# oicr-gsi/ConsensusCruncher

Measured on AMD Instinct MI355X. Metric: input reads/sec through SSCS+DCS+SC consensus, higher is better.
Workload: dtype u8

## Files before the change

### consensuscruncher_amd/csrc/bam_assemble.hip.inc

```
#include "assemble_core.h"

namespace {

static_assert(sizeof(asmb::Spec) == sizeof(cc_out_spec), "asmb::Spec is cc_out_spec");
static_assert(sizeof(asmb::Src) == 40 && sizeof(cc_asm_src) == 48, "source layouts");

struct AsmStatus {
    unsigned long long first_bad;
    unsigned long long total;
    unsigned long long key_or;
    uint32_t max_size, guard;
    uint32_t tot, pad;
};
static_assert(sizeof(AsmStatus) == 40, "status layout");

constexpr int ASM_T = 256;
constexpr int ASM_LANES = 16;

struct DevFetch {
    static __device__ __forceinline__ upk::W16 fetch(const uint8_t* base, uint64_t a, uint32_t valid) {
        return DevSrc{base, 0}.fetch(a, valid);
    }
};

__global__ __launch_bounds__(ASM_T) void k_asm_sizes(asmb::Tables T, const asmb::Spec* __restrict__ spec, int64_t n,
                                                     uint32_t* __restrict__ sz, uint64_t* __restrict__ key,
                                                     uint32_t* __restrict__ val, AsmStatus* st) {
    __shared__ unsigned long long s_bad, s_tot, s_or;
    __shared__ uint32_t s_max;
    if (threadIdx.x == 0) { s_bad = ~0ULL; s_tot = 0; s_or = 0; s_max = 0; }
    __syncthreads();
    const int64_t i = (int64_t)blockIdx.x * ASM_T + threadIdx.x;
    if (i < n) {
        asmb::Lay y;
        uint64_t k = 0;
        const uint32_t e = asmb::layout(spec[i], T, y, &k);
        if (e) {
            atomicMin(&s_bad, ((unsigned long long)i << 8) | e);
            y.size = 0;
            k = 0;
        } else {
            atomicAdd(&s_tot, (unsigned long long)y.size);
            atomicOr(&s_or, (unsigned long long)k);
            atomicMax(&s_max, y.size);
        }
        sz[i] = y.size;
        key[i] = k;
        val[i] = (uint32_t)i;
    }
    __syncthreads();
    if (threadIdx.x == 0) {
        if (s_bad != ~0ULL) atomicMin(&st->first_bad, s_bad);
        atomicAdd(&st->total, s_tot);
        atomicOr(&st->key_or, s_or);
        atomicMax(&st->max_size, s_max);
    }
}

__global__ __launch_bounds__(ASM_T) void k_asm_gather(const uint32_t* __restrict__ sz, const uint32_t* __restrict__ perm,
                                                      int64_t n, int64_t o0, int64_t cnt, uint32_t* __restrict__ ssz) {
    const int64_t i = (int64_t)blockIdx.x * ASM_T + threadIdx.x;
    if (i >= cnt) return;
    const int64_t s = perm ? (int64_t)perm[o0 + i] : o0 + i;
    ssz[i] = sz[CC_IDX(s, n, DS_REC)];
}

__global__ __launch_bounds__(ASM_T) void k_asm_copy(asmb::Tables T, const asmb::Spec* __restrict__ spec,
                                                    const uint32_t* __restrict__ perm, int64_t n, int64_t o0, int64_t cnt,
                                                    const uint32_t* __restrict__ off32, uint64_t base, uint64_t total,
                                                    uint8_t* __restrict__ out, uint64_t* __restrict__ at, AsmStatus* st) {
    const int64_t i = (int64_t)blockIdx.x * (ASM_T / ASM_LANES) + (threadIdx.x / ASM_LANES);
    const uint32_t j = threadIdx.x % ASM_LANES;
    if (i >= cnt) return;
    const int64_t o = o0 + i;
    const int64_t s = perm ? (int64_t)perm[o] : o;
    asmb::Lay y;
    uint64_t k;
    const uint32_t e = asmb::layout(spec[CC_IDX(s, n, DS_REC)], T, y, &k);
    const uint64_t off = base + off32[i];
    if (e || off > total || y.size > total - off || (uint64_t)s >= (uint64_t)n) {
        if (j == 0) atomicOr(&st->guard, 1u);
        return;
    }
    if (j == 0) {
        at[o] = off;
        if (o == n - 1) at[n] = off + y.size;
    }
    uint8_t* d = out + off;
    const uint32_t head = min(y.size, (16u - ((uint32_t)off & 15u)) & 15u);
    const uint32_t lines = (y.size - head) >> 4, tail_at = head + (lines << 4);
    if (j < head) d[j] = (uint8_t)asmb::out16<DevFetch>(y, T, j, 1u).w[0];
    uint4* dl = reinterpret_cast<uint4*>(d + head);
    for (uint32_t c = j; c < lines; c += ASM_LANES) {
        const upk::W16 w = asmb::out16<DevFetch>(y, T, head + (c << 4), 16u);
        dl[c] = make_uint4(w.w[0], w.w[1], w.w[2], w.w[3]);
    }
    if (tail_at + j < y.size) d[tail_at + j] = (uint8_t)asmb::out16<DevFetch>(y, T, tail_at + j, 1u).w[0];
}

struct AsmGuard {
    cc_ctx* ctx;
    std::vector<void*> tmp;
    uint8_t* kept = nullptr;
    ~AsmGuard() {
        (void)hipStreamSynchronize(ctx->stream);
        for (void* p : tmp) (void)hipFree(p);
        if (kept) (void)hipFree(kept);
    }
};

int asm_upload_padded(cc_ctx* ctx, std::vector<void*>& tmp, const uint8_t** dst, const void* src, uint64_t bytes) {
    const size_t padded = (size_t)((bytes + 15) & ~15ull) + 32;
    uint8_t* up = nullptr;
    RC(dev_alloc(ctx, tmp, &up, (int64_t)padded));
    if (bytes) HIPCHK(hipMemcpyAsync(up, src, (size_t)bytes, hipMemcpyHostToDevice, ctx->stream));
    HIPCHK(hipMemsetAsync(up + bytes, 0, padded - (size_t)bytes, ctx->stream));
    *dst = up;
    return 0;
}

const char* asm_refusal(uint32_t bits) {
    if (bits & asmb::AE_KIND) return "unknown kind";
    if (bits & asmb::AE_SRC) return "src_file or src_rec out of range";
    if (bits & asmb::AE_TMPL) return "a template whose l_read_name, n_cigar and l_seq do not fit its block_size or its stream";
    if (bits & asmb::AE_NAME) return "name_id out of range";
    if (bits & asmb::AE_LONGNAME) return "a new name longer than 254 bytes";
    if (bits & asmb::AE_CONS) return "cons_off + cons_len outside the consensus arrays";
    return "rg_id outside the RG table";
}

struct AsmArgs {
// ... 115 lines not shown
            char buf[240];
            snprintf(buf, sizeof buf, "cc_bam_assemble: spec %lld: %s", (long long)(h_st->first_bad >> 8),
                     asm_refusal((uint32_t)(h_st->first_bad & 0xff)));
            ctx->err = buf;
            return CC_E_INVALID;
        }
        sum += h_st->total;
    }
    if (total) *total = sum;
    if (!alloc && !keep) return 0;
    uint8_t* out = alloc ? alloc(actx, sum) : nullptr;
    if ((alloc && !out) || !at) { ctx->err = "cc_bam_assemble: no buffer for the stream"; return CC_E_INVALID; }
    at[0] = a.header_bytes;
    uint8_t* d_out = nullptr;
    if (keep) {
        const size_t padded = (size_t)((sum + 15) & ~15ull) + 32;
        HIPCHK(hipMalloc((void**)&guard.kept, padded));
        d_out = guard.kept;
        HIPCHK(hipMemsetAsync(d_out + sum, 0, padded - (size_t)sum, ctx->stream));
    }
    if (n == 0) {
        if (a.header_bytes && out) memcpy(out, a.header, (size_t)a.header_bytes);
        if (keep) {
            if (a.header_bytes) HIPCHK(hipMemcpyAsync(d_out, a.header, (size_t)a.header_bytes, hipMemcpyHostToDevice, ctx->stream));
            HIPCHK(hipStreamSynchronize(ctx->stream));
            *keep = Resident{guard.kept, sum};
            guard.kept = nullptr;
        }
        return 0;
    }
    if (a.flags & CCIO_W_SORT) {
        unsigned b0 = 0, b1 = 0;
        asmb::key_digits(h_st->key_or, &b0, &b1);
        RC(dev_alloc(ctx, guard.tmp, &key2, n, 64));
        RC(dev_alloc(ctx, guard.tmp, &perm, n, 64));
        RC(sort_pairs(ctx, key, key2, val, perm, n, "asm_sort", b0, b1));
    }
    uint64_t bound = 0xffffffffull;
    if (const char* e = getenv("CC_ASM_SLICE_BYTES")) {
        const unsigned long long v = strtoull(e, nullptr, 10);
        if (v > 0 && v < bound) bound = v;
    }
    const int64_t per = asmb::slice_records(bound, h_st->max_size);
    const int64_t cap = std::min(per, n);
    RC(dev_alloc(ctx, guard.tmp, &ssz, cap, 64));
    RC(dev_alloc(ctx, guard.tmp, &off32, cap, 64));
    if (!keep) RC(dev_alloc(ctx, guard.tmp, &d_out, (int64_t)sum, 64));
    uint64_t* d_at = nullptr;
    RC(dev_alloc(ctx, guard.tmp, &d_at, n + 1));
    if (a.header_bytes) HIPCHK(hipMemcpyAsync(d_out, a.header, (size_t)a.header_bytes, hipMemcpyHostToDevice, ctx->stream));
    uint64_t base = a.header_bytes;
    for (int64_t o0 = 0; o0 < n; o0 += per) {
        const int64_t cnt = std::min(per, n - o0);
        klaunch(ctx, "k_asm_gather", k_asm_gather, nblk(cnt, ASM_T), ASM_T, sz, perm, n, o0, cnt, ssz);
        RC(scan_launch(ctx, ssz, cnt, &d_st->tot, "asm_scan", ScanStore{off32}));
        klaunch(ctx, "k_asm_copy", k_asm_copy, nblk(cnt, ASM_T / ASM_LANES), ASM_T, T, d_spec, perm, n, o0, cnt, off32, base, sum,
                d_out, d_at, d_st);
        HIPCHK(hipGetLastError());
        HIPCHK(hipMemcpyAsync(h_st, d_st, sizeof(AsmStatus), hipMemcpyDeviceToHost, ctx->stream));
        HIPCHK(hipStreamSynchronize(ctx->stream));
        if (h_st->guard) { ctx->err = "cc_bam_assemble: a record outside the stream (guarded)"; return CC_E_INVALID; }
        base += h_st->tot;
    }
    if (base != sum) { ctx->err = "cc_bam_assemble: the offsets' scan totals do not match the sizes"; return CC_E_INVALID; }
    if (out) {
        ProfScope ps(ctx, "asm_download");
        HIPCHK(hipMemcpyAsync(out, d_out, (size_t)sum, hipMemcpyDeviceToHost, ctx->stream));
        HIPCHK(hipMemcpyAsync(at, d_at, sizeof(uint64_t) * (size_t)(n + 1), hipMemcpyDeviceToHost, ctx->stream));
    } else {
        HIPCHK(hipMemcpyAsync(at, d_at, sizeof(uint64_t) * (size_t)(n + 1), hipMemcpyDeviceToHost, ctx->stream));
    }
    HIPCHK(hipStreamSynchronize(ctx->stream));
    if (keep) {
        *keep = Resident{guard.kept, sum};
        guard.kept = nullptr;
    }
    return 0;
}

int bam_assemble_locked(cc_ctx* ctx, const AsmArgs& a, cc_asm_alloc_fn alloc, void* actx, uint64_t* at, uint64_t* total,
                        int64_t* rid = nullptr) {
    if (rid) *rid = 0;
    if (!ctx) return CC_E_INVALID;
    if (a.n < 0 || a.nsrc < 0 || a.n_names < 0 || a.n_rg < 0 || (a.header_bytes && !a.header) ||
        (a.n > 0 && (!a.spec || (a.nsrc > 0 && !a.srcs))) || (a.n_names > 0 && !a.name_off && !a.names_set) || (a.names_bytes && !a.names && !a.names_set) ||
        (a.n_rg > 0 && (!a.rg_off || !a.rg_blob)) ||
        (a.cons_group < 0 && ((a.cons_seq_bytes && !a.cons_seq) || (a.cons_qual_bytes && !a.cons_qual)))) {
        ctx->err = "cc_bam_assemble: null or negative argument";
        return CC_E_INVALID;
    }
    if (a.cons_group >= 0 && !ctx->groups.count(a.cons_group)) { ctx->err = "cc_bam_assemble: unknown group"; return CC_E_INVALID; }
    if (a.names_set) {
        const auto it = ctx->name_sets.find(a.names_set);
        if (it == ctx->name_sets.end()) { ctx->err = "cc_bam_assemble: unknown name set"; return CC_E_INVALID; }
        if (a.n_names > it->second.n || a.names_bytes > (uint64_t)it->second.total) {
            ctx->err = "cc_bam_assemble: n_names or names_bytes larger than the name set's";
            return CC_E_INVALID;
        }
    }
    std::vector<const uint8_t*> resident((size_t)a.nsrc, nullptr);
    bool any = false;
    for (int32_t f = 0; f < a.nsrc; ++f) {
        const cc_asm_src& s = a.srcs[f];
        if (s.nrec < 0 || (s.nrec > 0 && !s.rec_off) || (!s.stream && !s.resident_id && s.bytes)) {
            ctx->err = "cc_bam_assemble: a source without a stream";
            return CC_E_INVALID;
        }
// ... 115 lines not shown
```

### consensuscruncher_amd/csrc/cc_engine.hip

```cpp
#include <algorithm>
#include <climits>
#include <cstdint>
#include <cstdio>
#include <cstring>

#include <dlfcn.h>
#include <sched.h>

#include <chrono>

#include <hip/hip_runtime.h>
#include <atomic>
#include <map>
#include <memory>
#include <mutex>
#include <type_traits>
#include <string>
#include <unordered_map>
#include <unordered_set>
#include <utility>
#include <vector>

#include "../../include/consensuscruncher_amd.h"

static std::atomic<long long> g_launches{0};
#define hipMemsetAsync(...) (g_launches.fetch_add(1, std::memory_order_relaxed), ::hipMemsetAsync(__VA_ARGS__))
#define hipMemcpyAsync(...) (g_launches.fetch_add(1, std::memory_order_relaxed), ::hipMemcpyAsync(__VA_ARGS__))

enum : uint32_t {
    EB_COLLISION = 1u << 0,
    EB_DUP_QNAME = 1u << 1,
    EB_N_HIGHQ = 1u << 3,
    EB_BAD_BASE = 1u << 4,
    EB_SHORT = 1u << 5,
    EB_NO_QUAL = 1u << 6,
    EB_NO_CIGAR = 1u << 7,
    EB_RG = 1u << 8,
    EB_THR = 1u << 9,
    EB_TOO_LONG = 1u << 10,
    EB_KEYERROR = 1u << 12,
    EB_CHAIN = 1u << 13,
    EB_NEEDSORT = 1u << 14,
    EB_PLAN = 1u << 11,
    EB_DEEPSORT = 1u << 15,
    EB_SCANWAIT = 1u << 16,
    EB_GUARD = 1u << 17,
};

__device__ unsigned int g_guard;
__device__ __noinline__ int64_t guard_fail() {
    atomicOr(&g_guard, 1u);
    return 0;
}
#ifdef CC_DEBUG_BOUNDS
__device__ unsigned long long g_dbg_fault;
__device__ __noinline__ int64_t dbg_fail(int site, int64_t i) {
    atomicCAS(&g_dbg_fault, 0ULL, ((unsigned long long)site << 48) | ((unsigned long long)i & 0xffffffffffffULL));
    return 0;
}
__device__ __forceinline__ int64_t dbg_idx(int64_t i, int64_t n, int site) {
    return (i < 0 || i >= n) ? dbg_fail(site, i) : i;
}
#define CC_IDX(i, n, site) ((std::remove_cv_t<std::remove_reference_t<decltype(i)>>)dbg_idx((int64_t)(i), (int64_t)(n), (site)))
#elif defined(CC_NO_GUARD)
#define CC_IDX(i, n, site) (i)
#else
__device__ __forceinline__ int64_t guard_idx(int64_t i, int64_t n) {
    return (uint64_t)i < (uint64_t)n ? i : guard_fail();
}
#define CC_IDX(i, n, site) ((std::remove_cv_t<std::remove_reference_t<decltype(i)>>)guard_idx((int64_t)(i), (int64_t)(n)))
#endif
enum : int {
    DS_REC = 1, DS_QNAME = 2, DS_PAYLOAD = 3, DS_SLOT = 4, DS_PAIR = 5, DS_MEMBER = 6, DS_VOTE_REC = 7,
};

struct TagKey {
    int32_t bc, tid, pos, mtid, mpos, cigA, cigB;
    uint32_t bits;
};
struct CKey {
    int32_t bc, tidLo, posLo, tidHi, posHi, cigA, cigB;
    uint32_t strand;
    uint32_t abstlen;
    uint32_t pad[3];
};

constexpr int GRP_SMALL = 64;

struct alignas(32) RecCore {
    int32_t tid, pos, mtid, mpos, tlen, cig, bc, flag;
};

struct DevTable {
    int64_t n;
    int32_t *tid, *pos, *mtid, *mpos, *tlen, *cig, *qlen, *lseq, *bc, *rg;
    uint16_t* flag;
    uint8_t *mapq, *rflags;
    uint64_t* qn_off;
    uint16_t* qn_len;
    uint64_t* qn_ol;
    RecCore* core;
    uint8_t* qn_blob;
    uint64_t* pay_off;
    uint8_t* payload;
    uint64_t pay_bytes, qn_bytes;
    uint64_t* rdig;
    uint64_t* qdig;
    uint64_t qdig_mask;
    uint4* meta;
    uint64_t* rkey;
    uint32_t* ebits;
    uint8_t* rdeep;
    int32_t* dlist;
    uint32_t* ndeep;
    int64_t n_deep;
    bool derive_pending;
    bool host_layout;
    int32_t max_len;
    int64_t* tbase;
    int32_t* ext;
    int32_t* geom;
    int32_t ntid;
    int64_t bkt_cap;
};

__device__ __forceinline__ uint32_t nib_irregular(uint32_t x, uint32_t m88) {
    uint32_t p = x - ((x >> 1) & 0x55555555u);
    p = (p & 0x33333333u) + ((p >> 2) & 0x33333333u);
    const uint32_t a = p ^ 0x11111111u, b = p ^ 0x44444444u;
    const uint32_t za = ~((a | 0x88888888u) - 0x11111111u) & 0x88888888u;
    const uint32_t zb = ~((b | 0x88888888u) - 0x11111111u) & 0x88888888u;
    return ~(za | zb) & m88;
}
__device__ __forceinline__ uint32_t nib_mask(int nbase, int w) {
    int vb = nbase - 8 * w;
    vb = vb < 0 ? 0 : (vb > 8 ? 8 : vb);
    const int full = vb >> 1;
    uint32_t m = full >= 4 ? 0x88888888u : (((1u << (8 * full)) - 1u) & 0x88888888u);
    if ((vb & 1) && full < 4) m |= 0x80u << (8 * full);
    return m;
}

constexpr int BC_T = 256;
__device__ __forceinline__ uint64_t pos_key(int32_t tid, int32_t pos) {
    return ((uint64_t)(uint32_t)(tid < 0 ? -1 : tid) << 32) | (uint64_t)(uint32_t)pos;
}

constexpr int DEEP_MIN = 65;
constexpr uint64_t QDIG_SEED = 0x6a09e667f3bcc909ULL;
__device__ __forceinline__ uint64_t qname_hash(const DevTable& T, int32_t r, uint64_t seed);
__device__ __forceinline__ void build_meta_rec(const DevTable& T, int32_t* __restrict__ rec_e, uint32_t* __restrict__ err,
                                               int32_t* __restrict__ dlist, uint32_t* __restrict__ ndeep, int64_t dcap) {
    const int64_t r = (int64_t)blockIdx.x * BC_T + threadIdx.x;
    if (r == 0) {
        const uint32_t eb = *T.ebits;
        if (eb) atomicOr(err, eb);
    }
    if (dlist) {
        bool dp = false;
        if (r < T.n) {
            const int32_t t = T.tid[r], p = T.pos[r];
            const bool start = r == 0 || T.tid[r - 1] != t || T.pos[r - 1] != p;
            const int64_t q = r + DEEP_MIN - 1;
            dp = start && q < T.n && T.tid[q] == t && T.pos[q] == p;
// ... 2153 lines not shown
                    for (int k = 0; k < SE / 2; ++k) {
                        const uint32_t i = (uint32_t)((h + k) * DF_ST + t);
                        const uint32_t pm = A[lo[k] + sp - 1];
                        if ((i & w) ? (pm <= v[k]) : (pm < v[k])) lo[k] += sp;
                    }
                }
#pragma unroll
                for (int k = 0; k < SE / 2; ++k) {
                    const uint32_t i = (uint32_t)((h + k) * DF_ST + t);
                    if (i >= p2) continue;
                    const uint32_t pm = A[lo[k]];
                    if ((i & w) ? (pm <= v[k]) : (pm < v[k])) lo[k] += 1;
                    const uint32_t st = i & ~(2 * w - 1), other = st + ((i & w) ? 0u : w);
                    B[st + (i & (w - 1)) + (lo[k] - other)] = v[k];
                }
            }
            __syncthreads();
            uint32_t* tmp = A; A = B; B = tmp;
        }
        for (int h = 0; h < SE; h += SE / 2) {
            uint32_t v[SE / 2];
            int32_t r[SE / 2];
#pragma unroll
            for (int k = 0; k < SE / 2; ++k) {
                const uint32_t i = (uint32_t)((h + k) * DF_ST + t);
                v[k] = i < m ? A[i] : 0u;
                r[k] = i < m ? CC_IDX((v[k] & 1u) ? V.rec2[v[k] >> 1] : V.rec1[v[k] >> 1], T.n, DS_REC) : 0;
            }
#pragma unroll
            for (int k = 0; k < SE / 2; ++k) {
                const uint32_t i = (uint32_t)((h + k) * DF_ST + t);
                if (i < m) deep_put(out, V, T, d.z + (int64_t)i, v[k], r[k], i == 0, i == 0 || (v[k] >> 1) != (A[i - 1] >> 1), err);
            }
        }
    }
}

__global__ __launch_bounds__(256) void k_fam_build(int64_t F, int64_t R, int64_t n_known, int one_region,
                                                   const int32_t* __restrict__ fam_beg,
                                                   const int32_t* __restrict__ fam_drop,
                                                   const uint32_t* __restrict__ rs_val, const uint64_t* __restrict__ rs_key,
                                                   const int32_t* __restrict__ pr_region, const uint64_t* __restrict__ rhash,
                                                   const int32_t* __restrict__ mem_rec, int32_t* __restrict__ fam_end,
                                                   int32_t* __restrict__ fam_n, int32_t* __restrict__ fam_first,
                                                   int32_t* __restrict__ fam_region, uint64_t* __restrict__ fam_hash,
                                                   uint8_t* __restrict__ cflag, int32_t* __restrict__ cfam,
                                                   int32_t* __restrict__ fam_o, PairView V, DevTable T,
                                                   TagKey* __restrict__ fam_tag, int32_t* __restrict__ fam_rec) {
    int64_t f = (int64_t)blockIdx.x * blockDim.x + threadIdx.x;
    if (f < F) {
        fam_o[f] = 0x7f7f7f7f;
        int32_t b = CC_IDX(fam_beg[f], R, DS_SLOT);
        int32_t e = (f + 1 < F) ? fam_beg[f + 1] : (int32_t)R;
        if (e < b || e > R) e = b + (int32_t)guard_fail() + 1;
        fam_end[f] = e;
        fam_n[f] = e - b - fam_drop[f];
        uint32_t fe = rs_val[b];
        fam_first[f] = (int32_t)fe;
        fam_region[f] = one_region ? 0 : pr_region[fe >> 1];
        fam_hash[f] = rhash && b >= n_known ? rhash[CC_IDX(mem_rec[b], T.n, DS_REC)] : rs_key[b];
        cflag[fe] = 1;
        cfam[fe] = (int32_t)f;
        if (fam_tag) {
            const int32_t r0 = mem_rec[b];
            fam_tag[f] = tag_of_rec(T, r0, V.tag[fe >> 1]);
            fam_rec[f] = r0;
        }
    }
}

__global__ __launch_bounds__(256) void k_fam_tags(int64_t F, const int32_t* __restrict__ fam_first,
                                                  const int32_t* __restrict__ fam_beg, const int32_t* __restrict__ mem_rec,
                                                  PairView V, DevTable T, TagKey* __restrict__ fam_tag,
                                                  int32_t* __restrict__ fam_rec) {
    const int64_t f = (int64_t)blockIdx.x * blockDim.x + threadIdx.x;
    if (f < F) {
        const int32_t r0 = mem_rec[fam_beg[f]];
        fam_tag[f] = tag_of_rec(T, r0, V.tag[fam_first[f] >> 1]);
        fam_rec[f] = r0;
    }
}

__global__ __launch_bounds__(256) void k_csn_keys(int64_t F, const int32_t* __restrict__ fam_by_k,
                                                  const int32_t* __restrict__ fam_first, const uint64_t* __restrict__ chash,
                                                  uint64_t* __restrict__ ekey, uint32_t* __restrict__ eval) {
    int64_t k = (int64_t)blockIdx.x * blockDim.x + threadIdx.x;
    if (k >= F) return;
    int32_t f = fam_by_k[k];
    ekey[k] = chash[fam_first[f] >> 1];
    eval[k] = (uint32_t)k;
}

__global__ __launch_bounds__(256) void k_csn_mark(int64_t F, const uint64_t* __restrict__ es_key,
                                                  const uint32_t* __restrict__ es_val, const int32_t* __restrict__ fam_by_k,
                                                  const int32_t* __restrict__ fam_first, PairView V, DevTable T,
                                                  uint32_t* __restrict__ segf, uint32_t* __restrict__ err) {
    int64_t j = (int64_t)blockIdx.x * blockDim.x + threadIdx.x;
    if (j >= F) return;
    bool start = (j == 0) || es_key[j - 1] != es_key[j];
    if (!start) {
        int32_t pa = fam_first[fam_by_k[es_val[j]]] >> 1, pb = fam_first[fam_by_k[es_val[j - 1]]] >> 1;
        if (!ckey_eq(ckey_of_pair(T, V, pa), ckey_of_pair(T, V, pb))) {
            atomicOr(err, EB_COLLISION);
            start = true;
        }
    }
    segf[j] = start;
// ... 535 lines not shown
    for (int pi = 0; pi < 4; ++pi) {
        int32_t c = 0;
#pragma unroll
        for (int i = 0; i < MODE_K; ++i)
            if (i < nv && val[i] == pri[pi]) c = num[i];
        if (c == best_cnt) { out = pri[pi]; return true; }
    }
    return true;
}

struct SwarWord {
    uint32_t pc, ca, cc, cg, orb, ql;
};

__device__ __forceinline__ uint32_t ff_of_80(uint32_t m80) { return (m80 - (m80 >> 7)) | m80; }

__device__ __forceinline__ uint32_t min60_bytes(uint32_t q) {
    const uint32_t hi = ff_of_80((((q | 0x80808080u) - 0x3d3d3d3du) | q) & 0x80808080u);
    return (hi & 0x3c3c3c3cu) | (~hi & q);
}

__device__ __forceinline__ void swar_member(SwarWord& s, uint32_t w, uint32_t q) {
    const uint32_t p80 = (((q | 0x80808080u) - 0x1e1e1e1eu) | q) & 0x80808080u;
    const uint32_t p1 = p80 >> 7;
    const uint32_t pff = (p80 - p1) | p80;
    s.pc += p1;
    s.ql = (q & pff) | (s.ql & ~pff);
    const uint32_t wp = w & pff;
    s.orb |= wp;
    s.ca += wp & 0x01010101u;
    s.cc += wp & 0x02020202u;
    s.cg += wp & 0x04040404u;
}

__global__ __launch_bounds__(256) void k_vote_plan(
    int64_t n, int64_t nmem, int64_t nvcap, const uint8_t* __restrict__ needv, const uint32_t* __restrict__ vx,
    const int32_t* __restrict__ emit_fam, const int2* __restrict__ emit_span, const uint4* __restrict__ mem_meta,
    const int32_t* __restrict__ mem_rec, DevTable T, int32_t* __restrict__ vote_fam, int4* __restrict__ vote_order,
    int32_t* __restrict__ emit_vslot, int32_t* __restrict__ out_meta, uint32_t* __restrict__ slow_n,
    int32_t* __restrict__ slow_list, uint32_t* __restrict__ n_items, int all_slow, uint32_t* __restrict__ err) {
    __shared__ uint32_t s_bin[64], s_cur[64];
    __shared__ int64_t s_vb;
    const int tid = threadIdx.x;
    const int64_t o = (int64_t)blockIdx.x * blockDim.x + tid;
    int4 rec = make_int4(0, 0, 0, -1);
    int key = -1;
    uint32_t eb = 0;
    if (o < n) {
        const bool need = needv[o] != 0;
        const uint32_t vxo = vx[o];
        const int32_t f = emit_fam[o];
        int2 sp = emit_span[o];
        const bool over = need && (int64_t)vxo >= nvcap;
        if (over) guard_fail();
        if (!need || over) {
            emit_vslot[o] = -1;
        } else {
            const int32_t v = (int32_t)vxo;
            vote_fam[v] = f;
            emit_vslot[o] = v;
            if (sp.x < 0 || sp.y < 0 || (int64_t)sp.x + sp.y > nmem) sp = make_int2((int32_t)guard_fail(), 0);
            const int32_t beg = sp.x, cnt = sp.y;
            const uint4* fm = mem_meta + beg;
            const uint4 m0 = cnt > 0 ? fm[0] : make_uint4(0u, 0u, 0u, 0u);
            const uint32_t ql0 = m0.z >> 16;
            const int32_t L = ql0 == 0xffffu ? -1 : (int32_t)ql0;
            uint32_t d = 0;
            const bool slow = cnt > VOTE_BIGN || all_slow;
            for (int32_t k0 = 0; !slow && k0 < cnt; k0 += 4) {
                uint4 mm[4];
#pragma unroll
                for (int u = 0; u < 4; ++u) mm[u] = k0 + u < cnt ? fm[k0 + u] : make_uint4(0u, 0u, 0u, 0u);
#pragma unroll
                for (int u = 0; u < 4; ++u) {
                    const uint4 m = mm[u];
                    if (!((m.w >> 23) & 1u)) continue;
                    const uint32_t ls = m.z & 0xffffu;
                    if (L < 0) eb |= EB_NO_CIGAR;
                    else if ((int32_t)ls < L) eb |= EB_SHORT;
                    if (((m.w >> 20) & CC_RF_QUAL_MISSING) && L > 0) eb |= EB_NO_QUAL;
                    if (((m.w >> 12) & 0xffu) != ((m0.w >> 12) & 0xffu)) d |= 1u;
                    if (m.y != m0.y) d |= 2u;
                    if ((m.w & 0xfffu) != (m0.w & 0xfffu)) d |= 4u;
                    const uint32_t rg7 = (m.w >> 24) & 0x7fu;
                    const bool badrg = ((m.w >> 20) & CC_RF_RG_UNSUPPORTED) != 0;
                    if (rg7 != ((m0.w >> 24) & 0x7fu)) d |= 8u;
                    if (rg7 == 0x7eu) d |= 64u;
                    if (rg7 == 0x7fu && !badrg) d |= 16u;
                    if (badrg) d |= 32u;
                }
            }
            key = 0;
            rec = make_int4(beg, 0, 0, v);
            if (slow) {
                slow_list[atomicAdd(slow_n, 1u)] = v;
                if (cnt > BIG_CH) atomicAdd(n_items, (uint32_t)((cnt + BIG_CH - 1) / BIG_CH));
                eb = 0;
            } else {
                int32_t mapq = (int32_t)((m0.w >> 12) & 0xffu), tlen = (int32_t)m0.y, flag = (int32_t)(m0.w & 0xfffu);
                const auto g_mapq = [](const uint4& m) { return (int32_t)((m.w >> 12) & 0xffu); };
                const auto g_tlen = [](const uint4& m) { return (int32_t)m.y; };
                const auto g_flag = [](const uint4& m) { return (int32_t)(m.w & 0xfffu); };
                if ((d & 1u) && !table_mode(cnt, fm, g_mapq, false, mapq))
                    mapq = serial_mode(0, cnt, fm, [&](int32_t, const uint4& m) { return g_mapq(m); }, false);
                if ((d & 2u) && !table_mode(cnt, fm, g_tlen, false, tlen))
                    tlen = serial_mode(0, cnt, fm, [&](int32_t, const uint4& m) { return g_tlen(m); }, false);
                if ((d & 4u) && !table_mode(cnt, fm, g_flag, true, flag))
                    flag = serial_mode(0, cnt, fm, [&](int32_t, const uint4& m) { return g_flag(m); }, true);
                int32_t rg = -1;
                if (!(d & 16u)) {
                    if (d & 32u) eb |= EB_RG;
                    else if (!(d & (8u | 64u))) rg = (int32_t)((m0.w >> 24) & 0x7fu);
                    else rg = serial_mode(0, cnt, fm, [&](int32_t j, const uint4& m) {
                        const uint32_t r7 = (m.w >> 24) & 0x7fu;
                        return r7 == 0x7eu ? T.rg[mem_rec[beg + j]] : (int32_t)r7; }, false);
                }
                const int32_t Lp = L < 0 ? 0 : L;
                out_meta[5 * v + 0] = Lp;
                out_meta[5 * v + 1] = mapq;
                out_meta[5 * v + 2] = tlen;
                out_meta[5 * v + 3] = flag;
                out_meta[5 * v + 4] = rg;
                rec = make_int4(beg, cnt, Lp, v);
                key = cnt;
            }
        }
    }
    if (eb) atomicOr(err, eb);
    if (tid < 64) s_bin[tid] = 0u;
    if (tid == 0) s_vb = (int64_t)blockIdx.x * blockDim.x < n ? (int64_t)vx[(int64_t)blockIdx.x * blockDim.x] : 0;
    __syncthreads();
    if (key >= 0) atomicAdd(&s_bin[key], 1u);
    __syncthreads();
    if (tid < 64) {
        const uint32_t c = s_bin[tid];
        uint32_t x = c;
#pragma unroll
        for (int d2 = 1; d2 < 64; d2 <<= 1) {
            const uint32_t y = __shfl_up(x, d2, 64);
            if (tid >= d2) x += y;
        }
        s_cur[tid] = x - c;
    }
    __syncthreads();
    if (key >= 0) {
        const int64_t at = s_vb + atomicAdd(&s_cur[key], 1u);
        if (at < nvcap) vote_order[at] = rec;
        else guard_fail();
    }
}

__device__ __noinline__ uint32_t lone_quality(const uint4* __restrict__ fm, int32_t cnt, int32_t i, uint32_t code,
                                              const uint8_t* __restrict__ payload) {
    uint32_t qs = 0;
    for (int32_t k = 0; k < cnt; ++k) {
        const uint4 mk = fm[k];
        const uint32_t lsk = mk.z & 0xffffu;
        if (!((mk.w >> 23) & 1u) || i >= (int32_t)lsk) continue;
        const uint64_t qok = (uint64_t)mk.x << 4;
        const uint32_t qq = payload[qok + i];
        const uint32_t by = payload[qok + ((lsk + 15u) & ~15u) + (i >> 1)];
        const uint32_t b = (i & 1) ? (by & 15u) : (by >> 4);
        if (qq >= 30u && b == code) qs += qq;
    }
    return qs > 60u ? 60u : qs;
}

__device__ __noinline__ bool passing_n(const uint4* __restrict__ fm, int32_t cnt, int32_t i,
                                       const uint8_t* __restrict__ payload) {
    for (int32_t k = 0; k < cnt; ++k) {
        const uint4 mk = fm[k];
        const uint32_t lsk = mk.z & 0xffffu;
        if (!((mk.w >> 23) & 1u) || i >= (int32_t)lsk) continue;
        const uint64_t qok = (uint64_t)mk.x << 4;
        const uint32_t by = payload[qok + ((lsk + 15u) & ~15u) + (i >> 1)];
        const uint32_t b = (i & 1) ? (by & 15u) : (by >> 4);
        if (payload[qok + i] >= 30u && b == 15u) return true;
    }
    return false;
}

__device__ __forceinline__ void swar_finish(SwarWord (&s)[4], const uint32_t (&lm)[4], uint32_t irr, bool act,
                                            int32_t i0, int32_t cnt, int64_t v, const uint4* __restrict__ fm,
                                            const DevTable& T, const int32_t* __restrict__ thr, int32_t uni_ok,
                                            int32_t qstride, uint8_t* __restrict__ out_seq,
                                            uint8_t* __restrict__ out_qual, uint32_t& eb) {
    if (irr) eb |= EB_BAD_BASE;
    uint32_t code[4], qo[4], multi = 0;
#pragma unroll
    for (int w = 0; w < 4; ++w) {
        const SwarWord& x = s[w];
        const uint32_t z80 = ~((x.pc | 0x80808080u) - 0x01010101u) & 0x80808080u;
        const uint32_t z15 = (z80 >> 3) - (z80 >> 7);
        code[w] = uni_ok ? (x.orb | z15) : 0x0f0f0f0fu;
        const uint32_t g2 = ff_of_80(((x.pc | 0x80808080u) - 0x02020202u) & 0x80808080u);
        qo[w] = (g2 & 0x3c3c3c3cu) | (~g2 & min60_bytes(x.ql));
        const uint32_t mu = x.orb & ((x.orb | 0x80808080u) - 0x01010101u) & lm[w];
        const uint32_t mb = ((mu | (mu >> 1) | (mu >> 2) | (mu >> 3)) & 0x01010101u) * 0x01020408u;
        multi |= (mb >> 24) << (4 * w);
    }
#pragma unroll 1
// ... 5 lines not shown
#define SV_SEL4(f) (w == 0 ? s[0].f : w == 1 ? s[1].f : w == 2 ? s[2].f : s[3].f)
        const uint32_t xca = SV_SEL4(ca), xcc = SV_SEL4(cc), xcg = SV_SEL4(cg), xpc = SV_SEL4(pc), xql = SV_SEL4(ql),
                       xorb = SV_SEL4(orb);
#undef SV_SEL4
        const int32_t a = (int32_t)((xca >> sh) & 0xffu);
        const int32_t cC = (int32_t)(((xcc >> sh) & 0xffu) >> 1);
        const int32_t gG = (int32_t)(((xcg >> sh) & 0xffu) >> 2);
        const int32_t pass = (int32_t)((xpc >> sh) & 0xffu);
        const int32_t tT = pass - a - cC - gG;
        const int32_t pos = i0 + 8 * (w >> 1) + 2 * j + (w & 1);
        if (((xorb >> sh) & 0xffu) == 15u && passing_n(fm, cnt, pos, T.payload)) eb |= EB_N_HIGHQ;
        int32_t best = a, mbase = 0;
        if (cC > best) { best = cC; mbase = 1; }
        if (gG > best) { best = gG; mbase = 2; }
        if (tT > best) { best = tT; mbase = 3; }
        const uint32_t cj = (pass > 0 && best >= thr[pass]) ? (1u << mbase) : 15u;
        uint32_t qj;
        if (best >= 2) qj = 60u;
        else if (best <= 0) qj = 0u;
        else if (pass == 1) { const uint32_t qq = (xql >> sh) & 0xffu; qj = qq > 60u ? 60u : qq; }
        else qj = lone_quality(fm, cnt, pos, 1u << mbase, T.payload);
        const uint32_t keep = ~(0xffu << sh);
        if (w == 0) { code[0] = (code[0] & keep) | (cj << sh); qo[0] = (qo[0] & keep) | (qj << sh); }
        else if (w == 1) { code[1] = (code[1] & keep) | (cj << sh); qo[1] = (qo[1] & keep) | (qj << sh); }
        else if (w == 2) { code[2] = (code[2] & keep) | (cj << sh); qo[2] = (qo[2] & keep) | (qj << sh); }
        else { code[3] = (code[3] & keep) | (cj << sh); qo[3] = (qo[3] & keep) | (qj << sh); }
    }
    if (act) {
        uint4 qout;
        qout.x = __builtin_amdgcn_perm(qo[1] & lm[1], qo[0] & lm[0], 0x05010400u);
        qout.y = __builtin_amdgcn_perm(qo[1] & lm[1], qo[0] & lm[0], 0x07030602u);
        qout.z = __builtin_amdgcn_perm(qo[3] & lm[3], qo[2] & lm[2], 0x05010400u);
        qout.w = __builtin_amdgcn_perm(qo[3] & lm[3], qo[2] & lm[2], 0x07030602u);
        *reinterpret_cast<uint4*>(out_qual + v * (int64_t)qstride + i0) = qout;
        *reinterpret_cast<uint2*>(out_seq + v * (int64_t)(qstride >> 1) + (i0 >> 1)) =
            make_uint2(((code[0] & lm[0]) << 4) | (code[1] & lm[1]), ((code[2] & lm[2]) << 4) | (code[3] & lm[3]));
    }
}

__global__ __launch_bounds__(256, CC_SV_WAVES) void k_sscs_vote_swar(
    int64_t nv, int32_t fpw, int32_t chunks, const int4* __restrict__ vote_order, const uint4* __restrict__ mem_meta,
    int64_t nmem, DevTable T, const int32_t* __restrict__ thr, int32_t uni_ok, int32_t qstride,
    uint8_t* __restrict__ out_seq, uint8_t* __restrict__ out_qual, uint32_t* __restrict__ err) {
    const int lane = threadIdx.x & 63;
    const int64_t wave = (int64_t)blockIdx.x * (blockDim.x >> 6) + (threadIdx.x >> 6);
    const int g = lane / chunks, c = lane - g * chunks;
    const int64_t t = wave * fpw + g;
    int32_t beg = 0, cnt = 0, L = 0;
    int64_t v = 0;
    if (g < fpw && t < nv) {
        const int4 vi = vote_order[t];
        beg = vi.x; cnt = vi.y; L = vi.z; v = vi.w;
        if (beg < 0 || cnt < 0 || (int64_t)beg + cnt > nmem || v < 0 || v >= nv) {
            beg = (int32_t)guard_fail();
            cnt = 0;
        }
    }
    const int32_t i0 = SV_POS * c;
    uint32_t eb = 0;
    const bool act = i0 < L;
    if (cnt > 0) {
        uint32_t lm[4];
        {
            uint32_t lp[4];
#pragma unroll
            for (int k = 0; k < 4; ++k) {
                const int32_t rem = L - i0 - 4 * k;
                lp[k] = rem >= 4 ? 0xffffffffu : (rem <= 0 ? 0u : ((1u << (8 * rem)) - 1u));
            }
            lm[0] = __builtin_amdgcn_perm(lp[1], lp[0], 0x06040200u);
            lm[1] = __builtin_amdgcn_perm(lp[1], lp[0], 0x07050301u);
            lm[2] = __builtin_amdgcn_perm(lp[3], lp[2], 0x06040200u);
            lm[3] = __builtin_amdgcn_perm(lp[3], lp[2], 0x07050301u);
        }
        SwarWord s[4];
#pragma unroll
        for (int k = 0; k < 4; ++k) s[k] = SwarWord{};
        const uint4* fm = mem_meta + beg;
        const int nbl = L - i0 < 16 ? (L - i0 > 0 ? L - i0 : 0) : 16;
        const uint32_t irx = nib_mask(nbl, 0), iry = nib_mask(nbl, 1);
        uint32_t irr = 0;
        const int gl = g * chunks;
        for (int32_t k0 = 0; k0 < cnt; k0 += chunks) {
            const uint4 mine = (k0 + c < cnt) ? fm[k0 + c] : make_uint4(0u, 0u, 0u, 0u);
            const int kn = cnt - k0 < chunks ? cnt - k0 : chunks;
            for (int u0 = 0; u0 < kn; u0 += SV_U) {
                uint4 qv[SV_U];
                uint2 sv[SV_U];
                uint32_t vm[SV_U];
#pragma unroll
                for (int u = 0; u < SV_U; ++u) {
                    const int src = gl + (u0 + u < kn ? u0 + u : kn - 1);
                    const uint32_t mx = (uint32_t)__shfl((int)mine.x, src);
                    const uint32_t mz = (uint32_t)__shfl((int)mine.z, src);
                    const uint32_t mw = (uint32_t)__shfl((int)mine.w, src);
                    const uint32_t ls = mz & 0xffffu;
                    const bool ok = act & (u0 + u < kn) & (((mw >> 23) & 1u) != 0u) & (i0 < (int32_t)ls);
                    vm[u] = ok ? 0xffffffffu : 0u;
                    const uint32_t off = ok ? (uint32_t)i0 : 0u;
                    const uint8_t* base = T.payload + CC_IDX((uint64_t)mx << 4, T.pay_bytes + 1, DS_PAYLOAD);
                    qv[u] = *reinterpret_cast<const uint4*>(base + off);
                    sv[u] = *reinterpret_cast<const uint2*>(base + ((ls + 15u) & ~15u) + (off >> 1));
                }
#pragma unroll
                for (int u = 0; u < SV_U; ++u) {
                    const uint4 q = qv[u];
                    const uint2 sq = sv[u];
// ... 573 lines not shown
            if (s >= 0) { dx = 1; break; }
            if (g < 0) { dx = 3; break; }
            if (G.fam_o[g] >= ox) { dx = 2; comp = false; break; }
            if (n == DUPLEX_CHAIN) { atomicOr(err, EB_CHAIN); break; }
            ++n;
            x = g;
            ox = G.fam_o[g];
        }
        for (int i = n - 1; i >= 0; --i) {
            const bool deleted = dx == 1 || dx == 3 || (dx == 2 && comp);
            if (deleted) { dx = 3; comp = false; }
            else { comp = dx == 2 && !comp; dx = 2; }
        }
        d = dx == 1 ? 0 : dx == 2 ? 1 : 2;
        if (d == 0) pr = S.fam_rec[s0];
        else if (d == 1) pr = G.fam_rec[g0];
        if (gdel) {
            const int32_t rt = G.fam_region[f];
            if (dx == 1) { atomicMin(&gdel[f], rt); atomicMin(&sdel[s0], rt); }
            else if (dx == 3) atomicMin(&gdel[f], rt);
            else if (dx == 2 && comp) { atomicMin(&gdel[f], rt); atomicMin(&gdel[g0], rt); }
        }
    }
    dec[q] = d;
    t_rec[q] = tr;
    p_rec[q] = pr;
    fl_corr[q] = (d == 0 || d == 1) ? 1 : 0;
}


__device__ __forceinline__ void duplex_word(uint32_t wa, uint32_t wb, uint32_t qa, uint32_t qb, int sc,
                                            uint32_t& code, uint32_t& qual) {
    uint32_t ok = ~(((wa ^ wb) | 0x80808080u) - 0x01010101u) & 0x80808080u;
    if (sc) {
        ok &= (((qa | 0x80808080u) - 0x1e1e1e1eu) | qa) & 0x80808080u;
        ok &= (((qb | 0x80808080u) - 0x1e1e1e1eu) | qb) & 0x80808080u;
    }
    const uint32_t ff = ff_of_80(ok);
    code = (wa & ff) | (0x0f0f0f0fu & ~ff);
    qual = min60_bytes(min60_bytes(qa) + min60_bytes(qb)) & ff;
}

__global__ __launch_bounds__(256) void k_duplex_vote_swar(
    int64_t nv, int sc, int32_t fpw, int32_t chunks, const int4* __restrict__ vpair,
    DevTable TA, DevTable TB, int32_t qstride, uint8_t* __restrict__ out_seq, uint8_t* __restrict__ out_qual,
    int32_t* __restrict__ out_meta, uint32_t* __restrict__ err) {
    const int lane = threadIdx.x & 63;
    const int64_t wave = (int64_t)blockIdx.x * (blockDim.x >> 6) + (threadIdx.x >> 6);
    const int g = lane / chunks, c = lane - g * chunks;
    const int64_t w = wave * fpw + g;
    uint32_t eb = 0;
    if (g < fpw && w < nv) {
        const int4 vp = vpair[w];
        const int32_t a = CC_IDX(vp.x, TA.n, DS_VOTE_REC), b = vp.y;
        const bool b_in_a = sc && vp.z == 1;
        const DevTable& TBx = b_in_a ? TA : TB;
        const uint8_t* bpay = TBx.payload;
        const uint4 ma = TA.meta[a], mb = TBx.meta[CC_IDX(b, TBx.n, DS_VOTE_REC)];
        const int32_t la = (int32_t)(ma.z & 0xffffu), lb = (int32_t)(mb.z & 0xffffu);
        int32_t L = la;
        if (lb < L) { eb |= EB_SHORT; L = 0; }
        if (L > 0 && (((ma.w | mb.w) >> 20) & CC_RF_QUAL_MISSING)) eb |= EB_NO_QUAL;
        for (int32_t i0 = SV_POS * c; i0 < L; i0 += SV_POS * chunks) {
            const uint64_t qa = (uint64_t)ma.x << 4, qb = (uint64_t)mb.x << 4;
            const uint64_t sa = qa + (uint64_t)((la + 15) & ~15), sb = qb + (uint64_t)((lb + 15) & ~15);
            const uint4 QA = *reinterpret_cast<const uint4*>(TA.payload + qa + i0);
            const uint4 QB = *reinterpret_cast<const uint4*>(bpay + qb + i0);
            const uint2 SA = *reinterpret_cast<const uint2*>(TA.payload + sa + (i0 >> 1));
            const uint2 SB = *reinterpret_cast<const uint2*>(bpay + sb + (i0 >> 1));
            uint32_t lp[4];
#pragma unroll
            for (int k = 0; k < 4; ++k) {
                const int32_t rem = L - i0 - 4 * k;
                lp[k] = rem >= 4 ? 0xffffffffu : (rem <= 0 ? 0u : ((1u << (8 * rem)) - 1u));
            }
            const uint4 QM = make_uint4(QA.x & lp[0], QA.y & lp[1], QA.z & lp[2], QA.w & lp[3]);
            const uint4 QN = make_uint4(QB.x & lp[0], QB.y & lp[1], QB.z & lp[2], QB.w & lp[3]);
            uint32_t code[4], qo[4];
            duplex_word((SA.x >> 4) & 0x0f0f0f0fu, (SB.x >> 4) & 0x0f0f0f0fu,
                        __builtin_amdgcn_perm(QM.y, QM.x, 0x06040200u), __builtin_amdgcn_perm(QN.y, QN.x, 0x06040200u),
                        sc, code[0], qo[0]);
            duplex_word(SA.x & 0x0f0f0f0fu, SB.x & 0x0f0f0f0fu,
                        __builtin_amdgcn_perm(QM.y, QM.x, 0x07050301u), __builtin_amdgcn_perm(QN.y, QN.x, 0x07050301u),
                        sc, code[1], qo[1]);
            duplex_word((SA.y >> 4) & 0x0f0f0f0fu, (SB.y >> 4) & 0x0f0f0f0fu,
                        __builtin_amdgcn_perm(QM.w, QM.z, 0x06040200u), __builtin_amdgcn_perm(QN.w, QN.z, 0x06040200u),
                        sc, code[2], qo[2]);
            duplex_word(SA.y & 0x0f0f0f0fu, SB.y & 0x0f0f0f0fu,
                        __builtin_amdgcn_perm(QM.w, QM.z, 0x07050301u), __builtin_amdgcn_perm(QN.w, QN.z, 0x07050301u),
                        sc, code[3], qo[3]);
            const uint32_t lm0 = __builtin_amdgcn_perm(lp[1], lp[0], 0x06040200u);
            const uint32_t lm1 = __builtin_amdgcn_perm(lp[1], lp[0], 0x07050301u);
            const uint32_t lm2 = __builtin_amdgcn_perm(lp[3], lp[2], 0x06040200u);
            const uint32_t lm3 = __builtin_amdgcn_perm(lp[3], lp[2], 0x07050301u);
            code[0] &= lm0; code[1] &= lm1; code[2] &= lm2; code[3] &= lm3;
            uint4 qout;
            qout.x = __builtin_amdgcn_perm(qo[1], qo[0], 0x05010400u) & lp[0];
            qout.y = __builtin_amdgcn_perm(qo[1], qo[0], 0x07030602u) & lp[1];
            qout.z = __builtin_amdgcn_perm(qo[3], qo[2], 0x05010400u) & lp[2];
            qout.w = __builtin_amdgcn_perm(qo[3], qo[2], 0x07030602u) & lp[3];
            *reinterpret_cast<uint4*>(out_qual + w * (int64_t)qstride + i0) = qout;
            *reinterpret_cast<uint2*>(out_seq + w * (int64_t)(qstride >> 1) + (i0 >> 1)) =
                make_uint2((code[0] << 4) | code[1], (code[2] << 4) | code[3]);
        }
        if (c == 0) {
            const int fa = (int)(ma.w & 0xfffu), fb = (int)(mb.w & 0xfffu);
            int32_t mapq = (int32_t)((ma.w >> 12) & 0xffu), tlen = (int32_t)ma.y, flag = fa, rg;
            const int32_t ra = TA.rg[a], rb = TBx.rg[b];
            if (sc) {
                rg = ra;
                if ((ma.w >> 20) & CC_RF_RG_UNSUPPORTED) eb |= EB_RG;
// ... 446 lines not shown
    __syncthreads();
    if (base + SCAN_TILE <= n) {
        if constexpr (Emit::kStaged) {
            typename Emit::Ld ld[SCAN_I];
            uint32_t fx[SCAN_I], xx[SCAN_I];
#pragma unroll
            for (int j = 0; j < SCAN_I / 4; ++j) {
                const int o = (j * SCAN_T + tid) * 4;
                const uint4 x = reinterpret_cast<const uint4*>(s_tile)[o >> 2];
                const uint32_t f = *reinterpret_cast<const uint32_t*>(in + base + o);
                xx[4 * j] = x.x; xx[4 * j + 1] = x.y; xx[4 * j + 2] = x.z; xx[4 * j + 3] = x.w;
#pragma unroll
                for (int k = 0; k < 4; ++k) fx[4 * j + k] = (f >> (8 * k)) & 0xffu;
            }
#pragma unroll
            for (int e = 0; e < SCAN_I; ++e) ld[e] = em.ld1(base + ((e >> 2) * SCAN_T + tid) * 4 + (e & 3), fx[e]);
#pragma unroll
            for (int e = 0; e < SCAN_I; ++e) em.ld2(ld[e], fx[e]);
#pragma unroll
            for (int e = 0; e < SCAN_I; ++e) em.st(base + ((e >> 2) * SCAN_T + tid) * 4 + (e & 3), xx[e], fx[e], ld[e]);
        } else {
#pragma unroll
            for (int j = 0; j < SCAN_I / 4; ++j) {
                const int o = (j * SCAN_T + tid) * 4;
                const uint4 x = reinterpret_cast<const uint4*>(s_tile)[o >> 2];
                if constexpr (Emit::kPlain) {
                    *reinterpret_cast<uint4*>(em.out + base + o) = x;
                } else {
                    const uint32_t f = *reinterpret_cast<const uint32_t*>(in + base + o);
                    em(base + o, x.x, f & 0xffu);
                    em(base + o + 1, x.y, (f >> 8) & 0xffu);
                    em(base + o + 2, x.z, (f >> 16) & 0xffu);
                    em(base + o + 3, x.w, f >> 24);
                }
            }
        }
    } else {
        for (int o = tid; o < SCAN_TILE; o += SCAN_T) {
            if (base + o >= n) continue;
            if constexpr (Emit::kPlain) em.out[base + o] = s_tile[o];
            else emit_one(em, base + o, s_tile[o], (uint32_t)in[base + o]);
        }
    }
}

__device__ __forceinline__ uint32_t stripe_sum(const uint32_t* __restrict__ stripes, int slot) {
    uint32_t v = 0;
    if (stripes)
        for (int k = 0; k < PSTRIPES; ++k) v += stripes[((int64_t)slot * PSTRIPES + k) * PSTRIDE];
    return v;
}

__global__ __launch_bounds__(64) void k_guard_fold(uint32_t* __restrict__ err) {
    if (threadIdx.x == 0 && g_guard) {
        atomicOr(err, EB_GUARD);
        g_guard = 0u;
    }
}
__global__ __launch_bounds__(256) void k_defer_pack(const uint32_t* __restrict__ err,
                                                    const unsigned long long* __restrict__ cnt,
                                                    const uint32_t* __restrict__ plan, int nplan,
                                                    const uint32_t* __restrict__ stripes, uint8_t* __restrict__ h) {
    const int t = threadIdx.x;
    if (t == 0) {
        *reinterpret_cast<uint32_t*>(h) = *err | (g_guard ? EB_GUARD : 0u);
        if (g_guard) g_guard = 0u;
    }
    if (cnt && t < CC_NUM_COUNTERS) {
        unsigned long long v = 0;
        for (int k = 0; k < CNT_STRIPES; ++k) v += cnt[CC_NUM_COUNTERS * k + t];
        reinterpret_cast<unsigned long long*>(h + 1024)[t] = v;
    }
    if (plan)
        for (int i = t; i < nplan; i += blockDim.x)
            reinterpret_cast<uint32_t*>(h + 256)[i] = plan[i] + stripe_sum(stripes, i);
}

__global__ __launch_bounds__(64) void k_stripe_fold(const uint32_t* __restrict__ stripes, uint32_t* __restrict__ plan,
                                                    int nplan) {
    for (int i = threadIdx.x; i < nplan; i += blockDim.x) plan[i] += stripe_sum(stripes, i);
}

constexpr int RS_T = 256, RS_I = 16, RS_TILE = RS_T * RS_I, RS_BINS = 256;
__global__ __launch_bounds__(RS_T) void k_rs_hist(const uint64_t* __restrict__ keys, int64_t n, int shift,
                                                  uint32_t* __restrict__ hist, int64_t nt) {
    __shared__ uint32_t s_h[RS_BINS];
    const int t = threadIdx.x;
    s_h[t] = 0u;
    __syncthreads();
    const int64_t base = (int64_t)blockIdx.x * RS_TILE;
    uint32_t d[RS_I];
#pragma unroll
    for (int i = 0; i < RS_I; ++i) {
        const int64_t x = base + (int64_t)i * RS_T + t;
        d[i] = x < n ? (uint32_t)(keys[x] >> shift) & 255u : 0xffffffffu;
    }
#pragma unroll
    for (int i = 0; i < RS_I; ++i)
        if (d[i] != 0xffffffffu) atomicAdd(&s_h[d[i]], 1u);
    __syncthreads();
    hist[(int64_t)t * nt + blockIdx.x] = s_h[t];
}
__global__ __launch_bounds__(RS_T) void k_rs_scatter(const uint64_t* __restrict__ kin, const uint32_t* __restrict__ vin,
                                                     int64_t n, int shift, const uint32_t* __restrict__ off, int64_t nt,
                                                     uint64_t* __restrict__ kout, uint32_t* __restrict__ vout) {
    __shared__ uint32_t s_base[RS_BINS];
    __shared__ uint32_t s_wc[RS_T / 64][RS_BINS];
    const int t = threadIdx.x, lane = t & 63, wv = t >> 6;
    s_base[t] = off[(int64_t)t * nt + blockIdx.x];
#pragma unroll
    for (int w = 0; w < RS_T / 64; ++w) s_wc[w][t] = 0u;
    const uint64_t lt = (1ULL << lane) - 1ULL;
    const int64_t base = (int64_t)blockIdx.x * RS_TILE;
    for (int i = 0; i < RS_I; ++i) {
        const int64_t x = base + (int64_t)i * RS_T + t;
        const bool valid = x < n;
        const uint64_t k = valid ? kin[x] : 0ULL;
        const uint32_t v = valid ? vin[x] : 0u;
        const uint32_t d = (uint32_t)(k >> shift) & 255u;
// ... 60 lines not shown
    X(vote_slow_list, int32_t) X(cutoff_thr, int32_t) X(vote_big_item, int32_t) X(vote_items, int4)                  \
    X(vote_partial, uint8_t) X(vote_item_fl, uint32_t) X(bc_swap, int32_t) X(dec, int32_t) X(t_rec, int32_t)         \
    X(p_rec, int32_t) X(fl_dcs, uint8_t) X(fl_corr, uint8_t) X(ht_key, unsigned long long) X(ht_val, int32_t)        \
    X(fam_bkt, int32_t) X(fam_del, int32_t) X(vslot, int32_t) X(vpair, int4) X(q_pair, int32_t) X(q_ckey, int32_t)   \
                               \
    X(grp_keys, uint32_t) X(grp_tab, int32_t) X(grp_slot_of, int32_t) X(grp_slot_first, int32_t)                     \
    X(grp_slot_cnt, int32_t) X(grp_start, uint32_t) X(grp_fx, uint32_t) X(grp_fsize, uint32_t)                       \
    X(grp_foff, uint32_t) X(grp_fkey, uint64_t) X(grp_fval, uint32_t) X(grp_skey, uint64_t) X(grp_sval, uint32_t)    \
    X(join_keys, uint32_t) X(join_pkeys, uint32_t) X(join_xkeys, uint32_t) X(join_tab, int32_t)                      \
    X(join_xtab, int32_t) X(join_p, int32_t) X(join_xs, int32_t) X(join_xfirst, int32_t) X(join_indeg, int32_t)      \
    X(join_dec, int32_t) X(join_part, int32_t) X(join_flags, uint32_t) X(join_used, uint8_t) X(join_gone, uint8_t)   \
    X(join_xgone, uint8_t) X(eb_h1, uint8_t) X(eb_h2, uint8_t) X(eb_l1, int32_t) X(eb_l2, int32_t)                   \
    X(eb_status, uint8_t) X(eb_bc, char) X(eb_cut1, int32_t) X(eb_cut2, int32_t) X(eb_bad1, uint32_t)                \
    X(eb_bad2, uint32_t) X(eb_counts, unsigned long long) X(eb_hist, unsigned long long)                             \
    X(eb_tkey, unsigned long long) X(eb_tval, int32_t) X(reduce_buf, int64_t) X(reduce_max, int64_t)

enum class B : int {
#define X(name, T) name,
    CC_GROUP_BUFFERS(X)
#undef X
    COUNT
};
constexpr const char* BUF_NAME[] = {
#define X(name, T) #name,
    CC_GROUP_BUFFERS(X)
#undef X
};
template <B id> struct BufType;
#define X(name, T) template <> struct BufType<B::name> { using type = T; };
CC_GROUP_BUFFERS(X)
#undef X
template <B id> using BufT = typename BufType<id>::type;

#define CC_PLAN_TOTALS(X)                                                                                            \
    X(n_resid) X(n_big) X(n_drop) X(n_long) X(lp_found) X(n_multi) X(resid_app) X(lp_total) X(resid_multi)           \
    X(deep_ovf) X(deep_items) X(deep_big) X(csn_shared) X(scan_resid) X(scan_pairs) X(scan_small) X(scan_bigE)       \
    X(scan_deep) X(scan_fam) X(scan_creation) X(scan_entries) X(scan_emit) X(scan_vote) X(vote_items) X(vote_slow)   \
    X(scan_bad) X(scan_dcs) X(scan_sc) X(grp_scan_fam) X(grp_scan_off)

enum class PT : int {
#define X(name) name,
    CC_PLAN_TOTALS(X)
#undef X
    COUNT
};
constexpr const char* PLAN_NAME[] = {
#define X(name) #name,
    CC_PLAN_TOTALS(X)
#undef X
};
constexpr int PLAN_SLOTS = 64;
static_assert((int)PT::COUNT <= PLAN_SLOTS, "a planned total's slot is its id");

enum Stage { ST_READ_BAM, ST_SSCS, ST_DCS, ST_SC, ST_COUNT };
constexpr const char* STAGE_NAME[ST_COUNT] = {"read_bam", "sscs", "dcs", "sc"};

struct Group {
    int32_t table = -1;
    int64_t S = 0, P = 0, R = 0, F = 0, E = 0, Q = 0, NV = 0;
    uint64_t seed = 0;
    int scoped = 0, delim_filter = 0, badread = 0;
    uint64_t ht_mask = 0;
    bool csn_fast = false;
    bool stripes_pending = false;
    bool no_deep_fam = false;
    int coord_sorted = 0;
    bool force_sort = false;
    int ident = 0;
    bool local_groups = false;
    int64_t counters[CC_NUM_COUNTERS] = {0};
    DevBuf buf[(int)B::COUNT];
    template <B id> BufT<id>* ptr() const { return (BufT<id>*)buf[(int)id].p; }
    int64_t plan[(int)PT::COUNT] = {0};
    bool plan_set[(int)PT::COUNT] = {false};
    bool planned[ST_COUNT] = {false};
    bool fast = false;
    bool members_built = false;
    int64_t n_deepg = 0;
    bool fam_tags_built = false;
    bool overlap = false;
    int32_t n_regions = 1;
    std::vector<PT> verify;
    std::vector<int32_t> swap_host;
    double thr_cutoff = -1.0;
};

struct DeferredCheck {
    Group* g = nullptr;
    int32_t gid = -1;
    int slot = 0;
    bool counters = false;
    bool bad_listed = false;
    std::vector<std::pair<int, int64_t>> expect;
};
constexpr int DEFER_SLOTS = 64;
constexpr size_t DEFER_SLOT_BYTES = 12288;

constexpr int CC_E_PLAN = -100;
constexpr int CC_E_NEEDSORT = -101;
constexpr int CC_E_DEEPSORT = -102;
constexpr int CC_E_SCANWAIT = -103;

using NameIndex = std::unordered_map<std::string, int>;
NameIndex name_index(const char* const* names, int n) {
    NameIndex ix;
    for (int i = 0; i < n; ++i) ix[names[i]] = i;
    return ix;
}
const NameIndex BUF_IDS = name_index(BUF_NAME, (int)B::COUNT);
const NameIndex PLAN_IDS = name_index(PLAN_NAME, (int)PT::COUNT);
inline int name_id(const NameIndex& ix, const char* name) {
    const auto it = ix.find(name);
    return it != ix.end() ? it->second : -1;
}

struct EngineSwitches {
    int scan1 = -1;
    int pc_tile = 0;
    bool resid_sort = false;
    bool resid_scan = false;
    bool qdig = true;
    int qdig_bits = 0;
    bool dcs_per_entry = false;
    int64_t lp_min = LP_MIN;
    bool ltab_cas = false;
    bool group_staged = false;
    bool meta_scalar = false;
    bool derive_separate = false;
    bool gr_by_pair = false;
    bool deep_sort = false;
    bool trace_upload = false;
};

EngineSwitches read_switches() {
    EngineSwitches sw;
    if (const char* v = getenv("CC_SCAN1")) sw.scan1 = v[0] == '1' ? 1 : 0;
    if (const char* v = getenv("CC_PC_TILE")) sw.pc_tile = atoi(v) == 512 ? 512 : 1024;
    sw.resid_sort = getenv("CC_RESID_SORT") != nullptr;
    sw.resid_scan = getenv("CC_RESID_SCAN") != nullptr;
    if (const char* v = getenv("CC_QDIG")) sw.qdig = v[0] != '0';
    if (const char* v = getenv("CC_QDIG_BITS")) sw.qdig_bits = atoi(v) > 0 && atoi(v) < 64 ? atoi(v) : 0;
    sw.dcs_per_entry = getenv("CC_DCS_PER_ENTRY") != nullptr;
    if (const char* v = getenv("CC_LP_MIN")) sw.lp_min = atoll(v);
    sw.ltab_cas = getenv("CC_LTAB_CAS") != nullptr;
    sw.group_staged = getenv("CC_GROUP_STAGED") != nullptr;
    sw.meta_scalar = getenv("CC_META_SCALAR") != nullptr;
    sw.derive_separate = getenv("CC_DERIVE_SEPARATE") != nullptr;
    sw.gr_by_pair = getenv("CC_GR_BY_PAIR") != nullptr;
    sw.deep_sort = getenv("CC_DEEP_SORT") != nullptr;
    sw.trace_upload = getenv("CC_TRACE_UPLOAD") != nullptr;
    return sw;
}

}

struct BgzfEnc;

struct NameSet {
    uint8_t* blob = nullptr;
    int64_t* off = nullptr;
    int64_t n = 0, total = 0;
};

struct cc_ctx {
    int device = 0;
    hipStream_t stream = nullptr;
    std::string err;
    EngineSwitches sw;
    std::map<int32_t, DevTable> tables;
    std::map<int32_t, std::vector<void*>> table_allocs;
    std::map<int32_t, std::unique_ptr<Group>> groups;
    int32_t next_id = 1;
    DevBuf tmp;
    DevBuf sort_buf;
    unsigned long long* scan_st = nullptr;
    uint32_t* scan_ticket = nullptr;
    int64_t scan_cap = 0;
    uint32_t scan_epoch = 0;
    uint32_t scan_spin_max = 1u << 22;
    bool scan_two = false;
    std::unordered_set<int32_t> full_qhash;
    int64_t scan_retries = 0;
    int64_t guard_reruns = 0;
    uint32_t* d_err = nullptr;
    unsigned long long* d_cnt = nullptr;
    void* h_pinned = nullptr;
    std::atomic<bool> profiling{false};
    std::unordered_set<std::string> prof_only;
    struct Prof { double ms = 0; int64_t n = 0; };
    std::map<std::string, Prof> prof;
    std::vector<std::pair<std::string, std::pair<hipEvent_t, hipEvent_t>>> pending;
    std::vector<hipEvent_t> event_pool;
    std::unique_ptr<Group> scratch;
    bool defer = false;
    std::vector<DeferredCheck> deferred;
    uint8_t* h_defer = nullptr;
    uint8_t* d_defer = nullptr;
    BgzfEnc* bgzf = nullptr;
    std::mutex bgzf_mu;
    int32_t asm_group = -1;
    uint8_t* names_buf = nullptr;
    int64_t names_total = -1;
    int64_t* names_off = nullptr;
    int64_t names_n = 0;
    std::map<int64_t, NameSet> name_sets;
    int64_t asm_names = 0;
};

namespace {

#define HIPCHK(x)                                                                               \
    do {                                                                                        \
        hipError_t e_ = (x);                                                                    \
        if (e_ != hipSuccess) {                                                                 \
            ctx->err = std::string("HIP error ") + hipGetErrorString(e_) + " at " #x;           \
            return CC_E_HIP;                                                                    \
        }                                                                                       \
    } while (0)

#define RC(x)                     \
    do {                          \
        int rc_ = (x);            \
        if (rc_) return rc_;      \
    } while (0)

int enter(cc_ctx* ctx) {
    HIPCHK(hipSetDevice(ctx->device));
    ctx->sw = read_switches();
    return 0;
}

inline unsigned nblk(int64_t n, int b = 256) { return (unsigned)((n + b - 1) / b); }

template <class... P, class... A>
inline void klaunch(hipStream_t stream, void (*kernel)(P...), dim3 grid, dim3 block, A&&... args) {
    g_launches.fetch_add(1, std::memory_order_relaxed);
    kernel<<<grid, block, 0, stream>>>(std::forward<A>(args)...);
}
template <class... P, class... A>
inline void klaunch(cc_ctx* ctx, void (*kernel)(P...), dim3 grid, dim3 block, A&&... args) {
    klaunch(ctx->stream, kernel, grid, block, std::forward<A>(args)...);
}

struct Fills {
    cc_ctx* ctx;
    FillSet fs{};
    int64_t maxw = 0;
    explicit Fills(cc_ctx* c) : ctx(c) { fs.k = 0; }
    int add(void* p, size_t bytes, uint32_t word) {
        if (!p || bytes < 4) return 0;
        if (fs.k == FillSet::K) { int rc = launch(); if (rc) return rc; }
        fs.p[fs.k] = (uint32_t*)p;
        fs.n[fs.k] = (int64_t)(bytes / 4);
        fs.v[fs.k] = word;
        maxw = std::max<int64_t>(maxw, (int64_t)(bytes / 4));
        ++fs.k;
        return 0;
    }
    int launch();
};

void* gbuf_bytes(cc_ctx* ctx, Group& g, B id, size_t need, int* rc) {
    DevBuf& b = g.buf[(int)id];
    if (b.bytes < need) {
        if (b.p) (void)hipFree(b.p);
        b.p = nullptr;
        hipError_t e = hipMalloc(&b.p, need);
        if (e != hipSuccess) {
            ctx->err = std::string("hipMalloc failed for ") + BUF_NAME[(int)id] + ": " + hipGetErrorString(e);
            *rc = CC_E_HIP;
            b.bytes = 0;
            return nullptr;
        }
        b.bytes = need;
    }
    return b.p;
}

template <B id>
BufT<id>* gbuf(cc_ctx* ctx, Group& g, int64_t count, int* rc) {
    using T = BufT<id>;
    void* p = gbuf_bytes(ctx, g, id, (size_t)std::max<int64_t>(count, 1) * sizeof(T), rc);
    if (p) g.buf[(int)id].used = (size_t)std::max<int64_t>(count, 0) * sizeof(T);
    return (T*)p;
}

void* tmp_storage(cc_ctx* ctx, size_t bytes, int* rc) {
    if (ctx->tmp.bytes < bytes) {
        if (ctx->tmp.p) (void)hipFree(ctx->tmp.p);
        ctx->tmp.p = nullptr;
        size_t nb = bytes + bytes / 4 + 4096;
        if (hipMalloc(&ctx->tmp.p, nb) != hipSuccess) {
            ctx->err = "hipMalloc temp storage failed";
            *rc = CC_E_HIP;
            ctx->tmp.bytes = 0;
            return nullptr;
        }
        ctx->tmp.bytes = nb;
    }
    return ctx->tmp.p;
}

struct ProfScope {
    cc_ctx* ctx;
    const char* name;
    hipEvent_t a = nullptr, b = nullptr;
    static hipEvent_t take(cc_ctx* ctx) {
        hipEvent_t e = nullptr;
        if (!ctx->event_pool.empty()) {
            e = ctx->event_pool.back();
            ctx->event_pool.pop_back();
        } else {
            (void)hipEventCreate(&e);
        }
        return e;
    }
    ProfScope(cc_ctx* c, const char* n) : ctx(c), name(n) {
        if (ctx->profiling && !ctx->prof_only.empty() && !ctx->prof_only.count(n)) name = nullptr;
        if (ctx->profiling && name) {
            a = take(ctx);
            b = take(ctx);
            (void)hipEventRecord(a, ctx->stream);
        }
    }
    ~ProfScope() {
        if (ctx->profiling && name) {
            (void)hipEventRecord(b, ctx->stream);
            ctx->pending.push_back({name, {a, b}});
        }
    }
};

template <class... P, class... A>
inline void klaunch(cc_ctx* ctx, const char* scope, void (*kernel)(P...), dim3 grid, dim3 block, A&&... args) {
    ProfScope ps(ctx, scope);
    klaunch(ctx->stream, kernel, grid, block, std::forward<A>(args)...);
}

void flush_prof(cc_ctx* ctx) {
    if (ctx->pending.empty()) return;
    (void)hipStreamSynchronize(ctx->stream);
    for (auto& p : ctx->pending) {
        float ms = 0;
        (void)hipEventElapsedTime(&ms, p.second.first, p.second.second);
        auto& pr = ctx->prof[p.first];
        pr.ms += ms;
        pr.n += 1;
        ctx->event_pool.push_back(p.second.first);
        ctx->event_pool.push_back(p.second.second);
    }
    ctx->pending.clear();
}

template <class Emit, class TIn>
int scan_launch(cc_ctx* ctx, const TIn* in, int64_t n, uint32_t* d_tot, const char* name, Emit em);

int sort_pairs(cc_ctx* ctx, const uint64_t* kin, uint64_t* kout, const uint32_t* vin, uint32_t* vout, int64_t n,
               const char* name, unsigned begin_bit = 0, unsigned end_bit = 64) {
    if (n <= 0) return 0;
    if (n > (int64_t)UINT32_MAX - 1) { ctx->err = "sort: more than 2^32 - 2 pairs"; return CC_E_UNSUPPORTED; }
    const int passes = end_bit > begin_bit ? (int)((end_bit - begin_bit + 7) / 8) : 0;
    const int64_t nt = (n + RS_TILE - 1) / RS_TILE;
    const size_t need = (size_t)n * 12 + 2 * sizeof(uint32_t) * (size_t)RS_BINS * (size_t)nt + 256;
    if (ctx->sort_buf.bytes < need) {
        if (ctx->sort_buf.p) {
            HIPCHK(hipStreamSynchronize(ctx->stream));
            (void)hipFree(ctx->sort_buf.p);
        }
        ctx->sort_buf.p = nullptr;
        ctx->sort_buf.bytes = 0;
        const size_t nb = need + need / 4;
        HIPCHK(hipMalloc(&ctx->sort_buf.p, nb));
        ctx->sort_buf.bytes = nb;
    }
    uint8_t* sb = (uint8_t*)ctx->sort_buf.p;
    uint64_t* tk = (uint64_t*)sb;
    uint32_t* tv = (uint32_t*)(sb + (size_t)n * 8);
    uint32_t* hist = (uint32_t*)(sb + (((size_t)n * 12 + 127) & ~(size_t)127));
    uint32_t* off = hist + (size_t)RS_BINS * nt;
    uint32_t* tot = (uint32_t*)ctx->d_err + 14;
    ProfScope ps(ctx, name);
    if (passes == 0) {
        HIPCHK(hipMemcpyAsync(kout, kin, sizeof(uint64_t) * n, hipMemcpyDeviceToDevice, ctx->stream));
        HIPCHK(hipMemcpyAsync(vout, vin, sizeof(uint32_t) * n, hipMemcpyDeviceToDevice, ctx->stream));
        return 0;
    }
    const uint64_t* sk = kin;
    const uint32_t* sv = vin;
    for (int p = 0; p < passes; ++p) {
        const int shift = (int)begin_bit + 8 * p;
        uint64_t* dk = ((passes - p) & 1) ? kout : tk;
        uint32_t* dv = ((passes - p) & 1) ? vout : tv;
        klaunch(ctx, k_rs_hist, (unsigned)nt, RS_T, sk, n, shift, hist, nt);
        RC(scan_launch(ctx, hist, (int64_t)RS_BINS * nt, tot, "sort_scan", ScanStore{off}));
        klaunch(ctx, k_rs_scatter, (unsigned)nt, RS_T, sk, sv, n, shift, off, nt, dk, dv);
        sk = dk;
        sv = dv;
    }
    return 0;
}

constexpr int64_t SCAN_ONE_MAX = 64;
template <class Emit, class TIn>
int scan_launch(cc_ctx* ctx, const TIn* in, int64_t n, uint32_t* d_tot, const char* name, Emit em) {
    const int64_t nb = (n + SCAN_TILE - 1) / SCAN_TILE;
    uintptr_t al = (uintptr_t)in;
    if constexpr (Emit::kPlain) al |= (uintptr_t)em.out;
    if (al & 15u) { ctx->err = "scan operands must be 16-B aligned"; return CC_E_INVALID; }
    const bool one = !ctx->scan_two && (ctx->sw.scan1 >= 0 ? ctx->sw.scan1 == 1 : nb <= SCAN_ONE_MAX);
    if (one && nb > 0) {
        if (nb > ctx->scan_cap) {
            const int64_t cap = std::max<int64_t>(nb, 1 << 14);
            if (ctx->scan_st) {
                HIPCHK(hipStreamSynchronize(ctx->stream));
                (void)hipFree(ctx->scan_st);
            }
            ctx->scan_st = nullptr;
            ctx->scan_cap = 0;
            HIPCHK(hipMalloc((void**)&ctx->scan_st, sizeof(unsigned long long) * cap + 64));
            HIPCHK(hipMemsetAsync(ctx->scan_st, 0, sizeof(unsigned long long) * cap + 64, ctx->stream));
            ctx->scan_ticket = reinterpret_cast<uint32_t*>(ctx->scan_st + cap);
            ctx->scan_cap = cap;
            ctx->scan_epoch = 0;
        }
        if (++ctx->scan_epoch >= (1u << 30)) {
            HIPCHK(hipMemsetAsync(ctx->scan_st, 0, sizeof(unsigned long long) * ctx->scan_cap, ctx->stream));
            ctx->scan_epoch = 1;
        }
        const ScanLB lb{ctx->scan_st, ctx->scan_ticket, ctx->scan_epoch, ctx->d_err, ctx->scan_spin_max};
        klaunch(ctx, name, k_scan_one<Emit, TIn>, (unsigned)nb, SCAN_T, in, n, nb, d_tot, em, lb);
        return 0;
    }
    int rc = 0;
    uint32_t* part = (uint32_t*)tmp_storage(ctx, (size_t)nb * 4 + 64, &rc);
    if (!part) return rc;
    ProfScope ps(ctx, name);
    klaunch(ctx, k_scan_reduce<TIn>, (unsigned)nb, SCAN_T, in, n, part);
    klaunch(ctx, k_scan_down<Emit, TIn>, (unsigned)nb, SCAN_T, in, n, part, d_tot, em);
    return 0;
}



hipError_t stream_wait(cc_ctx* ctx) {
    const auto t0 = std::chrono::steady_clock::now();
    for (uint32_t i = 0;; ++i) {
        const hipError_t e = hipStreamQuery(ctx->stream);
        if (e != hipErrorNotReady) return e;
        if ((i & 63u) == 63u && std::chrono::steady_clock::now() - t0 > std::chrono::microseconds(200)) sched_yield();
    }
}

int dbg_fault(cc_ctx* ctx) {
#ifdef CC_DEBUG_BOUNDS
    unsigned long long f = 0;
    HIPCHK(hipMemcpyFromSymbol(&f, HIP_SYMBOL(g_dbg_fault), sizeof(f), 0, hipMemcpyDeviceToHost));
    if (f) {
        const unsigned long long zero = 0;
        HIPCHK(hipMemcpyToSymbol(HIP_SYMBOL(g_dbg_fault), &zero, sizeof(zero), 0, hipMemcpyHostToDevice));
        static const char* names[] = {"?", "record index", "qname offset", "payload offset", "ranked slot", "pair",
                                      "member record", "vote record"};
        const int site = (int)(f >> 48);
        char buf[160];
        snprintf(buf, sizeof buf, "device bounds check failed: %s %lld out of range (debug build)",
                 names[site >= 0 && site < 8 ? site : 0], (long long)(int64_t)(f & 0xffffffffffffULL));
        ctx->err = buf;
        return CC_E_INVALID;
    }
#else
    (void)ctx;
#endif
    return 0;
}

int Fills::launch() {
    if (fs.k == 0) return 0;
    const unsigned blocks = std::min<unsigned>(nblk((maxw + 3) / 4), 2048u);
    klaunch(ctx, k_fill, blocks, 256, fs);
    fs.k = 0;
    maxw = 0;
    return hipGetLastError() == hipSuccess ? 0 : CC_E_HIP;
}
// ... 36 lines not shown
template <class Emit, class TIn>
int scan_emit(cc_ctx* ctx, Group& g, const TIn* in, int64_t n, int64_t* total, PT id, Emit em) {
    if (n <= 0) { *total = 0; return 0; }
    int rc = 0;
    uint32_t* d_tot = plan_slot(ctx, g, id, &rc);
    if (rc) return rc;
    RC(scan_launch(ctx, in, n, d_tot, PLAN_NAME[(int)id], em));
    return planned_total(ctx, g, id, d_tot, total);
}
template <class TIn>
int scan_total(cc_ctx* ctx, Group& g, const TIn* in, uint32_t* out, int64_t n, int64_t* total, PT id) {
    return scan_emit(ctx, g, in, n, total, id, ScanStore{out});
}

int finish_pass(cc_ctx* ctx, Group& g, uint32_t* bits, bool counters, bool* plan_ok) {
    if (ctx->defer && g.fast && ctx->h_defer && ctx->deferred.size() < (size_t)DEFER_SLOTS) {
        DeferredCheck d;
        d.g = &g;
        for (auto& kv : ctx->groups)
            if (kv.second.get() == &g) d.gid = kv.first;
        d.slot = (int)ctx->deferred.size();
        d.counters = counters;
        d.bad_listed = g.counters[CC_CNT_BAD_LISTED] > 0;
        uint8_t* dh = ctx->d_defer + (size_t)d.slot * DEFER_SLOT_BYTES;
        const bool totals = !g.verify.empty();
        klaunch(ctx, k_defer_pack, 1, 256, ctx->d_err, counters ? ctx->d_cnt : nullptr,
                totals ? g.ptr<B::plan_totals>() : nullptr, PLAN_SLOTS,
                g.stripes_pending ? g.ptr<B::plan_stripes>() : nullptr, dh);
        g.stripes_pending = false;
        if (totals)
            for (const PT id : g.verify) d.expect.push_back({(int)id, g.plan[(int)id]});
        g.verify.clear();
        ctx->deferred.push_back(std::move(d));
        *bits = 0;
        *plan_ok = true;
        return 0;
    }
    uint8_t* h = (uint8_t*)ctx->h_pinned;
    klaunch(ctx, k_guard_fold, 1, 64, ctx->d_err);
    HIPCHK(hipMemcpyAsync(h + 16, ctx->d_err, 4, hipMemcpyDeviceToHost, ctx->stream));
    if (counters)
        HIPCHK(hipMemcpyAsync(h + 1024, ctx->d_cnt, sizeof(unsigned long long) * CC_NUM_COUNTERS * CNT_STRIPES,
                              hipMemcpyDeviceToHost,
                              ctx->stream));
    if (g.stripes_pending) {
        klaunch(ctx, k_stripe_fold, 1, 64, g.ptr<B::plan_stripes>(), g.ptr<B::plan_totals>(), PLAN_SLOTS);
        g.stripes_pending = false;
    }
    if (!g.verify.empty())
        HIPCHK(hipMemcpyAsync(h + 256, g.ptr<B::plan_totals>(), 4 * PLAN_SLOTS, hipMemcpyDeviceToHost, ctx->stream));
    HIPCHK(stream_wait(ctx));
    RC(dbg_fault(ctx));
    *bits = *(uint32_t*)(h + 16);
    if ((*bits & EB_GUARD) && g.fast) ++ctx->guard_reruns;
    const bool cap_over = (*bits & EB_PLAN) != 0 || (g.fast && (*bits & EB_GUARD) != 0);
    *bits &= g.fast ? ~(EB_PLAN | EB_GUARD) : ~EB_PLAN;
    if (counters)
        for (int i = 0; i < CC_NUM_COUNTERS; ++i) {
            int64_t t = 0;
            for (int k = 0; k < CNT_STRIPES; ++k) t += (int64_t)((unsigned long long*)(h + 1024))[CC_NUM_COUNTERS * k + i];
            g.counters[i] = t;
        }
    *plan_ok = !cap_over;
    for (const PT id : g.verify)
        if ((int64_t)((uint32_t*)(h + 256))[(int)id] != g.plan[(int)id]) *plan_ok = false;
    g.verify.clear();
    return 0;
}

template <typename Pass>
int run_planned(cc_ctx* ctx, Group& g, Stage stage, Pass pass) {
    int rc = CC_E_PLAN;
    if (g.planned[stage]) {
        g.fast = true;
        g.verify.clear();
        rc = pass();
        g.fast = false;
    }
    if (rc == CC_E_PLAN) {
        g.verify.clear();
        rc = pass();
    }
    if (rc == CC_E_SCANWAIT && !ctx->scan_two) {
        ++ctx->scan_retries;
        if (getenv("CC_SCAN_SPIN_MAX")) fprintf(stderr, "[cc] %s: look-back scan bound hit, pass re-run (%lld)\n", STAGE_NAME[stage],
                                                (long long)ctx->scan_retries);
        ctx->scan_two = true;
        g.verify.clear();
        rc = pass();
        ctx->scan_two = false;
    }
    if (rc == CC_E_SCANWAIT) rc = CC_E_INVALID;
    g.planned[stage] = rc == 0;
    return rc;
}

int read_err(cc_ctx* ctx, uint32_t* bits) {
    uint32_t* h = (uint32_t*)ctx->h_pinned + 4;
    klaunch(ctx, k_guard_fold, 1, 64, ctx->d_err);
    HIPCHK(hipMemcpyAsync(h, ctx->d_err, 4, hipMemcpyDeviceToHost, ctx->stream));
    HIPCHK(stream_wait(ctx));
    *bits = *h;
    return dbg_fault(ctx);
}

int err_code(cc_ctx* ctx, uint32_t bits) {
    if (!bits) return 0;
    if (bits & EB_COLLISION) { ctx->err = "64-bit key hash collision (retry with another seed)"; return CC_E_COLLISION; }
    if (bits & EB_KEYERROR) { ctx->err = "KeyError: read_dict[tag] already deleted (consensus_helper.py:490 with overlapping bed regions, or DCS_maker.py:258 with duplex keys that are not mutual)"; return CC_E_KEYERROR; }
    if (bits & EB_N_HIGHQ) { ctx->err = "IndexError: N base with quality >= 30 in a family of size >= 2 (SSCS_maker.py:129)"; return CC_E_N_HIGHQ; }
    if (bits & EB_SHORT) { ctx->err = "IndexError: read shorter than the consensus length"; return CC_E_SHORT_READ; }
    if (bits & EB_BAD_BASE) { ctx->err = "ValueError: base outside ACGTN in a voted family (SSCS_maker.py:122)"; return CC_E_BAD_BASE; }
    if (bits & EB_NO_QUAL) { ctx->err = "TypeError: read without base qualities in a vote"; return CC_E_NO_QUAL; }
    if (bits & EB_NO_CIGAR) { ctx->err = "TypeError: infer_query_length() is None (no cigar)"; return CC_E_NO_CIGAR; }
    if (bits & EB_RG) { ctx->err = "RG tag of a non-string type"; return CC_E_UNSUPPORTED; }
    if (bits & EB_THR) { ctx->err = "cutoff table too short"; return CC_E_INVALID; }
    if (bits & EB_CHAIN) { ctx->err = "a chain of duplex partners longer than the engine follows"; return CC_E_UNSUPPORTED; }
    if (bits & EB_SCANWAIT) { ctx->err = "scan look-back wait bound exceeded"; return CC_E_SCANWAIT; }
    if (bits & EB_TOO_LONG) { ctx->err = "record too long for the 16-bit length fields or payload > 64 GiB"; return CC_E_UNSUPPORTED; }
    if (bits & EB_GUARD) { ctx->err = "a guarded index was outside its array (no load was made from it)"; return CC_E_INVALID; }
    ctx->err = "unknown device error";
    return CC_E_INVALID;
}

int finish_stage(cc_ctx* ctx, Group& g, int64_t* n_out, int64_t n) {
    uint32_t bits = 0;
    bool plan_ok = true;
    RC(finish_pass(ctx, g, &bits, false, &plan_ok));
    if (!plan_ok) return CC_E_PLAN;
    if (n_out) *n_out = n;
    return err_code(ctx, bits);
}
// ... 107 lines not shown
    const int32_t fpw = 64 / chunks;
    klaunch(ctx, mode ? "k_duplex_vote_sc" : "k_duplex_vote_dcs", k_duplex_vote_swar, nblk((n + fpw - 1) / fpw, 4), 256,
            n, mode, fpw, chunks, vpair, TA, TB, qstride, cons_seq, cons_qual, vmeta, ctx->d_err);
}

struct DuplexBufs {
    int32_t *d_swap, *dec, *t_rec, *p_rec;
    uint8_t* fl;
};
template <B FL>
int duplex_head(cc_ctx* ctx, Group& g, const int32_t* bc_swap, int32_t n_bc, int64_t Q, DuplexBufs* d) {
    int brc = 0;
    g.Q = Q;
    HIPCHK(hipMemsetAsync(ctx->d_err, 0, 4, ctx->stream));
    d->d_swap = GB(bc_swap, std::max(n_bc, 1));
    RC(upload_swap(ctx, g, d->d_swap, bc_swap, n_bc));
    d->dec = GB(dec, Q);
    d->t_rec = GB(t_rec, Q);
    d->p_rec = GB(p_rec, Q);
    d->fl = gbuf<FL>(ctx, g, (Q + 15) & ~15LL, &brc);
    return brc;
}
int duplex_tail(cc_ctx* ctx, Group& g, const DuplexBufs& d, int64_t Q, PT id, int32_t mode, const DevTable& TA,
                const DevTable& TB) {
    int brc = 0;
    int64_t NV = 0;
    int32_t* vslot = GB(vslot, Q);
    int4* vpair = GB(vpair, Q);
    RC(scan_emit(ctx, g, d.fl, Q, &NV, id, EmitVotePairs{d.t_rec, d.p_rec, d.dec, vslot, vpair}));
    g.NV = NV;
    const int32_t ml = std::max(TA.max_len, TB.max_len);
    const int32_t qstride = (int32_t)((ml + 15) & ~15);
    uint8_t* cons_seq = GB(cons_seq, NV * (qstride / 2));
    uint8_t* cons_qual = GB(cons_qual, NV * qstride);
    int32_t* vmeta = GB(vote_meta, 5 * NV);
    duplex_vote(ctx, mode, NV, vpair, TA, TB, ml, qstride, cons_seq, cons_qual, vmeta);
    return 0;
}

}

#include "bgzf_crc32.hip.inc"
#include "bgzf_deflate.hip.inc"
#include "bgzf_inflate.hip.inc"

extern "C" {

int cc_create(int device_id, cc_ctx** out) {
    if (!out) return CC_E_INVALID;
    std::unique_ptr<cc_ctx> c(new cc_ctx());
    cc_ctx* ctx = c.get();
    ctx->device = device_id;
    HIPCHK(hipSetDevice(device_id));
    HIPCHK(hipStreamCreateWithFlags(&ctx->stream, hipStreamNonBlocking));
    HIPCHK(hipMalloc((void**)&ctx->d_err, 64));
    HIPCHK(hipMalloc((void**)&ctx->d_cnt, sizeof(unsigned long long) * CC_NUM_COUNTERS * CNT_STRIPES));
    HIPCHK(hipHostMalloc(&ctx->h_pinned, 1024 + sizeof(unsigned long long) * CC_NUM_COUNTERS * CNT_STRIPES));
    if (const char* sm = getenv("CC_SCAN_SPIN_MAX")) ctx->scan_spin_max = (uint32_t)strtoul(sm, nullptr, 10);
    *out = c.release();
    return 0;
}

int cc_destroy(cc_ctx* ctx) {
    if (!ctx) return CC_E_INVALID;
    (void)hipSetDevice(ctx->device);
    (void)hipStreamSynchronize(ctx->stream);
    bgzf_free(ctx);
    for (auto& g : ctx->groups)
        for (DevBuf& b : g.second->buf)
            if (b.p) (void)hipFree(b.p);
    for (auto& t : ctx->table_allocs)
        for (void* p : t.second) (void)hipFree(p);
    if (ctx->scratch)
        for (DevBuf& b : ctx->scratch->buf)
            if (b.p) (void)hipFree(b.p);
    if (ctx->tmp.p) (void)hipFree(ctx->tmp.p);
    if (ctx->sort_buf.p) (void)hipFree(ctx->sort_buf.p);
    if (ctx->scan_st) (void)hipFree(ctx->scan_st);
    if (ctx->names_buf) (void)hipFree(ctx->names_buf);
    if (ctx->names_off) (void)hipFree(ctx->names_off);
    for (auto& s : ctx->name_sets) {
        if (s.second.blob) (void)hipFree(s.second.blob);
        if (s.second.off) (void)hipFree(s.second.off);
    }
    flush_prof(ctx);
    for (hipEvent_t e : ctx->event_pool) (void)hipEventDestroy(e);
    (void)hipFree(ctx->d_err);
    (void)hipFree(ctx->d_cnt);
    (void)hipHostFree(ctx->h_pinned);
    if (ctx->h_defer) (void)hipHostFree(ctx->h_defer);
    (void)hipStreamDestroy(ctx->stream);
    delete ctx;
    return 0;
}

const char* cc_last_error(cc_ctx* ctx) { return ctx ? ctx->err.c_str() : "null context"; }

void* cc_host_alloc(cc_ctx* ctx, uint64_t bytes) {
    void* p = nullptr;
    if (hipHostMalloc(&p, bytes ? bytes : 1) != hipSuccess) {
        if (ctx) ctx->err = "hipHostMalloc failed";
        return nullptr;
    }
    return p;
}
void cc_host_free(cc_ctx*, void* p) {
    if (p) (void)hipHostFree(p);
}

int cc_set_profiling(cc_ctx* ctx, int on) {
    if (!ctx) return CC_E_INVALID;
    flush_prof(ctx);
    ctx->profiling = on != 0;
    if (on) ctx->prof.clear();
    if (on) bgzf_prof(ctx, true, nullptr, nullptr);
    if (on) bgzf_dec_prof(ctx, true, nullptr, nullptr, nullptr, nullptr);
    if (on) bgzf_crc_prof(ctx, true, nullptr, nullptr);
    if (on) bgzf_idx_prof(ctx, true, nullptr, nullptr);
    return 0;
}

int cc_profile_only(cc_ctx* ctx, const char* names) {
    if (!ctx) return CC_E_INVALID;
    ctx->prof_only.clear();
    if (!names) return 0;
    std::string all(names), cur;
    for (char c : all) {
        if (c == '\n') { if (!cur.empty()) ctx->prof_only.insert(cur); cur.clear(); }
        else cur.push_back(c);
    }
    if (!cur.empty()) ctx->prof_only.insert(cur);
    return 0;
}

int cc_kernel_times(cc_ctx* ctx, char* names, int names_cap, double* ms, int64_t* launches, int cap) {
    if (!ctx) return CC_E_INVALID;
    flush_prof(ctx);
    {
        double bms = 0, up = 0, down = 0;
        int64_t bn = 0, un = 0;
        bgzf_prof(ctx, false, &bms, &bn, &up, &down, &un);
        if (bn) {
            ctx->prof["bgzf_deflate"] = {bms, bn};
            ctx->prof["bgzf_upload"] = {up, un};
// ... 1 lines not shown
        }
    }
    {
        double ims = 0, up = 0, down = 0;
        int64_t in = 0;
        bgzf_dec_prof(ctx, false, &ims, &in, &up, &down);
        if (in) {
            ctx->prof["bgzf_inflate"] = {ims, in};
            ctx->prof["bgzf_in_upload"] = {up, in};
            ctx->prof["bgzf_in_download"] = {down, in};
        }
    }
    {
        double cms = 0;
        int64_t cn = 0;
        bgzf_crc_prof(ctx, false, &cms, &cn);
        if (cn) ctx->prof["bgzf_crc32"] = {cms, cn};
    }
    {
        double xms = 0, pms = 0;
        int64_t xn = 0, pn = 0;
        bgzf_idx_prof(ctx, false, &xms, &xn, &pms, &pn);
        if (xn) ctx->prof["index_fields"] = {xms, xn};
        if (pn) ctx->prof["resident_put"] = {pms, pn};
    }
    int i = 0;
    std::string all;
    for (auto& p : ctx->prof) {
        if (i < cap) {
            if (ms) ms[i] = p.second.ms;
            if (launches) launches[i] = p.second.n;
        }
        all += p.first;
        all.push_back('\n');
        ++i;
    }
    if (names && names_cap > 0) snprintf(names, names_cap, "%s", all.c_str());
    return i;
}

int cc_defer(cc_ctx* ctx, int on) {
    if (!ctx) return CC_E_INVALID;
    if (!ctx->h_defer && on) {
        HIPCHK(hipHostMalloc((void**)&ctx->h_defer, (size_t)DEFER_SLOTS * DEFER_SLOT_BYTES));
        HIPCHK(hipHostGetDevicePointer((void**)&ctx->d_defer, ctx->h_defer, 0));
    }
    ctx->defer = on != 0;
    return 0;
}

int cc_commit(cc_ctx* ctx) {
    if (!ctx) return CC_E_INVALID;
    if (ctx->deferred.empty()) return 0;
    HIPCHK(stream_wait(ctx));
    if (const int rc = dbg_fault(ctx)) { ctx->deferred.clear(); return rc; }
    bool ok = true;
    for (const DeferredCheck& d : ctx->deferred) {
        if (!ctx->groups.count(d.gid) || ctx->groups[d.gid].get() != d.g) continue;
        Group& g = *d.g;
        const uint8_t* h = ctx->h_defer + (size_t)d.slot * DEFER_SLOT_BYTES;
        if (*(const uint32_t*)h != 0) ok = false;
        for (const auto& e : d.expect)
            if ((int64_t)((const uint32_t*)(h + 256))[e.first] != e.second) ok = false;
        if (d.counters) {
            for (int i = 0; i < CC_NUM_COUNTERS; ++i) {
                if (i == CC_CNT_COUNTER || i == CC_CNT_PAIRS || i == CC_CNT_READ_ENDS || i == CC_CNT_FAMILIES ||
                    i == CC_CNT_ENTRIES || i == CC_CNT_DROPPED)
                    continue;
                g.counters[i] = (int64_t)((const unsigned long long*)(h + 1024))[i];
            }
            g.counters[CC_CNT_COUNTER] = g.S - g.counters[CC_CNT_FOREIGN] - g.counters[CC_CNT_UNMAPPED];
        }
        if (!d.counters && d.bad_listed != (g.counters[CC_CNT_BAD_LISTED] > 0)) ok = false;
    }
    ctx->deferred.clear();
    if (!ok) {
        ctx->err = "a deferred pass did not hold its plan or met an error: replay the calls with deferral off";
        return CC_E_REPLAY;
    }
    return 0;
}

int cc_debug_poison(cc_ctx* ctx, int32_t group_id, const char* name, int64_t bytes, int32_t value) {
    if (!ctx || !name || !ctx->groups.count(group_id) || bytes < 0) return CC_E_INVALID;
    RC(enter(ctx));
    Group& g = *ctx->groups[group_id];
    const int id = name_id(BUF_IDS, name);
    if (id < 0 || !g.buf[id].p) { ctx->err = std::string("no buffer named ") + name; return CC_E_INVALID; }
    DevBuf& b = g.buf[id];
    int brc = 0;
    void* p = gbuf_bytes(ctx, g, (B)id, std::max((size_t)bytes, b.bytes), &brc);
    if (brc) return brc;
    HIPCHK(hipMemsetAsync(p, value & 0xff, b.bytes, ctx->stream));
    HIPCHK(hipStreamSynchronize(ctx->stream));
    return 0;
}

int cc_debug_skew_plan(cc_ctx* ctx, int32_t group_id, const char* name, int64_t delta) {
    if (!ctx || !name || !ctx->groups.count(group_id)) return CC_E_INVALID;
    Group& g = *ctx->groups[group_id];
    const int id = name_id(PLAN_IDS, name);
    if (id < 0 || !g.plan_set[id]) { ctx->err = std::string("no planned total named ") + name; return CC_E_INVALID; }
    g.plan[id] += delta;
    return 0;
}

}
// ... 54 lines not shown
    uint32_t *d_a = nullptr, *d_b = nullptr, *d_tot = nullptr;
    const int64_t b_words = kind == 2 ? n + DBG_TAIL : kind == 3 ? 4 * (n + DBG_TAIL) : 0;
    RC(dbg_input(ctx, bufs, &d_in, in, n * (kind == 0 ? 4 : 1)));
    if (kind == 3) RC(dbg_input(ctx, bufs, &d_aux, aux, 12 * n));
    RC(dbg_words(ctx, bufs, &d_a, n + DBG_TAIL, DBG_CANARY));
    if (b_words) RC(dbg_words(ctx, bufs, &d_b, b_words, DBG_CANARY));
    RC(dbg_words(ctx, bufs, &d_tot, 4, 0u));
    HIPCHK(hipMemsetAsync(ctx->d_err, 0, 4, ctx->stream));
    if (n > 0) {
        if (kind == 0) RC(scan_launch(ctx, (const uint32_t*)d_in , n, d_tot, "debug_scan", ScanStore{d_a}));
        if (kind == 1) RC(scan_launch(ctx, d_in, n, d_tot, "debug_scan", ScanStore{d_a}));
        if (kind == 2)
            RC(scan_launch(ctx, d_in, n, d_tot, "debug_scan", EmitList{(int32_t*)d_a, (int32_t*)d_b}));
        if (kind == 3)
            RC(scan_launch(ctx, d_in, n, d_tot, "debug_scan",
                           EmitVotePairs{d_aux, d_aux + n, d_aux + 2 * n, (int32_t*)d_a, (int4*)d_b}));
    }
    uint32_t* h_tot = (uint32_t*)ctx->h_pinned;
    HIPCHK(hipMemcpyAsync(out_a, d_a, sizeof(uint32_t) * (size_t)(n + DBG_TAIL), hipMemcpyDeviceToHost, ctx->stream));
    if (b_words) HIPCHK(hipMemcpyAsync(out_b, d_b, sizeof(uint32_t) * (size_t)b_words, hipMemcpyDeviceToHost, ctx->stream));
    HIPCHK(hipMemcpyAsync(h_tot, d_tot, 4, hipMemcpyDeviceToHost, ctx->stream));
    RC(dbg_finish(ctx));
    *total = (int64_t)h_tot[0];
    return 0;
}

int cc_debug_sort_pairs(cc_ctx* ctx, int32_t engine, const uint64_t* keys, const uint32_t* vals, int64_t n,
                        uint32_t begin_bit, uint32_t end_bit, uint64_t* out_keys, uint32_t* out_vals) {
    if (!ctx) return CC_E_INVALID;
    if (engine < -1 || engine > 1 || n < 0 || n >= INT32_MAX - DBG_TAIL || begin_bit > end_bit || end_bit > 64 ||
        !out_keys || !out_vals || (n > 0 && (!keys || !vals))) {
        ctx->err = "cc_debug_sort_pairs: engine -1..1, 0 <= n < 2^31 - 65, begin_bit <= end_bit <= 64, and the arrays";
        return CC_E_INVALID;
    }
    RC(enter(ctx));
    DbgSwitches sw{ctx, ctx->sw};
    ctx->sw.scan1 = engine;
    DbgBufs bufs;
    uint64_t *d_k = nullptr, *d_ko = nullptr;
    uint32_t *d_v = nullptr, *d_vo = nullptr;
    RC(dbg_input(ctx, bufs, &d_k, keys, 8 * n));
    RC(dbg_input(ctx, bufs, &d_v, vals, 4 * n));
    RC(dbg_words(ctx, bufs, &d_ko, 2 * (n + DBG_TAIL), DBG_CANARY));
    RC(dbg_words(ctx, bufs, &d_vo, n + DBG_TAIL, DBG_CANARY));
    HIPCHK(hipMemsetAsync(ctx->d_err, 0, 4, ctx->stream));
    RC(sort_pairs(ctx, d_k, d_ko, d_v, d_vo, n, "debug_sort", begin_bit, end_bit));
    HIPCHK(hipMemcpyAsync(out_keys, d_ko, sizeof(uint64_t) * (size_t)(n + DBG_TAIL), hipMemcpyDeviceToHost, ctx->stream));
    HIPCHK(hipMemcpyAsync(out_vals, d_vo, sizeof(uint32_t) * (size_t)(n + DBG_TAIL), hipMemcpyDeviceToHost, ctx->stream));
    return dbg_finish(ctx);
}

int cc_synchronize(cc_ctx* ctx) {
    if (!ctx) return CC_E_INVALID;
    HIPCHK(hipStreamSynchronize(ctx->stream));
    flush_prof(ctx);
    return dbg_fault(ctx);
}

int cc_debug_build(void) {
#ifdef CC_DEBUG_BOUNDS
    return 1;
#else
    return 0;
#endif
}

int64_t cc_launch_count(void) { return g_launches.load(std::memory_order_relaxed); }

int64_t cc_guard_reruns(cc_ctx* ctx) { return ctx ? ctx->guard_reruns : CC_E_INVALID; }

}
namespace {
int derive_table(cc_ctx* ctx, DevTable& T) {
    if (T.n <= 0) return 0;
    HIPCHK(hipMemsetAsync(T.ndeep, 0, 16, ctx->stream));
    klaunch(ctx, "k_derive", k_derive<false>, nblk(T.n, GT), GT, T, T.dlist, T.ndeep, T.n / DEEP_MIN + 2, DeriveCls{});
    HIPCHK(hipGetLastError());
    return 0;
}
int flush_derive(cc_ctx* ctx, int32_t id) {
    auto it = ctx->tables.find(id);
    if (it == ctx->tables.end() || !it->second.derive_pending) return 0;
    it->second.derive_pending = false;
    return derive_table(ctx, it->second);
}
}
extern "C" {

int cc_table_derive(cc_ctx* ctx, int32_t table_id) {
    if (!ctx || !ctx->tables.count(table_id)) return CC_E_INVALID;
    if (ctx->tables[table_id].host_layout) return 0;
    RC(enter(ctx));
    if (ctx->sw.derive_separate) return derive_table(ctx, ctx->tables[table_id]);
    ctx->tables[table_id].derive_pending = true;
    return 0;
}

int cc_table_upload(cc_ctx* ctx, const cc_records* r, int32_t max_len, int32_t* table_id) {
    if (!ctx || !r || !table_id) return CC_E_INVALID;
    RC(enter(ctx));
    int32_t id = ctx->next_id++;
    std::vector<void*>& al = ctx->table_allocs[id];
    DevTable T;
    T.n = r->n;
    T.max_len = max_len;
    RC(upload(ctx, al, &T.tid, r->tid, r->n));
    RC(upload(ctx, al, &T.pos, r->pos, r->n));
    RC(upload(ctx, al, &T.mtid, r->mtid, r->n));
    RC(upload(ctx, al, &T.mpos, r->mpos, r->n));
    RC(upload(ctx, al, &T.tlen, r->tlen, r->n));
    RC(upload(ctx, al, &T.flag, r->flag, r->n));
    RC(upload(ctx, al, &T.mapq, r->mapq, r->n));
    RC(upload(ctx, al, &T.cig, r->cigar_id, r->n));
    RC(upload(ctx, al, &T.qlen, r->qlen, r->n));
    RC(upload(ctx, al, &T.lseq, r->lseq, r->n));
    RC(upload(ctx, al, &T.bc, r->bc_id, r->n));
    RC(upload(ctx, al, &T.rg, r->rg_id, r->n));
    RC(upload(ctx, al, &T.rflags, r->rflags, r->n));
    RC(upload(ctx, al, &T.qn_off, r->qn_off, r->n));
    RC(upload(ctx, al, &T.qn_len, r->qn_len, r->n));
    RC(upload(ctx, al, &T.qn_blob, r->qn_blob, (int64_t)r->qn_blob_bytes + 16));
    HIPCHK(hipMalloc((void**)&T.qn_ol, sizeof(uint64_t) * std::max<int64_t>(r->n, 1)));
    al.push_back(T.qn_ol);
    RC(upload(ctx, al, &T.pay_off, r->pay_off, r->n));
    RC(upload(ctx, al, &T.payload, r->payload, (int64_t)r->payload_bytes + 64));
    T.pay_bytes = r->payload_bytes;
    T.qn_bytes = r->qn_blob_bytes;
    if (!r->rdig) { ctx->err = "cc_records.rdig is required"; return CC_E_INVALID; }
    RC(upload(ctx, al, &T.rdig, r->rdig, r->n));
    T.qdig_mask = ctx->sw.qdig_bits ? (1ULL << ctx->sw.qdig_bits) - 1 : ~0ULL;
    T.host_layout = r->meta && r->rkey && r->core && r->qn_ol && r->qdig && r->rdeep && r->dlist && r->ext &&
                    r->n_deep >= 0 && r->n_deep <= r->n / DEEP_MIN + 2 && T.qdig_mask == ~0ULL;
    if (T.host_layout) {
        RC(upload(ctx, al, &T.core, reinterpret_cast<const RecCore*>(r->core), r->n));
        RC(upload(ctx, al, &T.meta, reinterpret_cast<const uint4*>(r->meta), r->n));
        RC(upload(ctx, al, &T.rkey, r->rkey, r->n));
        RC(upload(ctx, al, &T.qdig, r->qdig, r->n));
        RC(upload(ctx, al, &T.rdeep, r->rdeep, r->n));
        HIPCHK(hipMemcpyAsync(T.qn_ol, r->qn_ol, sizeof(uint64_t) * (size_t)r->n, hipMemcpyHostToDevice, ctx->stream));
        g_launches.fetch_add(1, std::memory_order_relaxed);
        HIPCHK(hipMalloc((void**)&T.dlist, sizeof(int32_t) * (r->n / DEEP_MIN + 2)));
        al.push_back(T.dlist);
        if (r->n_deep > 0)
            HIPCHK(hipMemcpyAsync(T.dlist, r->dlist, sizeof(int32_t) * (size_t)r->n_deep, hipMemcpyHostToDevice,
                                  ctx->stream));
    } else {
        HIPCHK(hipMalloc((void**)&T.core, sizeof(RecCore) * std::max<int64_t>(r->n, 1)));
        al.push_back(T.core);
        HIPCHK(hipMalloc((void**)&T.meta, sizeof(uint4) * std::max<int64_t>(r->n, 1)));
        al.push_back(T.meta);
        HIPCHK(hipMalloc((void**)&T.rkey, sizeof(uint64_t) * std::max<int64_t>(r->n, 1)));
        al.push_back(T.rkey);
        HIPCHK(hipMalloc((void**)&T.qdig, sizeof(uint64_t) * std::max<int64_t>(r->n, 1)));
        al.push_back(T.qdig);
        HIPCHK(hipMalloc((void**)&T.rdeep, std::max<int64_t>(r->n, 1)));
        al.push_back(T.rdeep);
// ... 16 lines not shown
    HIPCHK(hipMalloc((void**)&T.tbase, sizeof(int64_t) * (T.ntid + 1)));
    al.push_back(T.tbase);
    HIPCHK(hipMalloc((void**)&T.geom, 16));
    al.push_back(T.geom);
    HIPCHK(hipMemsetAsync(T.ext, 0, sizeof(int32_t) * std::max(T.ntid, 1), ctx->stream));
    if (T.host_layout) {
        const int32_t ne = std::min(T.ntid, r->n_ext);
        if (ne > 0)
            HIPCHK(hipMemcpyAsync(T.ext, r->ext, sizeof(int32_t) * (size_t)ne, hipMemcpyHostToDevice, ctx->stream));
        HIPCHK(hipMemsetAsync(T.ndeep, 0, 16, ctx->stream));
        const uint32_t nd = (uint32_t)r->n_deep;
        HIPCHK(hipMemcpyAsync(T.ndeep, &nd, 4, hipMemcpyHostToDevice, ctx->stream));
        HIPCHK(hipStreamSynchronize(ctx->stream));
        T.n_deep = r->n_deep;
    } else {
        RC(derive_table(ctx, T));
        if (r->n > 0) {
            uint32_t nd = 0;
            HIPCHK(hipMemcpyAsync(&nd, T.ndeep, 4, hipMemcpyDeviceToHost, ctx->stream));
            HIPCHK(hipStreamSynchronize(ctx->stream));
            T.n_deep = nd;
        }
    }
    HIPCHK(hipStreamSynchronize(ctx->stream));
    if (ctx->sw.trace_upload)
        fprintf(stderr, "[cc] table %d: %lld records, %lld deep groups, %s layout\n", id, (long long)T.n,
                (long long)T.n_deep, T.host_layout ? "decoder" : "device");
    ctx->tables[id] = T;
    *table_id = id;
    return 0;
}

}

#include "table_unpack.hip.inc"
#include "bam_assemble.hip.inc"
#include "name_format.hip.inc"
#include "bam_index.hip.inc"

namespace {
int prep_table(cc_ctx* ctx, const DevTable& T, Fills& fill, int32_t* rec_e) {
    RC(fill.launch());
    if (T.n <= 0) return 0;
    klaunch(ctx, "k_build_meta", k_build_meta, nblk(T.n, BC_T), BC_T, T, rec_e, ctx->d_err, nullptr, nullptr,
            (int64_t)0);
    return 0;
}
}

extern "C" {

int cc_table_free(cc_ctx* ctx, int32_t id) {
    if (!ctx || !ctx->tables.count(id)) return CC_E_INVALID;
    (void)hipStreamSynchronize(ctx->stream);
    for (void* p : ctx->table_allocs[id]) (void)hipFree(p);
    ctx->table_allocs.erase(id);
    ctx->tables.erase(id);
    return 0;
}

int64_t cc_table_fetch(cc_ctx* ctx, int32_t id, const char* name, void* dst, int64_t cap) {
    if (!ctx || !name || !ctx->tables.count(id)) return CC_E_INVALID;
    RC(enter(ctx));
    RC(flush_derive(ctx, id));
    const DevTable& T = ctx->tables[id];
    const std::string nm(name);
    const void* src = nullptr;
    int64_t bytes = 0;
    if (nm == "rkey") { src = T.rkey; bytes = 8 * T.n; }
    else if (nm == "meta") { src = T.meta; bytes = 16 * T.n; }
    else if (nm == "core") { src = T.core; bytes = 32 * T.n; }
    else if (nm == "qn_ol") { src = T.qn_ol; bytes = 8 * T.n; }
    else if (nm == "qdig") { src = T.qdig; bytes = 8 * T.n; }
    else if (nm == "rdeep") { src = T.rdeep; bytes = T.n; }
    else if (nm == "dlist") { src = T.dlist; bytes = 4 * T.n_deep; }
    else if (nm == "ext") { src = T.ext; bytes = 4 * (int64_t)T.ntid; }
    else if (nm == "tid") { src = T.tid; bytes = 4 * T.n; }
    else if (nm == "pos") { src = T.pos; bytes = 4 * T.n; }
    else if (nm == "mtid") { src = T.mtid; bytes = 4 * T.n; }
    else if (nm == "mpos") { src = T.mpos; bytes = 4 * T.n; }
    else if (nm == "tlen") { src = T.tlen; bytes = 4 * T.n; }
    else if (nm == "flag") { src = T.flag; bytes = 2 * T.n; }
    else if (nm == "mapq") { src = T.mapq; bytes = T.n; }
    else if (nm == "cigar_id") { src = T.cig; bytes = 4 * T.n; }
    else if (nm == "qlen") { src = T.qlen; bytes = 4 * T.n; }
    else if (nm == "lseq") { src = T.lseq; bytes = 4 * T.n; }
    else if (nm == "bc_id") { src = T.bc; bytes = 4 * T.n; }
    else if (nm == "rg_id") { src = T.rg; bytes = 4 * T.n; }
    else if (nm == "rflags") { src = T.rflags; bytes = T.n; }
    else if (nm == "qn_off") { src = T.qn_off; bytes = 8 * T.n; }
    else if (nm == "qn_len") { src = T.qn_len; bytes = 2 * T.n; }
    else if (nm == "pay_off") { src = T.pay_off; bytes = 8 * T.n; }
    else if (nm == "rdig") { src = T.rdig; bytes = 8 * T.n; }
    else if (nm == "qn_blob") { src = T.qn_blob; bytes = (int64_t)T.qn_bytes + 16; }
    else if (nm == "payload") { src = T.payload; bytes = (int64_t)T.pay_bytes + 64; }
    else { ctx->err = "no table column " + nm; return CC_E_INVALID; }
    if (!dst) return bytes;
    if (cap < bytes) { ctx->err = "cc_table_fetch: destination too small"; return CC_E_INVALID; }
    if (bytes > 0) HIPCHK(hipMemcpyAsync(dst, src, (size_t)bytes, hipMemcpyDeviceToHost, ctx->stream));
    HIPCHK(hipStreamSynchronize(ctx->stream));
    return bytes;
}

}

namespace {
int vote_families(cc_ctx* ctx, Group& g, const DevTable& T, int64_t NE, uint8_t* needv, uint32_t* vxs,
                  int32_t* emit_fam, int2* emit_span, double cutoff, int64_t* NV_out) {
    int brc = 0;
    int64_t NV = 0;
// ... 612 lines not shown
    ReadBamPass p(ctx, *ctx->groups[gid]);
    RC(p.setup());
    RC(p.filters());
    RC(p.pairing());
    RC(p.pair_keys());
    RC(p.grouping());
    RC(p.families());
    RC(p.csn());
    Group& g = p.g;
    uint32_t bits = 0;
    bool plan_ok = true;
    RC(finish_pass(ctx, g, &bits, true, &plan_ok));
    if (bits & EB_NEEDSORT) return CC_E_NEEDSORT;
    if (bits & EB_DEEPSORT) return CC_E_DEEPSORT;
    if (!plan_ok) return CC_E_PLAN;
    g.counters[CC_CNT_COUNTER] = p.S - g.counters[CC_CNT_FOREIGN] - g.counters[CC_CNT_UNMAPPED];
    g.counters[CC_CNT_PAIRS] = p.P;
    g.counters[CC_CNT_READ_ENDS] = p.R;
    g.counters[CC_CNT_FAMILIES] = p.F;
    g.counters[CC_CNT_ENTRIES] = p.E;
    g.counters[CC_CNT_DROPPED] = p.R - p.V;
    g.members_built = p.members;
    return err_code(ctx, bits);
}

int read_bam_run(cc_ctx* ctx, int32_t gid) {
    Group& g = *ctx->groups[gid];
    auto run = [&]() {
        int rc = run_planned(ctx, g, ST_READ_BAM, [&] { return read_bam_pass(ctx, gid); });
        for (int k = 0; k < 2 && (rc == CC_E_NEEDSORT || rc == CC_E_DEEPSORT); ++k) {
            if (rc == CC_E_NEEDSORT) g.force_sort = true;
            else g.no_deep_fam = true;
            g.planned[ST_READ_BAM] = false;
            rc = run_planned(ctx, g, ST_READ_BAM, [&] { return read_bam_pass(ctx, gid); });
        }
        return rc;
    };
    int rc = run();
    if (rc == CC_E_COLLISION && !ctx->full_qhash.count(g.table)) {
        ctx->full_qhash.insert(g.table);
        g.planned[ST_READ_BAM] = false;
        rc = run();
    }
    return rc;
}

}

extern "C" {

int cc_read_bam(cc_ctx* ctx, int32_t table_id, int64_t S, const int32_t* stream_rec, const int32_t* stream_region,
                int32_t n_regions, const int32_t* region_run, const cc_read_bam_params* prm, int32_t* group_id) {
    if (!ctx || !prm || !group_id || !ctx->tables.count(table_id) || S < 0 || S >= INT32_MAX / 2) return CC_E_INVALID;
    RC(enter(ctx));
    int32_t gid = ctx->next_id++;
    ctx->groups[gid].reset(new Group());
    Group& g = *ctx->groups[gid];
    g.table = table_id;
    g.seed = prm->seed;
    g.scoped = prm->scope_by_run;
    g.delim_filter = prm->delim_filter;
    g.badread = prm->badread_file;
    g.coord_sorted = prm->coord_sorted;
    g.S = S;
    g.n_regions = n_regions;
    g.ident = S == ctx->tables[table_id].n;
    for (int64_t i = 0; g.ident && i < S; ++i) g.ident = stream_rec[i] == (int32_t)i;
    if (!g.ident) {
        std::vector<bool> seen((size_t)ctx->tables[table_id].n, false);
        for (int64_t i = 0; i < S && !g.overlap; ++i) {
            const int32_t r = stream_rec[i];
            if (r < 0 || r >= ctx->tables[table_id].n) continue;
            g.overlap = seen[(size_t)r];
            seen[(size_t)r] = true;
        }
        if (g.overlap) g.coord_sorted = 0;
    }
    int brc = 0;
    int32_t* d_srec = GB(stream_rec, S);
    int32_t* d_sreg = GB(stream_region, S);
    int32_t* d_run = GB(region_run, std::max<int32_t>(n_regions, 1));
    if (S > 0) {
        HIPCHK(hipMemcpyAsync(d_srec, stream_rec, sizeof(int32_t) * S, hipMemcpyHostToDevice, ctx->stream));
        HIPCHK(hipMemcpyAsync(d_sreg, stream_region, sizeof(int32_t) * S, hipMemcpyHostToDevice, ctx->stream));
    }
    if (n_regions > 0)
        HIPCHK(hipMemcpyAsync(d_run, region_run, sizeof(int32_t) * n_regions, hipMemcpyHostToDevice, ctx->stream));
    *group_id = gid;
    return read_bam_run(ctx, gid);
}

int cc_read_bam_rerun(cc_ctx* ctx, int32_t group_id, uint64_t seed) {
    if (!ctx || !ctx->groups.count(group_id)) return CC_E_INVALID;
    RC(enter(ctx));
    ctx->groups[group_id]->seed = seed;
    return read_bam_run(ctx, group_id);
}

int cc_group_counters(cc_ctx* ctx, int32_t group_id, int64_t* counters) {
    if (!ctx || !ctx->groups.count(group_id) || !counters) return CC_E_INVALID;
    memcpy(counters, ctx->groups[group_id]->counters, sizeof(int64_t) * CC_NUM_COUNTERS);
    return 0;
}

int cc_group_free(cc_ctx* ctx, int32_t group_id) {
    if (!ctx || !ctx->groups.count(group_id)) return CC_E_INVALID;
    (void)hipStreamSynchronize(ctx->stream);
    {
        Group* gp = ctx->groups[group_id].get();
        std::vector<DeferredCheck> keep;
        for (auto& d : ctx->deferred)
            if (d.g != gp) keep.push_back(d);
        ctx->deferred.swap(keep);
    }
    for (DevBuf& b : ctx->groups[group_id]->buf)
        if (b.p) (void)hipFree(b.p);
    ctx->groups.erase(group_id);
    return 0;
}

int cc_consensus_maker(cc_ctx* ctx, int32_t group_id, double cutoff, int64_t* n_out) {
    if (!ctx || !ctx->groups.count(group_id)) return CC_E_INVALID;
    RC(enter(ctx));
    Group& g = *ctx->groups[group_id];
    auto pass = [&]() -> int {
        RC(flush_derive(ctx, g.table));
        const DevTable& T = ctx->tables[g.table];
        int brc = 0;
        const int64_t E = g.E, R = g.R;
        if (!g.members_built) {
            uint4* mm = GB(mem_meta, R);
            if (R > 0)
                klaunch(ctx, k_mem_meta, nblk(R), 256, R, g.ptr<B::mem_rec>(), g.ptr<B::mem_valid>(), T, mm);
            g.members_built = true;
        }
        const uint8_t* has2 = g.ptr<B::has2>();
        uint32_t* hx = GB(hx, (E + 3) & ~3LL);
        int64_t E2 = 0;
        RC(scan_total(ctx, g, has2, hx, E, &E2, PT::scan_emit));
        if (!g.csn_fast && g.n_regions > 1 && E > 0) {
            uint64_t* ek = GB(emit_ekey, E);
            uint64_t* sk = GB(emit_skey, E);
            uint32_t* ev = GB(emit_eval, E);
            uint32_t* sv = GB(emit_sval, E);
            klaunch(ctx, k_emit_keys, nblk(E), 256, E, has2, g.ptr<B::ent_f>(), g.ptr<B::fam_region>(), ek, ev);
            RC(sort_pairs(ctx, ek, sk, ev, sv, E, "sort_emit"));
            if (E2 > 0)
                klaunch(ctx, k_emit_rank, nblk(E2), 256, E2, sv, hx);
        }
        const int64_t NE = 2 * E2;
        int32_t* emit_fam = GB(emit_fam, NE);
        int32_t* emit_n = GB(emit_n, NE);
        int32_t* emit_rec = GB(emit_rec, NE);
        int32_t* emit_ckey = GB(emit_ckey, 9 * E2);
        uint8_t* needv = GB(needv, (NE + 15) & ~15LL);
        int2* emit_span = GB(emit_span, NE);
        uint32_t* vxs = GB(vxs, (NE + 3) & ~3LL);
        if (E > 0)
            klaunch(ctx, "k_sscs_emit", k_sscs_emit, nblk(E), 256, E, g.ptr<B::ent_f>(), g.ptr<B::ent_pair>(), has2, hx,
                    g.ptr<B::fam_n>(), g.ptr<B::fam_beg>(), g.ptr<B::fam_end>(), g.ptr<B::mem_rec>(), emit_fam, emit_n,
                    emit_rec, needv, emit_span, pair_view(g), T, emit_ckey);
        int64_t NV = 0;
        RC(vote_families(ctx, g, T, NE, needv, vxs, emit_fam, emit_span, cutoff, &NV));
        const int64_t S = g.S;
        int64_t NB = 0;
        int32_t* bad_rec = GB(bad_rec, S);
        if (g.counters[CC_CNT_BAD_LISTED] > 0)
            RC(scan_emit(ctx, g, g.ptr<B::badflag>(), S, &NB, PT::scan_bad,
                         EmitGather{g.ptr<B::stream_rec>(), bad_rec}));
        bad_rec = GB(bad_rec, NB);
        return finish_stage(ctx, g, n_out, NE);
    };
    return run_planned(ctx, g, ST_SSCS, pass);
}

int cc_duplex_consensus(cc_ctx* ctx, int32_t group_id, const int32_t* bc_swap, int32_t n_bc, int64_t* n_out) {
    if (!ctx || !ctx->groups.count(group_id) || (!bc_swap && n_bc > 0)) return CC_E_INVALID;
    RC(enter(ctx));
    Group& g = *ctx->groups[group_id];
    auto pass = [&]() -> int {
        RC(flush_derive(ctx, g.table));
        const DevTable& T = ctx->tables[g.table];
        int brc = 0;
        const int64_t Q = 2 * g.E;
        DuplexBufs d;
        RC(duplex_head<B::fl_dcs>(ctx, g, bc_swap, n_bc, Q, &d));
        int32_t *const d_swap = d.d_swap, *const dec = d.dec, *const t_rec = d.t_rec, *const p_rec = d.p_rec;
        uint8_t* const fl_dcs = d.fl;
        if (!g.local_groups) RC(build_ht(ctx, g));
        RC(ensure_fam_tags(ctx, g));
        GroupView G = view_of(g);
        if (Q > 0) {
            ProfScope ps(ctx, "k_dcs_decide");
            if (G.local && !ctx->sw.dcs_per_entry)
                klaunch(ctx, k_dcs_decide_fam, (unsigned)((std::max<int64_t>(g.F, Q) + DD_T - 1) / DD_T), DD_T, Q, G,
                        d_swap, n_bc, dec, t_rec, p_rec, fl_dcs, ctx->d_err);
            else
                klaunch(ctx, k_dcs_decide, nblk(Q), 256, Q, G, d_swap, n_bc, dec, t_rec, p_rec, fl_dcs, ctx->d_err);
        }
        if (g.n_regions > 1 && g.F > 0) {
            int32_t* fdel = GB(fam_del, g.F);
            klaunch(ctx, k_dcs_deleted, nblk(g.F), 256, g.F, g.ptr<B::fam_o>(), g.ptr<B::fam_region>(), Q, dec, fdel);
            RC(deleted_late(ctx, g, fdel));
        }
        RC(duplex_tail(ctx, g, d, Q, PT::scan_dcs, 0, T, T));
        return finish_stage(ctx, g, n_out, Q);
    };
    return run_planned(ctx, g, ST_DCS, pass);
}

int cc_singleton_correction(cc_ctx* ctx, int32_t sgroup, int32_t ssgroup, const int32_t* bc_swap, int32_t n_bc,
                            int64_t* n_out) {
    if (!ctx || !ctx->groups.count(sgroup) || !ctx->groups.count(ssgroup) || (!bc_swap && n_bc > 0))
        return CC_E_INVALID;
    RC(enter(ctx));
    Group& g = *ctx->groups[sgroup];
    Group& s = *ctx->groups[ssgroup];
    auto pass = [&]() -> int {
        RC(flush_derive(ctx, g.table));
        RC(flush_derive(ctx, s.table));
        const DevTable& TA = ctx->tables[g.table];
        const DevTable& TB = ctx->tables[s.table];
        int brc = 0;
        const int64_t Q = 2 * g.E;
        DuplexBufs d;
        RC(duplex_head<B::fl_corr>(ctx, g, bc_swap, n_bc, Q, &d));
        int32_t *const d_swap = d.d_swap, *const dec = d.dec, *const t_rec = d.t_rec, *const p_rec = d.p_rec;
        uint8_t* const fl = d.fl;
        const bool deep_g = TA.n_deep > 0, deep_s = TB.n_deep > 0;
        if (!g.local_groups || deep_g) RC(build_ht(ctx, g));
        RC(ensure_fam_tags(ctx, g));
        RC(ensure_fam_tags(ctx, s));
        GroupView G = view_of(g), SV = view_of(s);
        G.use_ht = deep_g ? 1 : 0;
        bool sb = false;
        if (!deep_s) RC(build_fam_buckets(ctx, s, &SV, &sb));
        if (!sb) {
            RC(build_ht(ctx, s));
            SV = view_of(s);
        }
        const bool ov = (g.n_regions > 1 || s.n_regions > 1) && g.F > 0;
        int32_t* gdel = nullptr;
        int32_t* sdel = nullptr;
        if (ov) {
            gdel = GB(fam_del, g.F);
            HIPCHK(hipMemsetAsync(gdel, 0x7f, sizeof(int32_t) * g.F, ctx->stream));
            sdel = gbuf<B::fam_del>(ctx, s, std::max<int64_t>(s.F, 1), &brc);
            if (brc) return brc;
            HIPCHK(hipMemsetAsync(sdel, 0x7f, sizeof(int32_t) * std::max<int64_t>(s.F, 1), ctx->stream));
        }
        if (Q > 0)
            klaunch(ctx, "k_sc_decide", k_sc_decide, nblk(Q), 256, Q, G, SV, g.ptr<B::region_run>(), d_swap, n_bc, dec,
                    t_rec, p_rec, fl, gdel, sdel, ctx->d_err);
        if (ov) {
            RC(deleted_late(ctx, g, gdel));
            if (s.F > 0) RC(deleted_late(ctx, s, sdel));
        }
        RC(duplex_tail(ctx, g, d, Q, PT::scan_sc, 1, TA, TB));
        int32_t* q_pair = GB(q_pair, Q);
        int32_t* q_ckey = GB(q_ckey, 9 * Q);
        if (Q > 0) {
            klaunch(ctx, k_q_pairs, nblk(Q), 256, Q, g.ptr<B::ent_pair>(), q_pair);
            klaunch(ctx, k_ckey_out, nblk(Q), 256, Q, q_pair, pair_view(g), ctx->tables[g.table], q_ckey);
        }
        return finish_stage(ctx, g, n_out, Q);
    };
    return run_planned(ctx, g, ST_SC, pass);
}

int64_t cc_fetch(cc_ctx* ctx, int32_t group_id, const char* name, void* dst, int64_t cap) {
    if (!ctx || !ctx->groups.count(group_id) || !name) return CC_E_INVALID;
    RC(enter(ctx));
    Group& g = *ctx->groups[group_id];
    const int id = name_id(BUF_IDS, name);
    if (id < 0 || !g.buf[id].p) {
        ctx->err = std::string("no result array named ") + name;
        return CC_E_INVALID;
    }
    const DevBuf& b = g.buf[id];
    int64_t bytes = (int64_t)b.used;
    if (!dst) return bytes;
    int64_t nb = std::min(bytes, cap);
    if (nb > 0) {
        HIPCHK(hipMemcpyAsync(dst, b.p, (size_t)nb, hipMemcpyDeviceToHost, ctx->stream));
        HIPCHK(hipStreamSynchronize(ctx->stream));
    }
    return nb;
}


}

namespace {
int function_prep(cc_ctx* ctx, const DevTable& T) {
    if (T.n > 0)
        klaunch(ctx, "k_build_meta", k_build_meta, 1, BC_T, T, nullptr, ctx->d_err, nullptr, nullptr, (int64_t)0);
    return 0;
}

Group& scratch_group(cc_ctx* ctx, int32_t table) {
    if (!ctx->scratch) ctx->scratch.reset(new Group());
    Group& g = *ctx->scratch;
    g.table = table;
    g.fast = false;
    g.verify.clear();
    return g;
}

int copy_rows(cc_ctx* ctx, void* dst, int64_t to, const void* src, int64_t from, int64_t width, int64_t rows) {
    if (rows <= 0 || width <= 0) return 0;
    HIPCHK(hipMemcpy2DAsync(dst, (size_t)to, src, (size_t)from, (size_t)width, (size_t)rows, hipMemcpyDeviceToHost,
                            ctx->stream));
    return 0;
}
}

extern "C" {

int cc_sscs_vote(cc_ctx* ctx, int32_t table_id, const int32_t* member_index, const int64_t* fam_offsets, int64_t nfam,
                 double cutoff, uint8_t* out_seq, uint8_t* out_qual, int32_t* out_meta, int32_t out_stride) {
    if (!ctx || !ctx->tables.count(table_id) || nfam < 0 || (nfam > 0 && (!fam_offsets || !out_seq || !out_qual ||
                                                                         !out_meta)))
        return CC_E_INVALID;
    if (nfam > 0 && fam_offsets[nfam] > 0 && !member_index) return CC_E_INVALID;
    RC(enter(ctx));
    RC(flush_derive(ctx, table_id));
    const DevTable T = ctx->tables[table_id];
    if (out_stride < T.max_len || (out_stride & 1)) {
        ctx->err = "out_stride must be even and at least the table's longest read";
        return CC_E_INVALID;
    }
    const int64_t R = nfam > 0 ? fam_offsets[nfam] : 0;
    if (nfam > 0 && fam_offsets[0] != 0) { ctx->err = "fam_offsets[0] must be 0"; return CC_E_INVALID; }
    if (R > INT32_MAX) { ctx->err = "too many members"; return CC_E_INVALID; }
    std::vector<int32_t> beg(nfam), end(nfam), cnt(nfam), fam(nfam);
    std::vector<int2> span(nfam);
    for (int64_t k = 0; k < nfam; ++k) {
        if (fam_offsets[k + 1] <= fam_offsets[k]) {
            ctx->err = "IndexError: empty family (SSCS_maker.py:107)";
            return CC_E_INVALID;
        }
        beg[k] = (int32_t)fam_offsets[k];
        end[k] = (int32_t)fam_offsets[k + 1];
        cnt[k] = end[k] - beg[k];
        fam[k] = (int32_t)k;
        span[k] = make_int2(beg[k], cnt[k]);
    }
    for (int64_t j = 0; j < R; ++j)
        if (member_index[j] < 0 || member_index[j] >= T.n) { ctx->err = "member index outside the table"; return CC_E_INVALID; }
    Group& g = scratch_group(ctx, table_id);
    int brc = 0;
    int32_t* mem_rec = GB(mem_rec, R);
    uint32_t* mem_valid = GB(mem_valid, R);
    uint4* mem_meta = GB(mem_meta, R);
// ... 810 lines not shown

struct cc_comm {
    void* comm = nullptr;
    int32_t world = 1, rank = 0;
};

extern "C" {

int cc_comm_unique_id(char* id, int32_t cap) {
    Rccl* r = rccl(nullptr);
    if (!r || !id || cap < NCCL_ID_BYTES) return CC_E_INVALID;
    return r->get_id(id) == 0 ? 0 : CC_E_UNSUPPORTED;
}

int cc_comm_init(cc_ctx* ctx, int32_t world, int32_t rank, const char* id, cc_comm** out) {
    if (!ctx || !out || !id || world < 1 || rank < 0 || rank >= world) return CC_E_INVALID;
    Rccl* r = rccl(&ctx->err);
    if (!r) return CC_E_UNSUPPORTED;
    RC(enter(ctx));
    std::unique_ptr<cc_comm> c(new cc_comm());
    c->world = world;
    c->rank = rank;
    NcclId uid;
    memcpy(uid.internal, id, sizeof(uid.internal));
    const int rc = r->init_rank(&c->comm, world, uid, rank);
    if (rc != 0) {
        ctx->err = std::string("ncclCommInitRank: ") + (r->errstr ? r->errstr(rc) : "error");
        return CC_E_UNSUPPORTED;
    }
    *out = c.release();
    return 0;
}

int cc_comm_destroy(cc_comm* comm) {
    if (!comm) return CC_E_INVALID;
    Rccl* r = rccl(nullptr);
    if (r && comm->comm) r->destroy(comm->comm);
    delete comm;
    return 0;
}

int cc_reduce_stats(cc_ctx* ctx, cc_comm* comm, int64_t* counters, int32_t n_counters, int64_t* fam_count,
                    int64_t* fam_first, int32_t fam_len) {
    if (!ctx || n_counters < 0 || fam_len < 0 || (n_counters > 0 && !counters) ||
        (fam_len > 0 && (!fam_count || !fam_first)))
        return CC_E_INVALID;
    if (!comm) return 0;
    Rccl* r = rccl(&ctx->err);
    if (!r) return CC_E_UNSUPPORTED;
    RC(enter(ctx));
    const int64_t nsum = (int64_t)n_counters + fam_len, ntot = nsum + fam_len;
    if (ntot == 0) return 0;
    int brc = 0;
    if (!ctx->scratch) ctx->scratch.reset(new Group());
    Group& g = *ctx->scratch;
    int64_t* d = GB(reduce_buf, ntot);
    std::vector<int64_t> h((size_t)ntot);
    std::copy(counters, counters + n_counters, h.begin());
    if (fam_len) {
        std::copy(fam_count, fam_count + fam_len, h.begin() + n_counters);
        std::copy(fam_first, fam_first + fam_len, h.begin() + nsum);
    }
    HIPCHK(hipMemcpyAsync(d, h.data(), sizeof(int64_t) * ntot, hipMemcpyHostToDevice, ctx->stream));
    int rc = r->group_start();
    if (rc == 0 && nsum > 0) rc = r->allreduce(d, d, (size_t)nsum, NCCL_INT64, NCCL_SUM, comm->comm, ctx->stream);
    if (rc == 0 && fam_len > 0)
        rc = r->allreduce(d + nsum, d + nsum, (size_t)fam_len, NCCL_INT64, NCCL_MIN, comm->comm, ctx->stream);
    const int rc2 = r->group_end();
    if (rc || rc2) {
        ctx->err = std::string("ncclAllReduce: ") + (r->errstr ? r->errstr(rc ? rc : rc2) : "error");
        return CC_E_UNSUPPORTED;
    }
    HIPCHK(hipMemcpyAsync(h.data(), d, sizeof(int64_t) * ntot, hipMemcpyDeviceToHost, ctx->stream));
    HIPCHK(hipStreamSynchronize(ctx->stream));
    std::copy(h.begin(), h.begin() + n_counters, counters);
    if (fam_len) {
        std::copy(h.begin() + n_counters, h.begin() + nsum, fam_count);
        std::copy(h.begin() + nsum, h.end(), fam_first);
    }
    return 0;
}

int cc_allreduce_max(cc_ctx* ctx, cc_comm* comm, int64_t* v, int32_t n) {
    if (!ctx || n < 0 || (n > 0 && !v)) return CC_E_INVALID;
    if (!comm || n == 0) return 0;
    Rccl* r = rccl(&ctx->err);
    if (!r) return CC_E_UNSUPPORTED;
    RC(enter(ctx));
    int brc = 0;
    if (!ctx->scratch) ctx->scratch.reset(new Group());
    Group& g = *ctx->scratch;
    int64_t* d = GB(reduce_max, n);
    HIPCHK(hipMemcpyAsync(d, v, sizeof(int64_t) * n, hipMemcpyHostToDevice, ctx->stream));
    const int rc = r->allreduce(d, d, (size_t)n, NCCL_INT64, NCCL_MAX, comm->comm, ctx->stream);
    if (rc) {
        ctx->err = std::string("ncclAllReduce: ") + (r->errstr ? r->errstr(rc) : "error");
        return CC_E_UNSUPPORTED;
    }
    HIPCHK(hipMemcpyAsync(v, d, sizeof(int64_t) * n, hipMemcpyDeviceToHost, ctx->stream));
    HIPCHK(hipStreamSynchronize(ctx->stream));
    return 0;
}

}
```

### consensuscruncher_amd/csrc/name_format.hip.inc

```
#include "name_core.h"

namespace {

struct NameStatus {
    unsigned long long first_bad;
    unsigned long long total;
    uint32_t guard, tot;
};
static_assert(sizeof(NameStatus) == 24, "status layout");

constexpr int NM_T = 256;
constexpr int NM_LANES = 16;

struct NameTab {
    const uint8_t* blob;
    const uint64_t* qn_off;
    const uint16_t* qn_len;
    uint64_t bytes;
    int64_t n;
};

struct DevNameSrc {
    static __device__ __forceinline__ upk::W16 fetch(const uint8_t* base, uint64_t a, uint32_t valid) {
        return DevFetch::fetch(base, a, valid);
// ... 57 lines not shown
    return *tl <= 255u && *dl <= 255u && !(*ta & 7u) && !(*da & 7u) && *ta <= T.bytes && ((*tl + 7u) & ~7u) <= T.bytes - *ta &&
           *da <= T.bytes && ((*dl + 7u) & ~7u) <= T.bytes - *da;
}

__global__ __launch_bounds__(NM_T) void k_name_sizes_dcs(NameTab T, const int64_t* __restrict__ rec_tag,
                                                         const int64_t* __restrict__ rec_ds, int64_t n,
                                                         uint32_t* __restrict__ len, uint64_t* __restrict__ lay,
                                                         NameStatus* st) {
    const int64_t i = (int64_t)blockIdx.x * NM_T + threadIdx.x;
    unsigned long long bad = ~0ULL;
    uint32_t l = 0;
    if (i < n) {
        uint64_t ta, da;
        uint32_t tl, dl;
        nmc::DcsLay y;
        uint32_t e = nmc::NE_REC;
        if (name_slots(T, rec_tag[i], rec_ds[i], &ta, &tl, &da, &dl)) e = nmc::dcs_layout<DevNameSrc>(T.blob, ta, tl, da, dl, y);
        if (e) bad = ((unsigned long long)i << 8) | e;
        else l = y.len;
        len[i] = l;
        lay[i] = e ? 0ull : nmc::dcs_pack(y);
    }
    name_status(bad, l, st);
}

template <class Out>
__device__ __forceinline__ void name_store(uint8_t* __restrict__ out, uint64_t off, uint32_t len, uint32_t j, Out out16) {
    uint8_t* d = out + off;
    const uint32_t head = min(len, (16u - ((uint32_t)off & 15u)) & 15u);
    const uint32_t lines = (len - head) >> 4, tail_at = head + (lines << 4);
    uint4* dl = reinterpret_cast<uint4*>(d + head);
    const uint32_t steps = 2u + (lines + NM_LANES - 1u) / NM_LANES;
    for (uint32_t s = 0; s < steps; ++s) {
        const bool line = s >= 2u;
        const uint32_t c = (s - 2u) * NM_LANES + j;
        const uint32_t at = line ? head + (c << 4) : (s == 0u ? j : tail_at + j);
        const bool on = line ? c < lines : (s == 0u ? j < head : at < len);
        if (!on) continue;
        const upk::W16 w = out16(at, line ? 16u : 1u);
        if (line) dl[c] = make_uint4(w.w[0], w.w[1], w.w[2], w.w[3]);
        else d[at] = (uint8_t)w.w[0];
    }
}

template <class Src>
__global__ __launch_bounds__(NM_T) void k_name_write_csn(Src src, int64_t n, nmc::Strs bc, nmc::Strs cg,
                                                         const uint32_t* __restrict__ off32, uint64_t total,
                                                         uint8_t* __restrict__ out, int64_t* __restrict__ off64,
                                                         NameStatus* st) {
    const int64_t i = (int64_t)blockIdx.x * (NM_T / NM_LANES) + (threadIdx.x / NM_LANES);
    const uint32_t j = threadIdx.x % NM_LANES;
    if (i >= n) return;
    const int32_t* f = src.fields(i);
    (void)CC_IDX(f[0], bc.n, DS_REC);
    (void)CC_IDX(f[5], cg.n, DS_REC);
    (void)CC_IDX(f[6], cg.n, DS_REC);
    nmc::CsnLay y;
    const uint32_t e = nmc::csn_layout(f, src.suf(i), bc, cg, y);
    const uint64_t off = off32[i];
    if (e || off > total || y.len > total - off) {
        if (j == 0) atomicOr(&st->guard, 1u);
        return;
    }
    if (j == 0) {
        off64[i] = (int64_t)off;
        if (i == n - 1) off64[n] = (int64_t)(off + y.len);
    }
    name_store(out, off, y.len, j, [&](uint32_t at, uint32_t valid) NMC_INL { return nmc::csn_out16<DevNameSrc>(y, bc, cg, at, valid); });
}

__global__ __launch_bounds__(NM_T) void k_name_write_dcs(NameTab T, const int64_t* __restrict__ rec_tag,
                                                         const int64_t* __restrict__ rec_ds, const uint64_t* __restrict__ lay,
                                                         int64_t n, const uint32_t* __restrict__ off32, uint64_t total,
                                                         uint8_t* __restrict__ out, int64_t* __restrict__ off64,
                                                         NameStatus* st) {
    const int64_t i = (int64_t)blockIdx.x * (NM_T / NM_LANES) + (threadIdx.x / NM_LANES);
    const uint32_t j = threadIdx.x % NM_LANES;
    if (i >= n) return;
    const int64_t rt = CC_IDX(rec_tag[i], T.n, DS_REC), rd = CC_IDX(rec_ds[i], T.n, DS_REC);
    uint64_t ta, da;
    uint32_t tl, dl;
    const bool ok = name_slots(T, rt, rd, &ta, &tl, &da, &dl);
    const nmc::DcsLay y = nmc::dcs_unpack(lay[i]);
    const uint64_t off = off32[i];
    if (!ok || off > total || y.len > total - off || y.tb + 1u + y.cl > tl || y.t1 + 1u + y.tfl > tl || y.db > dl ||
        y.d1 + 1u + y.dfl > dl) {
        if (j == 0) atomicOr(&st->guard, 1u);
        return;
    }
    if (j == 0) {
        off64[i] = (int64_t)off;
        if (i == n - 1) off64[n] = (int64_t)(off + y.len);
    }
    name_store(out, off, y.len, j,
               [&](uint32_t at, uint32_t valid) NMC_INL { return nmc::dcs_out16<DevNameSrc>(y, T.blob, ta, da, at, valid); });
}

const char* name_refusal(uint32_t bits) {
    if (bits & nmc::NE_BC) return "field 0 outside the barcode table";
    if (bits & nmc::NE_CG5) return "field 5 outside the cigar table";
    if (bits & nmc::NE_CG6) return "field 6 outside the cigar table";
    if (bits & nmc::NE_STR) return "a string's offsets outside its blob";
    if (bits & nmc::NE_T_NOUS) return "no '_' in the tag name";
    if (bits & nmc::NE_T_NOCOLON) return "no ':' in the tag name";
    if (bits & nmc::NE_D_NOCOLON) return "no ':' in the partner name";
    return "a record index outside the table";
}

std::atomic<int64_t> g_names_next{1};

void names_release(cc_ctx* ctx) {
    if (ctx->names_buf || ctx->names_off) {
        (void)hipStreamSynchronize(ctx->stream);
        if (ctx->names_buf) (void)hipFree(ctx->names_buf);
        if (ctx->names_off) (void)hipFree(ctx->names_off);
    }
    ctx->names_buf = nullptr;
    ctx->names_off = nullptr;
    ctx->names_n = 0;
    ctx->names_total = -1;
}

const NameSet* names_find(cc_ctx* ctx, int64_t id) {
    const auto it = id > 0 ? ctx->name_sets.find(id) : ctx->name_sets.end();
    return it != ctx->name_sets.end() ? &it->second : nullptr;
}

struct NameGuard {
    cc_ctx* ctx;
    std::vector<void*> tmp;
    uint8_t* blob = nullptr;
    int64_t* off = nullptr;
// ... 274 lines not shown
```

### consensuscruncher_amd/csrc/table_unpack.hip.inc

```
#include "unpack_core.h"

namespace {

enum : uint32_t { UE_BAD = 1u, UE_TOO_LONG = 2u, UE_RFLAGS = 4u };
struct UnpackStatus {
    uint32_t err, pad;
    unsigned long long first_bad;
    int32_t max_len, max_tid;
    unsigned long long sum16, sum8;
    uint32_t tot16, tot8;
};
static_assert(sizeof(UnpackStatus) == 48, "status layout");

constexpr int UPK_T = 256;
constexpr int UPK_LANES = 16;

struct DevSrc {
    const uint8_t* base;
    uint64_t off;
    __device__ __forceinline__ upk::W16 fetch(uint64_t a, uint32_t valid) const {
        const uint4* p = reinterpret_cast<const uint4*>(base + (a & ~15ull));
        const uint32_t sh = (uint32_t)a & 15u;
        const uint4 v0 = p[0];
        uint4 v1 = make_uint4(0u, 0u, 0u, 0u);
// ... 104 lines not shown
        T.qn_off[r] = qo;
    }
    const DevSrc s{recs, off};
    const uint32_t np = (uint32_t)(upk::pay_slot(lseq) >> 4);
    uint4* pd = reinterpret_cast<uint4*>(T.payload + po);
    for (uint32_t c = j; c < np; c += UPK_LANES) {
        const upk::W16 w = upk::pay_chunk(s, qual_off, seq_off, lseq, c);
        pd[c] = make_uint4(w.w[0], w.w[1], w.w[2], w.w[3]);
    }
    const uint32_t nq = upk::qn_slot(lqn) >> 3;
    uint2* qd = reinterpret_cast<uint2*>(T.qn_blob + qo);
    for (uint32_t c = j; c < nq; c += UPK_LANES) {
        const upk::W8 w = upk::qn_chunk(s, qn_len, c);
        qd[c] = make_uint2(w.w[0], w.w[1]);
    }
}

struct UnpackGuard {
    cc_ctx* ctx;
    int32_t id;
    std::vector<void*> tmp;
    bool keep = false;
    ~UnpackGuard() {
        (void)hipStreamSynchronize(ctx->stream);
        for (void* p : tmp) (void)hipFree(p);
        if (!keep) {
            for (void* p : ctx->table_allocs[id]) (void)hipFree(p);
            ctx->table_allocs.erase(id);
        }
    }
};

template <class T>
int dev_alloc(cc_ctx* ctx, std::vector<void*>& allocs, T** dst, int64_t count, size_t extra = 0) {
    HIPCHK(hipMalloc((void**)dst, (size_t)std::max<int64_t>(count, 1) * sizeof(T) + extra));
    allocs.push_back(*dst);
    return 0;
}

int table_unpack(cc_ctx* ctx, const uint8_t* recs, const uint8_t* resident, uint64_t shift, uint64_t bytes,
                 const uint64_t* rec_off, int64_t n, const int32_t* cigar_id, const int32_t* bc_id, const int32_t* rg_id,
                 const uint8_t* rflags, int32_t* max_len, int32_t* table_id) {
    if (!ctx || !max_len || !table_id || n < 0) return CC_E_INVALID;
    if (n > 0 && ((!recs && !resident) || !rec_off || !cigar_id || !bc_id || !rg_id || !rflags)) {
        ctx->err = "cc_table_unpack: null argument";
        return CC_E_INVALID;
    }
    if (n > (int64_t)INT32_MAX) { ctx->err = "cc_table_unpack: more than 2^31 - 1 records"; return CC_E_UNSUPPORTED; }
    RC(enter(ctx));
    const int32_t id = ctx->next_id++;
    std::vector<void*>& al = ctx->table_allocs[id];
    UnpackGuard guard{ctx, id};
    DevTable T{};
    T.n = n;
    RC(dev_alloc(ctx, al, &T.tid, n));
    RC(dev_alloc(ctx, al, &T.pos, n));
    RC(dev_alloc(ctx, al, &T.mtid, n));
    RC(dev_alloc(ctx, al, &T.mpos, n));
    RC(dev_alloc(ctx, al, &T.tlen, n));
    RC(dev_alloc(ctx, al, &T.flag, n));
    RC(dev_alloc(ctx, al, &T.mapq, n));
    RC(upload(ctx, al, &T.cig, cigar_id, n));
    RC(dev_alloc(ctx, al, &T.qlen, n));
    RC(dev_alloc(ctx, al, &T.lseq, n));
    RC(upload(ctx, al, &T.bc, bc_id, n));
    RC(upload(ctx, al, &T.rg, rg_id, n));
    RC(dev_alloc(ctx, al, &T.rflags, n));
    RC(dev_alloc(ctx, al, &T.qn_off, n));
    RC(dev_alloc(ctx, al, &T.qn_len, n));
    RC(dev_alloc(ctx, al, &T.qn_ol, n));
    RC(dev_alloc(ctx, al, &T.pay_off, n));
    RC(dev_alloc(ctx, al, &T.rdig, n));
    UnpackStatus* h_st = reinterpret_cast<UnpackStatus*>((uint8_t*)ctx->h_pinned + 768);
    *h_st = UnpackStatus{};
    h_st->first_bad = ~0ULL;
    h_st->max_tid = -1;
    const uint8_t* d_recs = resident;
    uint8_t* d_rf = nullptr;
    uint64_t* d_off = nullptr;
    uint32_t *sz16 = nullptr, *sz8 = nullptr, *off16 = nullptr, *off8 = nullptr;
    if (n > 0) {
        if (!resident) {
            const size_t padded = (size_t)((bytes + 15) & ~15ull) + 32;
            uint8_t* up = nullptr;
            RC(dev_alloc(ctx, guard.tmp, &up, (int64_t)padded));
            ProfScope ps(ctx, "unpack_stream_upload");
            HIPCHK(hipMemcpyAsync(up, recs, (size_t)bytes, hipMemcpyHostToDevice, ctx->stream));
            HIPCHK(hipMemsetAsync(up + bytes, 0, padded - (size_t)bytes, ctx->stream));
            d_recs = up;
        }
        RC(upload(ctx, guard.tmp, &d_off, rec_off, n));
        RC(upload(ctx, guard.tmp, &d_rf, rflags, n));
        RC(dev_alloc(ctx, guard.tmp, &sz16, n, 64));
        RC(dev_alloc(ctx, guard.tmp, &sz8, n, 64));
        RC(dev_alloc(ctx, guard.tmp, &off16, n, 64));
        RC(dev_alloc(ctx, guard.tmp, &off8, n, 64));
        UnpackStatus* d_st = nullptr;
        RC(dev_alloc(ctx, guard.tmp, &d_st, 1));
        HIPCHK(hipMemcpyAsync(d_st, h_st, sizeof(UnpackStatus), hipMemcpyHostToDevice, ctx->stream));
        klaunch(ctx, "k_unpack_sizes", k_unpack_sizes, nblk(n, UPK_T), UPK_T, d_recs, shift, bytes, d_off, n, d_rf, T, sz16,
                sz8, d_st);
        HIPCHK(hipGetLastError());
        RC(scan_launch(ctx, sz16, n, &d_st->tot16, "unpack_scan_pay", ScanStore{off16}));
        RC(scan_launch(ctx, sz8, n, &d_st->tot8, "unpack_scan_qn", ScanStore{off8}));
        HIPCHK(hipGetLastError());
        HIPCHK(hipMemcpyAsync(h_st, d_st, sizeof(UnpackStatus), hipMemcpyDeviceToHost, ctx->stream));
// ... 98 lines not shown
```

### consensuscruncher_amd/native.py

```python
import ctypes as C
import os

import numpy as np

LIBDIR = os.path.join(os.path.dirname(os.path.abspath(__file__)), "lib")

CC_E = {
    -1: "CC_E_INVALID", -2: "CC_E_HIP", -3: "CC_E_N_HIGHQ", -4: "CC_E_BAD_BASE", -5: "CC_E_SHORT_READ",
    -6: "CC_E_NO_QUAL", -7: "CC_E_NO_CIGAR", -8: "CC_E_DUP_QNAME",
    -9: "CC_E_AMBIGUOUS",
    -10: "CC_E_COLLISION", -11: "CC_E_UNSUPPORTED", -12: "CC_E_KEYERROR",
    -13: "CC_E_REPLAY",
}
CC_E_INVALID = -1
CC_E_N_HIGHQ = -3
CC_E_COLLISION = -10
CC_E_UNSUPPORTED = -11
CC_E_KEYERROR = -12
CC_E_REPLAY = -13

CNT = dict(COUNTER=0, UNMAPPED=1, UNMAPPED_MATE=2, MULTIPLE_MAPPING=3, BAD_SPACER=4, PAIRS=5, READ_ENDS=6,
           FAMILIES=7, ENTRIES=8, UNPAIRED=9, ORPHAN_TAGS=10, DROPPED=11, BAD_LISTED=12, FOREIGN=13)
NUM_COUNTERS = 16
REGION_MOVED = 1 << 30
# ... 176 lines not shown
    "cc_synchronize": (C.c_int, [P]),
    "cc_bgzf_deflate": (C.c_int64, [P, P, C.c_uint64, P, C.c_uint64, P, C.c_int64]),
    "cc_bgzf_hook": (C.c_int, [P, C.POINTER(P), C.POINTER(P)]),
    "cc_bgzf_set_effort": (C.c_int, [P, C.c_int]),
    "cc_bgzf_inflate": (C.c_int64, [P, P, P, P, P, P, C.c_int64, P, P]),
    "cc_bgzf_inflate_hook": (C.c_int, [P, C.POINTER(P), C.POINTER(P)]),
    "cc_bgzf_inflate_keep": (C.c_int64, [P, P, P, P, P, P, C.c_int64, P, P, C.c_uint64, i64p]),
    "cc_bgzf_inflate_keep_hook": (C.c_int, [P, C.POINTER(P), C.POINTER(P), C.POINTER(P)]),
    "cc_resident_patch": (C.c_int, [P, C.c_int64, C.c_uint64, P, C.c_uint64]),
    "cc_resident_free": (C.c_int, [P, C.c_int64]),
    "cc_resident_fetch": (C.c_int64, [P, C.c_int64, P, C.c_uint64]),
    "cc_resident_count": (C.c_int64, [P]),
    "cc_crc32": (C.c_int, [P, P, C.c_uint64, P, P, C.c_int64, P]),
    "cc_resident_crc32": (C.c_int, [P, C.c_int64, P, P, C.c_int64, P]),
    "cc_bgzf_inflate_crc": (C.c_int64, [P, P, P, P, P, P, C.c_int64, P, P, P]),
    "cc_bgzf_inflate_keep_crc": (C.c_int64, [P, P, P, P, P, P, C.c_int64, P, P, C.c_uint64, i64p, P]),
    "cc_bgzf_inflate_crc_hook": (C.c_int, [P, C.POINTER(P), C.POINTER(P)]),
    "cc_bgzf_inflate_keep_crc_hook": (C.c_int, [P, C.POINTER(P), C.POINTER(P), C.POINTER(P)]),
    "cc_bgzf_set_crc": (C.c_int, [P, C.c_int]),
    "cc_defer": (C.c_int, [P, C.c_int]),
    "cc_commit": (C.c_int, [P]),
    "cc_debug_skew_plan": (C.c_int, [P, C.c_int32, C.c_char_p, C.c_int64]),
    "cc_debug_build": (C.c_int, []),
    "cc_launch_count": (C.c_int64, []),
    "cc_table_upload": (C.c_int, [P, C.POINTER(cc_records), C.c_int32, i32p]),
    "cc_table_unpack": (C.c_int, [P, P, C.c_uint64, P, C.c_int64, P, P, P, P, i32p, i32p]),
    "cc_table_unpack_resident": (C.c_int, [P, C.c_int64, C.c_uint64, C.c_uint64, P, C.c_int64, P, P, P, P, i32p,
                                           i32p]),
    "cc_bam_assemble": (C.c_int, [P, P, C.c_uint64, C.POINTER(cc_asm_src), C.c_int32, P, C.c_int64, P, P, C.c_int64,
                                  C.c_uint64, P, C.c_uint64, P, C.c_uint64, C.c_int32, P, P, C.c_int32, C.c_int, P,
                                  C.c_uint64, P, C.POINTER(C.c_uint64)]),
    "cc_bam_assemble_hook": (C.c_int, [P, C.POINTER(P), C.POINTER(P)]),
    "cc_bam_assemble_keep": (C.c_int, [P, P, C.c_uint64, C.POINTER(cc_asm_src), C.c_int32, P, C.c_int64, P, P,
                                       C.c_int64, C.c_uint64, P, C.c_uint64, P, C.c_uint64, C.c_int32, P, P, C.c_int32,
                                       C.c_int, P, C.c_uint64, P, C.POINTER(C.c_uint64), i64p]),
    "cc_out_resident_hooks": (C.c_int, [P, C.POINTER(ccio_out_resident), C.POINTER(P)]),
    "cc_bgzf_deflate_resident": (C.c_int64, [P, C.c_int64, C.c_uint64, C.c_uint64, P, C.c_uint64, P, C.c_int64]),
    "cc_index_fields": (C.c_int, [P, C.c_int64, P, C.c_int64, P]),
    "cc_resident_put": (C.c_int, [P, P, C.c_uint64, i64p]),
    "cc_bam_assemble_group": (C.c_int, [P, C.c_int32]),
    "cc_format_csn_names": (C.c_int, [P, C.c_int64, P, P, P, P, C.c_int64, P, P, C.c_int64, P, i64p]),
    "cc_format_dcs_names": (C.c_int, [P, C.c_int32, C.c_int64, P, P, P, i64p]),
    "cc_names_read": (C.c_int, [P, P, C.c_int64]),
    "cc_format_csn_names_group": (C.c_int, [P, C.c_int32, P, P, C.c_int64, P, P, C.c_int64, P, i64p]),
    "cc_names_keep": (C.c_int, [P, i64p]),
    "cc_names_fetch": (C.c_int64, [P, C.c_int64, P, C.c_int64]),
    "cc_names_free": (C.c_int, [P, C.c_int64]),
    "cc_names_count": (C.c_int64, [P]),
    "cc_bam_assemble_names": (C.c_int, [P, C.c_int64]),
    "cc_table_free": (C.c_int, [P, C.c_int32]),
    "cc_table_derive": (C.c_int, [P, C.c_int32]),
    "cc_table_fetch": (C.c_int64, [P, C.c_int32, C.c_char_p, P, C.c_int64]),
    "cc_guard_reruns": (C.c_int64, [P]),
    "cc_debug_poison": (C.c_int, [P, C.c_int32, C.c_char_p, C.c_int64, C.c_int32]),
    "cc_debug_scan": (C.c_int, [P, C.c_int32, C.c_int32, P, C.c_int64, P, P, P, i64p]),
    "cc_debug_sort_pairs": (C.c_int, [P, C.c_int32, P, P, C.c_int64, C.c_uint32, C.c_uint32, P, P]),
    "cc_read_bam": (C.c_int, [P, C.c_int32, C.c_int64, P, P, C.c_int32, P, C.POINTER(cc_read_bam_params), i32p]),
    "cc_read_bam_rerun": (C.c_int, [P, C.c_int32, C.c_uint64]),
    "cc_group_counters": (C.c_int, [P, C.c_int32, P]),
    "cc_group_free": (C.c_int, [P, C.c_int32]),
    "cc_consensus_maker": (C.c_int, [P, C.c_int32, C.c_double, i64p]),
    "cc_duplex_consensus": (C.c_int, [P, C.c_int32, P, C.c_int32, i64p]),
    "cc_singleton_correction": (C.c_int, [P, C.c_int32, C.c_int32, P, C.c_int32, i64p]),
    "cc_fetch": (C.c_int64, [P, C.c_int32, C.c_char_p, P, C.c_int64]),
    "cc_sscs_vote": (C.c_int, [P, C.c_int32, P, P, C.c_int64, C.c_double, P, P, P, C.c_int32]),
    "cc_pair_vote": (C.c_int, [P, C.c_int32, C.c_int32, C.c_int32, P, P, C.c_int64, P, P, P, C.c_int32]),
    "cc_group": (C.c_int, [P, C.c_int64, P, C.c_int32, P, P, i64p]),
    "cc_duplex_join": (C.c_int, [P, C.c_int32, C.c_int64, P, P, C.c_int64, P, C.c_int32, P, P, C.c_int32, P,
                                 C.c_int32, P, P, P, P, C.c_int32]),
    "cc_extract_barcodes": (C.c_int, [P, C.c_int64, P, P, P, P, C.c_char_p, P, C.c_int32, P, P, P, P, P, P, P, P, P]),
    "cc_comm_unique_id": (C.c_int, [C.c_char_p, C.c_int32]),
    "cc_comm_init": (C.c_int, [P, C.c_int32, C.c_int32, C.c_char_p, C.POINTER(P)]),
    "cc_comm_destroy": (C.c_int, [P]),
    "cc_reduce_stats": (C.c_int, [P, P, P, C.c_int32, P, P, C.c_int32]),
    "cc_allreduce_max": (C.c_int, [P, P, P, C.c_int32]),
}


def _bind(lib, sigs):
    for name, (res, args) in sigs.items():
        fn = getattr(lib, name)
        fn.restype = res
        fn.argtypes = args
    return lib


def io():
    global _io
    if _io is None:
        path = os.path.join(LIBDIR, "libccio.so")
        if not os.path.exists(path):
            raise ImportError("libccio.so not built; run __graft_entry__.build()")
        _io = _bind(C.CDLL(path), IO_SIGS)
    return _io


def amd_path():
    return os.environ.get("CCAMD_LIB") or os.path.join(LIBDIR, "libccamd.so")


def lib_sha(path=None):
    import hashlib
    h = hashlib.sha256()
    with open(path or amd_path(), "rb") as f:
        for blk in iter(lambda: f.read(1 << 20), b""):
            h.update(blk)
# ... 20 lines not shown
```

### include/consensuscruncher_amd.h

```cpp
#ifndef CONSENSUSCRUNCHER_AMD_H
#define CONSENSUSCRUNCHER_AMD_H

#include <stdint.h>

#ifdef __cplusplus
extern "C" {
#endif

#define CC_OK 0
#define CC_E_INVALID -1
#define CC_E_HIP -2
#define CC_E_N_HIGHQ -3
#define CC_E_BAD_BASE -4
#define CC_E_SHORT_READ -5
#define CC_E_NO_QUAL -6
#define CC_E_NO_CIGAR -7
#define CC_E_DUP_QNAME -8
#define CC_E_AMBIGUOUS -9
#define CC_E_COLLISION -10
#define CC_E_UNSUPPORTED -11
#define CC_E_KEYERROR -12
#define CC_E_REPLAY -13

#define CC_RF_BAD_SPACER 1u
// ... 220 lines not shown
    int32_t badread_file;
    int32_t scope_by_run;
    int32_t coord_sorted;
    uint64_t seed;
} cc_read_bam_params;

int cc_create(int device_id, cc_ctx **ctx);
int cc_destroy(cc_ctx *ctx);
const char *cc_last_error(cc_ctx *ctx);
void *cc_host_alloc(cc_ctx *ctx, uint64_t bytes);
void cc_host_free(cc_ctx *ctx, void *p);
int cc_set_profiling(cc_ctx *ctx, int on);
int cc_profile_only(cc_ctx *ctx, const char *names);
int cc_kernel_times(cc_ctx *ctx, char *names, int names_cap, double *ms, int64_t *launches, int cap);
int cc_synchronize(cc_ctx *ctx);
int64_t cc_bgzf_deflate(cc_ctx *ctx, const uint8_t *data, uint64_t n, uint8_t *stage, uint64_t slot,
                        uint32_t *out_len, int64_t cap);
int cc_bgzf_hook(cc_ctx *ctx, ccio_deflate_fn *fn, void **user);
int cc_bgzf_set_effort(cc_ctx *ctx, int effort);
int64_t cc_bgzf_inflate(cc_ctx *ctx, const uint8_t *comp, const uint64_t *coff, const uint32_t *clen,
                        const uint64_t *uoff, const uint32_t *ulen, int64_t members, uint8_t *out, uint8_t *ok);
int cc_bgzf_inflate_hook(cc_ctx *ctx, ccio_inflate_fn *fn, void **user);
int64_t cc_bgzf_inflate_keep(cc_ctx *ctx, const uint8_t *comp, const uint64_t *coff, const uint32_t *clen,
                             const uint64_t *uoff, const uint32_t *ulen, int64_t members, uint8_t *out, uint8_t *ok,
                             uint64_t total, int64_t *resident_id);
int cc_bgzf_inflate_keep_hook(cc_ctx *ctx, ccio_inflate_keep_fn *keep, ccio_resident_patch_fn *patch, void **user);
int cc_resident_patch(cc_ctx *ctx, int64_t id, uint64_t off, const uint8_t *bytes, uint64_t n);
int cc_resident_free(cc_ctx *ctx, int64_t id);
int64_t cc_resident_fetch(cc_ctx *ctx, int64_t id, uint8_t *dst, uint64_t cap);
int64_t cc_resident_count(cc_ctx *ctx);
int cc_resident_put(cc_ctx *ctx, const uint8_t *bytes, uint64_t n, int64_t *id);
int64_t cc_bgzf_deflate_resident(cc_ctx *ctx, int64_t id, uint64_t off, uint64_t n, uint8_t *stage, uint64_t slot,
                                 uint32_t *out_len, int64_t cap);
int cc_index_fields(cc_ctx *ctx, int64_t id, const uint64_t *at, int64_t n, cc_index_field *fields);
int cc_crc32(cc_ctx *ctx, const uint8_t *data, uint64_t nbytes, const uint64_t *off, const uint64_t *len, int64_t n,
             uint32_t *crc);
int cc_resident_crc32(cc_ctx *ctx, int64_t id, const uint64_t *off, const uint64_t *len, int64_t n, uint32_t *crc);
int64_t cc_bgzf_inflate_crc(cc_ctx *ctx, const uint8_t *comp, const uint64_t *coff, const uint32_t *clen,
                            const uint64_t *uoff, const uint32_t *ulen, int64_t members, uint8_t *out, uint8_t *ok,
                            uint32_t *crc);
int64_t cc_bgzf_inflate_keep_crc(cc_ctx *ctx, const uint8_t *comp, const uint64_t *coff, const uint32_t *clen,
                                 const uint64_t *uoff, const uint32_t *ulen, int64_t members, uint8_t *out, uint8_t *ok,
                                 uint64_t total, int64_t *resident_id, uint32_t *crc);
int cc_bgzf_inflate_crc_hook(cc_ctx *ctx, ccio_inflate_crc_fn *fn, void **user);
int cc_bgzf_inflate_keep_crc_hook(cc_ctx *ctx, ccio_inflate_keep_crc_fn *keep, ccio_resident_patch_fn *patch,
                                  void **user);
int cc_bgzf_set_crc(cc_ctx *ctx, int on);
int cc_defer(cc_ctx *ctx, int on);
int cc_commit(cc_ctx *ctx);
int cc_debug_skew_plan(cc_ctx *ctx, int32_t group_id, const char *name, int64_t delta);
int cc_debug_build(void);
int64_t cc_launch_count(void);
int64_t cc_guard_reruns(cc_ctx *ctx);
int cc_debug_poison(cc_ctx *ctx, int32_t group_id, const char *name, int64_t bytes, int32_t value);
int cc_debug_scan(cc_ctx *ctx, int32_t kind, int32_t engine, const void *in, int64_t n, const int32_t *aux,
                  void *out_a, void *out_b, int64_t *total);
int cc_debug_sort_pairs(cc_ctx *ctx, int32_t engine, const uint64_t *keys, const uint32_t *vals, int64_t n,
                        uint32_t begin_bit, uint32_t end_bit, uint64_t *out_keys, uint32_t *out_vals);

int cc_table_upload(cc_ctx *ctx, const cc_records *rec, int32_t max_len, int32_t *table_id);
int cc_table_unpack(cc_ctx *ctx, const uint8_t *recs, uint64_t bytes, const uint64_t *rec_off, int64_t n,
                    const int32_t *cigar_id, const int32_t *bc_id, const int32_t *rg_id, const uint8_t *rflags,
                    int32_t *max_len, int32_t *table_id);
int cc_bam_assemble(cc_ctx *ctx, const uint8_t *header, uint64_t header_bytes, const cc_asm_src *srcs, int32_t nsrc,
                    const cc_out_spec *spec, int64_t n, const char *names, const int64_t *name_off, int64_t n_names,
                    uint64_t names_bytes, const uint8_t *cons_seq, uint64_t cons_seq_bytes, const uint8_t *cons_qual,
                    uint64_t cons_qual_bytes, int32_t cons_group, const char *rg_blob, const int64_t *rg_off,
                    int32_t n_rg, int flags, uint8_t *out, uint64_t cap, uint64_t *at, uint64_t *total);
int cc_bam_assemble_hook(cc_ctx *ctx, ccio_assemble_fn *fn, void **user);
int cc_bam_assemble_keep(cc_ctx *ctx, const uint8_t *header, uint64_t header_bytes, const cc_asm_src *srcs,
                         int32_t nsrc, const cc_out_spec *spec, int64_t n, const char *names, const int64_t *name_off,
                         int64_t n_names, uint64_t names_bytes, const uint8_t *cons_seq, uint64_t cons_seq_bytes,
                         const uint8_t *cons_qual, uint64_t cons_qual_bytes, int32_t cons_group, const char *rg_blob,
                         const int64_t *rg_off, int32_t n_rg, int flags, uint8_t *out, uint64_t cap, uint64_t *at,
                         uint64_t *total, int64_t *resident_id);
int cc_out_resident_hooks(cc_ctx *ctx, ccio_out_resident *cb, void **user);
int cc_bam_assemble_group(cc_ctx *ctx, int32_t group_id);
int cc_bam_assemble_names(cc_ctx *ctx, int64_t names_id);
int cc_format_csn_names(cc_ctx *ctx, int64_t n, const int32_t *f9, const int64_t *suffix, const char *bc_blob,
                        const int64_t *bc_off, int64_t n_bc, const char *cg_blob, const int64_t *cg_off, int64_t n_cg,
                        int64_t *off, int64_t *total);
int cc_format_dcs_names(cc_ctx *ctx, int32_t table, int64_t n, const int64_t *rec_tag, const int64_t *rec_ds,
                        int64_t *off, int64_t *total);
int cc_names_read(cc_ctx *ctx, char *blob, int64_t cap);
int cc_format_csn_names_group(cc_ctx *ctx, int32_t group_id, const char *bc_blob, const int64_t *bc_off, int64_t n_bc,
                              const char *cg_blob, const int64_t *cg_off, int64_t n_cg, int64_t *off, int64_t *total);
int cc_names_keep(cc_ctx *ctx, int64_t *names_id);
int64_t cc_names_fetch(cc_ctx *ctx, int64_t names_id, char *blob, int64_t cap);
int cc_names_free(cc_ctx *ctx, int64_t names_id);
int64_t cc_names_count(cc_ctx *ctx);
int cc_table_unpack_resident(cc_ctx *ctx, int64_t id, uint64_t base, uint64_t bytes, const uint64_t *rec_off,
                             int64_t n, const int32_t *cigar_id, const int32_t *bc_id, const int32_t *rg_id,
                             const uint8_t *rflags, int32_t *max_len, int32_t *table_id);
int cc_table_free(cc_ctx *ctx, int32_t table_id);
int cc_table_derive(cc_ctx *ctx, int32_t table_id);
int64_t cc_table_fetch(cc_ctx *ctx, int32_t table_id, const char *name, void *dst, int64_t cap);

#define CC_REGION_MOVED (1 << 30)
int cc_read_bam(cc_ctx *ctx, int32_t table_id, int64_t n_stream, const int32_t *stream_rec,
                const int32_t *stream_region, int32_t n_regions, const int32_t *region_run,
                const cc_read_bam_params *params, int32_t *group_id);
int cc_group_counters(cc_ctx *ctx, int32_t group_id, int64_t *counters );
int cc_group_free(cc_ctx *ctx, int32_t group_id);

int cc_consensus_maker(cc_ctx *ctx, int32_t group_id, double cutoff, int64_t *n_out);
int cc_read_bam_rerun(cc_ctx *ctx, int32_t group_id, uint64_t seed);
// ... 40 lines not shown
```

Measured before the change: 2.977 billion.

## Run consensus groups on multiple HIP stream lanes with per-group error state

```diff
diff --git a/consensuscruncher_amd/csrc/bam_assemble.hip.inc b/consensuscruncher_amd/csrc/bam_assemble.hip.inc
--- a/consensuscruncher_amd/csrc/bam_assemble.hip.inc
+++ b/consensuscruncher_amd/csrc/bam_assemble.hip.inc
@@ -58,11 +58,12 @@
 }
 
 __global__ __launch_bounds__(ASM_T) void k_asm_gather(const uint32_t* __restrict__ sz, const uint32_t* __restrict__ perm,
-                                                      int64_t n, int64_t o0, int64_t cnt, uint32_t* __restrict__ ssz) {
+                                                      int64_t n, int64_t o0, int64_t cnt, uint32_t* __restrict__ ssz,
+                                                      AsmStatus* st) {
     const int64_t i = (int64_t)blockIdx.x * ASM_T + threadIdx.x;
     if (i >= cnt) return;
     const int64_t s = perm ? (int64_t)perm[o0 + i] : o0 + i;
-    ssz[i] = sz[CC_IDX(s, n, DS_REC)];
+    ssz[i] = sz[CC_IDXG(s, n, DS_REC, &st->guard)];
 }
 
 __global__ __launch_bounds__(ASM_T) void k_asm_copy(asmb::Tables T, const asmb::Spec* __restrict__ spec,
@@ -76,7 +77,7 @@
     const int64_t s = perm ? (int64_t)perm[o] : o;
     asmb::Lay y;
     uint64_t k;
-    const uint32_t e = asmb::layout(spec[CC_IDX(s, n, DS_REC)], T, y, &k);
+    const uint32_t e = asmb::layout(spec[CC_IDXG(s, n, DS_REC, &st->guard)], T, y, &k);
     const uint64_t off = base + off32[i];
     if (e || off > total || y.size > total - off || (uint64_t)s >= (uint64_t)n) {
         if (j == 0) atomicOr(&st->guard, 1u);
@@ -298,7 +299,7 @@
     uint64_t base = a.header_bytes;
     for (int64_t o0 = 0; o0 < n; o0 += per) {
         const int64_t cnt = std::min(per, n - o0);
-        klaunch(ctx, "k_asm_gather", k_asm_gather, nblk(cnt, ASM_T), ASM_T, sz, perm, n, o0, cnt, ssz);
+        klaunch(ctx, "k_asm_gather", k_asm_gather, nblk(cnt, ASM_T), ASM_T, sz, perm, n, o0, cnt, ssz, d_st);
         RC(scan_launch(ctx, ssz, cnt, &d_st->tot, "asm_scan", ScanStore{off32}));
         klaunch(ctx, "k_asm_copy", k_asm_copy, nblk(cnt, ASM_T / ASM_LANES), ASM_T, T, d_spec, perm, n, o0, cnt, off32, base, sum,
                 d_out, d_at, d_st);
diff --git a/consensuscruncher_amd/csrc/cc_engine.hip b/consensuscruncher_amd/csrc/cc_engine.hip
--- a/consensuscruncher_amd/csrc/cc_engine.hip
+++ b/consensuscruncher_amd/csrc/cc_engine.hip
@@ -47,9 +47,10 @@
     EB_GUARD = 1u << 17,
 };
 
-__device__ unsigned int g_guard;
-__device__ __noinline__ int64_t guard_fail() {
-    atomicOr(&g_guard, 1u);
+constexpr int ERR_WORDS = 16, ERR_GUARD = 15;
+
+__device__ __noinline__ int64_t guard_fail(unsigned int* guard) {
+    if (guard) atomicOr(guard, 1u);
     return 0;
 }
 #ifdef CC_DEBUG_BOUNDS
@@ -61,15 +62,16 @@
 __device__ __forceinline__ int64_t dbg_idx(int64_t i, int64_t n, int site) {
     return (i < 0 || i >= n) ? dbg_fail(site, i) : i;
 }
-#define CC_IDX(i, n, site) ((std::remove_cv_t<std::remove_reference_t<decltype(i)>>)dbg_idx((int64_t)(i), (int64_t)(n), (site)))
+#define CC_IDXG(i, n, site, guard) ((std::remove_cv_t<std::remove_reference_t<decltype(i)>>)dbg_idx((int64_t)(i), (int64_t)(n), (site)))
 #elif defined(CC_NO_GUARD)
-#define CC_IDX(i, n, site) (i)
+#define CC_IDXG(i, n, site, guard) (i)
 #else
-__device__ __forceinline__ int64_t guard_idx(int64_t i, int64_t n) {
-    return (uint64_t)i < (uint64_t)n ? i : guard_fail();
-}
-#define CC_IDX(i, n, site) ((std::remove_cv_t<std::remove_reference_t<decltype(i)>>)guard_idx((int64_t)(i), (int64_t)(n)))
+__device__ __forceinline__ int64_t guard_idx(int64_t i, int64_t n, unsigned int* guard) {
+    return (uint64_t)i < (uint64_t)n ? i : guard_fail(guard);
+}
+#define CC_IDXG(i, n, site, guard) ((std::remove_cv_t<std::remove_reference_t<decltype(i)>>)guard_idx((int64_t)(i), (int64_t)(n), (guard)))
 #endif
+#define CC_IDX(i, n, site) CC_IDXG(i, n, site, T.guard)
 enum : int {
     DS_REC = 1, DS_QNAME = 2, DS_PAYLOAD = 3, DS_SLOT = 4, DS_PAIR = 5, DS_MEMBER = 6, DS_VOTE_REC = 7,
 };
@@ -110,6 +112,7 @@
     uint4* meta;
     uint64_t* rkey;
     uint32_t* ebits;
+    uint32_t* guard;
     uint8_t* rdeep;
     int32_t* dlist;
     uint32_t* ndeep;
@@ -2369,7 +2372,7 @@
         fam_o[f] = 0x7f7f7f7f;
         int32_t b = CC_IDX(fam_beg[f], R, DS_SLOT);
         int32_t e = (f + 1 < F) ? fam_beg[f + 1] : (int32_t)R;
-        if (e < b || e > R) e = b + (int32_t)guard_fail() + 1;
+        if (e < b || e > R) e = b + (int32_t)guard_fail(T.guard) + 1;
         fam_end[f] = e;
         fam_n[f] = e - b - fam_drop[f];
         uint32_t fe = rs_val[b];
@@ -3011,14 +3014,14 @@
         const int32_t f = emit_fam[o];
         int2 sp = emit_span[o];
         const bool over = need && (int64_t)vxo >= nvcap;
-        if (over) guard_fail();
+        if (over) guard_fail(T.guard);
         if (!need || over) {
             emit_vslot[o] = -1;
         } else {
             const int32_t v = (int32_t)vxo;
             vote_fam[v] = f;
             emit_vslot[o] = v;
-            if (sp.x < 0 || sp.y < 0 || (int64_t)sp.x + sp.y > nmem) sp = make_int2((int32_t)guard_fail(), 0);
+            if (sp.x < 0 || sp.y < 0 || (int64_t)sp.x + sp.y > nmem) sp = make_int2((int32_t)guard_fail(T.guard), 0);
             const int32_t beg = sp.x, cnt = sp.y;
             const uint4* fm = mem_meta + beg;
             const uint4 m0 = cnt > 0 ? fm[0] : make_uint4(0u, 0u, 0u, 0u);
@@ -3105,7 +3108,7 @@
     if (key >= 0) {
         const int64_t at = s_vb + atomicAdd(&s_cur[key], 1u);
         if (at < nvcap) vote_order[at] = rec;
-        else guard_fail();
+        else guard_fail(T.guard);
     }
 }
 
@@ -3217,7 +3220,7 @@
         const int4 vi = vote_order[t];
         beg = vi.x; cnt = vi.y; L = vi.z; v = vi.w;
         if (beg < 0 || cnt < 0 || (int64_t)beg + cnt > nmem || v < 0 || v >= nv) {
-            beg = (int32_t)guard_fail();
+            beg = (int32_t)guard_fail(T.guard);
             cnt = 0;
         }
     }
@@ -3897,11 +3900,11 @@
     uint32_t eb = 0;
     if (g < fpw && w < nv) {
         const int4 vp = vpair[w];
-        const int32_t a = CC_IDX(vp.x, TA.n, DS_VOTE_REC), b = vp.y;
+        const int32_t a = CC_IDXG(vp.x, TA.n, DS_VOTE_REC, TA.guard), b = vp.y;
         const bool b_in_a = sc && vp.z == 1;
         const DevTable& TBx = b_in_a ? TA : TB;
         const uint8_t* bpay = TBx.payload;
-        const uint4 ma = TA.meta[a], mb = TBx.meta[CC_IDX(b, TBx.n, DS_VOTE_REC)];
+        const uint4 ma = TA.meta[a], mb = TBx.meta[CC_IDXG(b, TBx.n, DS_VOTE_REC, TA.guard)];
         const int32_t la = (int32_t)(ma.z & 0xffffu), lb = (int32_t)(mb.z & 0xffffu);
         int32_t L = la;
         if (lb < L) { eb |= EB_SHORT; L = 0; }
@@ -4454,9 +4457,9 @@
 }
 
 __global__ __launch_bounds__(64) void k_guard_fold(uint32_t* __restrict__ err) {
-    if (threadIdx.x == 0 && g_guard) {
+    if (threadIdx.x == 0 && err[ERR_GUARD]) {
         atomicOr(err, EB_GUARD);
-        g_guard = 0u;
+        err[ERR_GUARD] = 0u;
     }
 }
 __global__ __launch_bounds__(256) void k_defer_pack(const uint32_t* __restrict__ err,
@@ -4465,8 +4468,9 @@
                                                     const uint32_t* __restrict__ stripes, uint8_t* __restrict__ h) {
     const int t = threadIdx.x;
     if (t == 0) {
-        *reinterpret_cast<uint32_t*>(h) = *err | (g_guard ? EB_GUARD : 0u);
-        if (g_guard) g_guard = 0u;
+        uint32_t* guard = const_cast<uint32_t*>(err) + ERR_GUARD;
+        *reinterpret_cast<uint32_t*>(h) = *err | (*guard ? EB_GUARD : 0u);
+        if (*guard) *guard = 0u;
     }
     if (cnt && t < CC_NUM_COUNTERS) {
         unsigned long long v = 0;
@@ -4633,11 +4637,24 @@
 constexpr int PLAN_SLOTS = 64;
 static_assert((int)PT::COUNT <= PLAN_SLOTS, "a planned total's slot is its id");
 
+struct Touch {
+    hipEvent_t ev = nullptr;
+    int lane = -1;
+};
+constexpr int CC_MAX_LANES = 4;
+
 enum Stage { ST_READ_BAM, ST_SSCS, ST_DCS, ST_SC, ST_COUNT };
 constexpr const char* STAGE_NAME[ST_COUNT] = {"read_bam", "sscs", "dcs", "sc"};
 
 struct Group {
     int32_t table = -1;
+    int lane = 0;
+    Touch touch;
+    uint32_t* d_err = nullptr;
+    unsigned long long* d_cnt = nullptr;
+    int64_t reruns = 0;
+    int64_t guard_reruns = 0;
+    int64_t lane_waits = 0;
     int64_t S = 0, P = 0, R = 0, F = 0, E = 0, Q = 0, NV = 0;
     uint64_t seed = 0;
     int scoped = 0, delim_filter = 0, badread = 0;
@@ -4711,6 +4728,7 @@
     bool gr_by_pair = false;
     bool deep_sort = false;
     bool trace_upload = false;
+    int lanes = CC_MAX_LANES;
 };
 
 EngineSwitches read_switches() {
@@ -4730,6 +4748,7 @@
     sw.gr_by_pair = getenv("CC_GR_BY_PAIR") != nullptr;
     sw.deep_sort = getenv("CC_DEEP_SORT") != nullptr;
     sw.trace_upload = getenv("CC_TRACE_UPLOAD") != nullptr;
+    if (const char* v = getenv("CC_LANES")) sw.lanes = std::min(std::max(atoi(v), 1), CC_MAX_LANES);
     return sw;
 }
 
@@ -4743,21 +4762,34 @@
     int64_t n = 0, total = 0;
 };
 
+struct Lane {
+    hipStream_t stream = nullptr;
+    DevBuf tmp;
+    DevBuf sort_buf;
+    unsigned long long* scan_st = nullptr;
+    uint32_t* scan_ticket = nullptr;
+    int64_t scan_cap = 0;
+    uint32_t scan_epoch = 0;
+    void* h_pinned = nullptr;
+};
+
 struct cc_ctx {
     int device = 0;
+    Lane lanes[CC_MAX_LANES];
+    Lane* lane = nullptr;
     hipStream_t stream = nullptr;
+    int n_lanes = 1;
+    int next_lane = 0;
+    bool loose = false;
+    hipEvent_t loose_ev = nullptr;
+    bool loose_wait[CC_MAX_LANES] = {false, false, false, false};
+    std::map<int32_t, Touch> table_touch;
     std::string err;
     EngineSwitches sw;
     std::map<int32_t, DevTable> tables;
     std::map<int32_t, std::vector<void*>> table_allocs;
     std::map<int32_t, std::unique_ptr<Group>> groups;
     int32_t next_id = 1;
-    DevBuf tmp;
-    DevBuf sort_buf;
-    unsigned long long* scan_st = nullptr;
-    uint32_t* scan_ticket = nullptr;
-    int64_t scan_cap = 0;
-    uint32_t scan_epoch = 0;
     uint32_t scan_spin_max = 1u << 22;
     bool scan_two = false;
     std::unordered_set<int32_t> full_qhash;
@@ -4805,10 +4837,107 @@
         if (rc_) return rc_;      \
     } while (0)
 
+int wait_lanes(cc_ctx* ctx) {
+    for (Lane& l : ctx->lanes) HIPCHK(hipStreamSynchronize(l.stream));
+    return 0;
+}
+int lanes_in_use(cc_ctx* ctx) {
+    const int n = ctx->profiling && ctx->prof_only.empty() ? 1 : ctx->sw.lanes;
+    if (n != ctx->n_lanes) {
+        RC(wait_lanes(ctx));
+        ctx->n_lanes = n;
+    }
+    return 0;
+}
+void bind(cc_ctx* ctx, int lane, Group& g) {
+    ctx->lane = &ctx->lanes[lane];
+    ctx->stream = ctx->lane->stream;
+    ctx->h_pinned = ctx->lane->h_pinned;
+    ctx->d_err = g.d_err;
+    ctx->d_cnt = g.d_cnt;
+    for (auto& t : ctx->tables) t.second.guard = g.d_err + ERR_GUARD;
+}
 int enter(cc_ctx* ctx) {
     HIPCHK(hipSetDevice(ctx->device));
     ctx->sw = read_switches();
+    RC(lanes_in_use(ctx));
+    if (ctx->n_lanes > 1) RC(wait_lanes(ctx));
+    bind(ctx, 0, *ctx->scratch);
+    ctx->loose = true;
     return 0;
+}
+
+struct PassScope {
+    cc_ctx* ctx = nullptr;
+    int lane = 0;
+    Touch* t[4] = {nullptr, nullptr, nullptr, nullptr};
+    ~PassScope() {
+        if (!ctx || ctx->n_lanes <= 1) return;
+        for (Touch* x : t) {
+            if (!x) continue;
+            if (!x->ev && hipEventCreateWithFlags(&x->ev, hipEventDisableTiming) != hipSuccess) {
+                (void)hipStreamSynchronize(ctx->lanes[lane].stream);
+                x->ev = nullptr;
+                x->lane = -1;
+                continue;
+            }
+            (void)hipEventRecord(x->ev, ctx->lanes[lane].stream);
+            x->lane = lane;
+        }
+    }
+};
+int pass_enter(cc_ctx* ctx, PassScope& ps, Group& g, Group* other) {
+    HIPCHK(hipSetDevice(ctx->device));
+    ctx->sw = read_switches();
+    RC(lanes_in_use(ctx));
+    const int lane = g.lane % ctx->n_lanes;
+    if (ctx->loose && ctx->n_lanes > 1) {
+        if (!ctx->loose_ev) HIPCHK(hipEventCreateWithFlags(&ctx->loose_ev, hipEventDisableTiming));
+        HIPCHK(hipEventRecord(ctx->loose_ev, ctx->lanes[0].stream));
+        for (int l = 1; l < CC_MAX_LANES; ++l) ctx->loose_wait[l] = true;
+    }
+    ctx->loose = false;
+    bind(ctx, lane, g);
+    if (ctx->loose_wait[lane]) {
+        HIPCHK(hipStreamWaitEvent(ctx->stream, ctx->loose_ev, 0));
+        ctx->loose_wait[lane] = false;
+    }
+    ps.ctx = ctx;
+    ps.lane = lane;
+    ps.t[0] = &g.touch;
+    ps.t[1] = &ctx->table_touch[g.table];
+    if (other && other != &g) {
+        ps.t[2] = &other->touch;
+        if (other->table != g.table) ps.t[3] = &ctx->table_touch[other->table];
+    }
+    for (Touch* x : ps.t)
+        if (x && x->ev && x->lane >= 0 && x->lane != lane) {
+            HIPCHK(hipStreamWaitEvent(ctx->stream, x->ev, 0));
+            ++g.lane_waits;
+        }
+    return 0;
+}
+
+Group* new_group(cc_ctx* ctx) {
+    std::unique_ptr<Group> g(new Group());
+    const size_t cb = sizeof(unsigned long long) * CC_NUM_COUNTERS * CNT_STRIPES;
+    if (hipMalloc((void**)&g->d_err, sizeof(uint32_t) * ERR_WORDS) != hipSuccess ||
+        hipMalloc((void**)&g->d_cnt, cb) != hipSuccess ||
+        hipMemset(g->d_err, 0, sizeof(uint32_t) * ERR_WORDS) != hipSuccess || hipMemset(g->d_cnt, 0, cb) != hipSuccess) {
+        if (g->d_err) (void)hipFree(g->d_err);
+        if (g->d_cnt) (void)hipFree(g->d_cnt);
+        ctx->err = "hipMalloc failed for a group's error block";
+        return nullptr;
+    }
+    g->lane = ctx->next_lane++ % CC_MAX_LANES;
+    return g.release();
+}
+void free_group(Group& g) {
+    for (DevBuf& b : g.buf)
+        if (b.p) (void)hipFree(b.p);
+    if (g.d_err) (void)hipFree(g.d_err);
+    if (g.d_cnt) (void)hipFree(g.d_cnt);
+    if (g.touch.ev) (void)hipEventDestroy(g.touch.ev);
 }
 
 inline unsigned nblk(int64_t n, int b = 256) { return (unsigned)((n + b - 1) / b); }
@@ -4867,19 +4996,19 @@
 }
 
 void* tmp_storage(cc_ctx* ctx, size_t bytes, int* rc) {
-    if (ctx->tmp.bytes < bytes) {
-        if (ctx->tmp.p) (void)hipFree(ctx->tmp.p);
-        ctx->tmp.p = nullptr;
+    if (ctx->lane->tmp.bytes < bytes) {
+        if (ctx->lane->tmp.p) (void)hipFree(ctx->lane->tmp.p);
+        ctx->lane->tmp.p = nullptr;
         size_t nb = bytes + bytes / 4 + 4096;
-        if (hipMalloc(&ctx->tmp.p, nb) != hipSuccess) {
+        if (hipMalloc(&ctx->lane->tmp.p, nb) != hipSuccess) {
             ctx->err = "hipMalloc temp storage failed";
             *rc = CC_E_HIP;
-            ctx->tmp.bytes = 0;
+            ctx->lane->tmp.bytes = 0;
             return nullptr;
         }
-        ctx->tmp.bytes = nb;
-    }
-    return ctx->tmp.p;
+        ctx->lane->tmp.bytes = nb;
+    }
+    return ctx->lane->tmp.p;
 }
 
 struct ProfScope {
@@ -4920,7 +5049,7 @@
 
 void flush_prof(cc_ctx* ctx) {
     if (ctx->pending.empty()) return;
-    (void)hipStreamSynchronize(ctx->stream);
+    (void)wait_lanes(ctx);
     for (auto& p : ctx->pending) {
         float ms = 0;
         (void)hipEventElapsedTime(&ms, p.second.first, p.second.second);
@@ -4943,18 +5072,18 @@
     const int passes = end_bit > begin_bit ? (int)((end_bit - begin_bit + 7) / 8) : 0;
     const int64_t nt = (n + RS_TILE - 1) / RS_TILE;
     const size_t need = (size_t)n * 12 + 2 * sizeof(uint32_t) * (size_t)RS_BINS * (size_t)nt + 256;
-    if (ctx->sort_buf.bytes < need) {
-        if (ctx->sort_buf.p) {
+    if (ctx->lane->sort_buf.bytes < need) {
+        if (ctx->lane->sort_buf.p) {
             HIPCHK(hipStreamSynchronize(ctx->stream));
-            (void)hipFree(ctx->sort_buf.p);
-        }
-        ctx->sort_buf.p = nullptr;
-        ctx->sort_buf.bytes = 0;
+            (void)hipFree(ctx->lane->sort_buf.p);
+        }
+        ctx->lane->sort_buf.p = nullptr;
+        ctx->lane->sort_buf.bytes = 0;
         const size_t nb = need + need / 4;
-        HIPCHK(hipMalloc(&ctx->sort_buf.p, nb));
-        ctx->sort_buf.bytes = nb;
-    }
-    uint8_t* sb = (uint8_t*)ctx->sort_buf.p;
+        HIPCHK(hipMalloc(&ctx->lane->sort_buf.p, nb));
+        ctx->lane->sort_buf.bytes = nb;
+    }
+    uint8_t* sb = (uint8_t*)ctx->lane->sort_buf.p;
     uint64_t* tk = (uint64_t*)sb;
     uint32_t* tv = (uint32_t*)(sb + (size_t)n * 8);
     uint32_t* hist = (uint32_t*)(sb + (((size_t)n * 12 + 127) & ~(size_t)127));
@@ -4990,25 +5119,25 @@
     if (al & 15u) { ctx->err = "scan operands must be 16-B aligned"; return CC_E_INVALID; }
     const bool one = !ctx->scan_two && (ctx->sw.scan1 >= 0 ? ctx->sw.scan1 == 1 : nb <= SCAN_ONE_MAX);
     if (one && nb > 0) {
-        if (nb > ctx->scan_cap) {
+        if (nb > ctx->lane->scan_cap) {
             const int64_t cap = std::max<int64_t>(nb, 1 << 14);
-            if (ctx->scan_st) {
+            if (ctx->lane->scan_st) {
                 HIPCHK(hipStreamSynchronize(ctx->stream));
-                (void)hipFree(ctx->scan_st);
+                (void)hipFree(ctx->lane->scan_st);
             }
-            ctx->scan_st = nullptr;
-            ctx->scan_cap = 0;
-            HIPCHK(hipMalloc((void**)&ctx->scan_st, sizeof(unsigned long long) * cap + 64));
-            HIPCHK(hipMemsetAsync(ctx->scan_st, 0, sizeof(unsigned long long) * cap + 64, ctx->stream));
-            ctx->scan_ticket = reinterpret_cast<uint32_t*>(ctx->scan_st + cap);
-            ctx->scan_cap = cap;
-            ctx->scan_epoch = 0;
-        }
-        if (++ctx->scan_epoch >= (1u << 30)) {
-            HIPCHK(hipMemsetAsync(ctx->scan_st, 0, sizeof(unsigned long long) * ctx->scan_cap, ctx->stream));
-            ctx->scan_epoch = 1;
-        }
-        const ScanLB lb{ctx->scan_st, ctx->scan_ticket, ctx->scan_epoch, ctx->d_err, ctx->scan_spin_max};
+            ctx->lane->scan_st = nullptr;
+            ctx->lane->scan_cap = 0;
+            HIPCHK(hipMalloc((void**)&ctx->lane->scan_st, sizeof(unsigned long long) * cap + 64));
+            HIPCHK(hipMemsetAsync(ctx->lane->scan_st, 0, sizeof(unsigned long long) * cap + 64, ctx->stream));
+            ctx->lane->scan_ticket = reinterpret_cast<uint32_t*>(ctx->lane->scan_st + cap);
+            ctx->lane->scan_cap = cap;
+            ctx->lane->scan_epoch = 0;
+        }
+        if (++ctx->lane->scan_epoch >= (1u << 30)) {
+            HIPCHK(hipMemsetAsync(ctx->lane->scan_st, 0, sizeof(unsigned long long) * ctx->lane->scan_cap, ctx->stream));
+            ctx->lane->scan_epoch = 1;
+        }
+        const ScanLB lb{ctx->lane->scan_st, ctx->lane->scan_ticket, ctx->lane->scan_epoch, ctx->d_err, ctx->scan_spin_max};
         klaunch(ctx, name, k_scan_one<Emit, TIn>, (unsigned)nb, SCAN_T, in, n, nb, d_tot, em, lb);
         return 0;
     }
@@ -5151,7 +5280,10 @@
     HIPCHK(stream_wait(ctx));
     RC(dbg_fault(ctx));
     *bits = *(uint32_t*)(h + 16);
-    if ((*bits & EB_GUARD) && g.fast) ++ctx->guard_reruns;
+    if ((*bits & EB_GUARD) && g.fast) {
+        ++ctx->guard_reruns;
+        ++g.guard_reruns;
+    }
     const bool cap_over = (*bits & EB_PLAN) != 0 || (g.fast && (*bits & EB_GUARD) != 0);
     *bits &= g.fast ? ~(EB_PLAN | EB_GUARD) : ~EB_PLAN;
     if (counters)
@@ -5177,6 +5309,7 @@
         g.fast = false;
     }
     if (rc == CC_E_PLAN) {
+        if (g.planned[stage]) ++g.reruns;
         g.verify.clear();
         rc = pass();
     }
@@ -5390,10 +5523,15 @@
     cc_ctx* ctx = c.get();
     ctx->device = device_id;
     HIPCHK(hipSetDevice(device_id));
-    HIPCHK(hipStreamCreateWithFlags(&ctx->stream, hipStreamNonBlocking));
-    HIPCHK(hipMalloc((void**)&ctx->d_err, 64));
-    HIPCHK(hipMalloc((void**)&ctx->d_cnt, sizeof(unsigned long long) * CC_NUM_COUNTERS * CNT_STRIPES));
-    HIPCHK(hipHostMalloc(&ctx->h_pinned, 1024 + sizeof(unsigned long long) * CC_NUM_COUNTERS * CNT_STRIPES));
+    for (Lane& l : ctx->lanes) {
+        HIPCHK(hipStreamCreateWithFlags(&l.stream, hipStreamNonBlocking));
+        HIPCHK(hipHostMalloc(&l.h_pinned, 1024 + sizeof(unsigned long long) * CC_NUM_COUNTERS * CNT_STRIPES));
+    }
+    ctx->scratch.reset(new_group(ctx));
+    if (!ctx->scratch) return CC_E_HIP;
+    ctx->next_lane = 0;
+    ctx->scratch->lane = 0;
+    bind(ctx, 0, *ctx->scratch);
     if (const char* sm = getenv("CC_SCAN_SPIN_MAX")) ctx->scan_spin_max = (uint32_t)strtoul(sm, nullptr, 10);
     *out = c.release();
     return 0;
@@ -5402,19 +5540,14 @@
 int cc_destroy(cc_ctx* ctx) {
     if (!ctx) return CC_E_INVALID;
     (void)hipSetDevice(ctx->device);
-    (void)hipStreamSynchronize(ctx->stream);
+    (void)wait_lanes(ctx);
     bgzf_free(ctx);
-    for (auto& g : ctx->groups)
-        for (DevBuf& b : g.second->buf)
-            if (b.p) (void)hipFree(b.p);
+    for (auto& g : ctx->groups) free_group(*g.second);
     for (auto& t : ctx->table_allocs)
         for (void* p : t.second) (void)hipFree(p);
-    if (ctx->scratch)
-        for (DevBuf& b : ctx->scratch->buf)
-            if (b.p) (void)hipFree(b.p);
-    if (ctx->tmp.p) (void)hipFree(ctx->tmp.p);
-    if (ctx->sort_buf.p) (void)hipFree(ctx->sort_buf.p);
-    if (ctx->scan_st) (void)hipFree(ctx->scan_st);
+    for (auto& t : ctx->table_touch)
+        if (t.second.ev) (void)hipEventDestroy(t.second.ev);
+    if (ctx->scratch) free_group(*ctx->scratch);
     if (ctx->names_buf) (void)hipFree(ctx->names_buf);
     if (ctx->names_off) (void)hipFree(ctx->names_off);
     for (auto& s : ctx->name_sets) {
@@ -5423,11 +5556,15 @@
     }
     flush_prof(ctx);
     for (hipEvent_t e : ctx->event_pool) (void)hipEventDestroy(e);
-    (void)hipFree(ctx->d_err);
-    (void)hipFree(ctx->d_cnt);
-    (void)hipHostFree(ctx->h_pinned);
     if (ctx->h_defer) (void)hipHostFree(ctx->h_defer);
-    (void)hipStreamDestroy(ctx->stream);
+    if (ctx->loose_ev) (void)hipEventDestroy(ctx->loose_ev);
+    for (Lane& l : ctx->lanes) {
+        if (l.tmp.p) (void)hipFree(l.tmp.p);
+        if (l.sort_buf.p) (void)hipFree(l.sort_buf.p);
+        if (l.scan_st) (void)hipFree(l.scan_st);
+        if (l.h_pinned) (void)hipHostFree(l.h_pinned);
+        if (l.stream) (void)hipStreamDestroy(l.stream);
+    }
     delete ctx;
     return 0;
 }
@@ -5535,7 +5672,11 @@
 int cc_commit(cc_ctx* ctx) {
     if (!ctx) return CC_E_INVALID;
     if (ctx->deferred.empty()) return 0;
-    HIPCHK(stream_wait(ctx));
+    for (Lane& l : ctx->lanes) {
+        ctx->stream = l.stream;
+        HIPCHK(stream_wait(ctx));
+    }
+    ctx->stream = ctx->lane->stream;
     if (const int rc = dbg_fault(ctx)) { ctx->deferred.clear(); return rc; }
     bool ok = true;
     for (const DeferredCheck& d : ctx->deferred) {
@@ -5696,7 +5837,7 @@
 
 int cc_synchronize(cc_ctx* ctx) {
     if (!ctx) return CC_E_INVALID;
-    HIPCHK(hipStreamSynchronize(ctx->stream));
+    RC(wait_lanes(ctx));
     flush_prof(ctx);
     return dbg_fault(ctx);
 }
@@ -5712,6 +5853,15 @@
 int64_t cc_launch_count(void) { return g_launches.load(std::memory_order_relaxed); }
 
 int64_t cc_guard_reruns(cc_ctx* ctx) { return ctx ? ctx->guard_reruns : CC_E_INVALID; }
+
+int cc_group_reruns(cc_ctx* ctx, int32_t group_id, int64_t* out) {
+    if (!ctx || !out || !ctx->groups.count(group_id)) return CC_E_INVALID;
+    const Group& g = *ctx->groups[group_id];
+    out[0] = g.reruns;
+    out[1] = g.guard_reruns;
+    out[2] = g.lane_waits;
+    return 0;
+}
 
 }
 namespace {
@@ -5734,8 +5884,11 @@
 int cc_table_derive(cc_ctx* ctx, int32_t table_id) {
     if (!ctx || !ctx->tables.count(table_id)) return CC_E_INVALID;
     if (ctx->tables[table_id].host_layout) return 0;
-    RC(enter(ctx));
-    if (ctx->sw.derive_separate) return derive_table(ctx, ctx->tables[table_id]);
+    ctx->sw = read_switches();
+    if (ctx->sw.derive_separate) {
+        RC(enter(ctx));
+        return derive_table(ctx, ctx->tables[table_id]);
+    }
     ctx->tables[table_id].derive_pending = true;
     return 0;
 }
@@ -5746,6 +5899,7 @@
     int32_t id = ctx->next_id++;
     std::vector<void*>& al = ctx->table_allocs[id];
     DevTable T;
+    T.guard = ctx->d_err + ERR_GUARD;
     T.n = r->n;
     T.max_len = max_len;
     RC(upload(ctx, al, &T.tid, r->tid, r->n));
@@ -5868,10 +6022,12 @@
 
 int cc_table_free(cc_ctx* ctx, int32_t id) {
     if (!ctx || !ctx->tables.count(id)) return CC_E_INVALID;
-    (void)hipStreamSynchronize(ctx->stream);
+    (void)wait_lanes(ctx);
     for (void* p : ctx->table_allocs[id]) (void)hipFree(p);
     ctx->table_allocs.erase(id);
     ctx->tables.erase(id);
+    if (ctx->table_touch.count(id) && ctx->table_touch[id].ev) (void)hipEventDestroy(ctx->table_touch[id].ev);
+    ctx->table_touch.erase(id);
     return 0;
 }
 
@@ -6590,11 +6746,21 @@
 int cc_read_bam(cc_ctx* ctx, int32_t table_id, int64_t S, const int32_t* stream_rec, const int32_t* stream_region,
                 int32_t n_regions, const int32_t* region_run, const cc_read_bam_params* prm, int32_t* group_id) {
     if (!ctx || !prm || !group_id || !ctx->tables.count(table_id) || S < 0 || S >= INT32_MAX / 2) return CC_E_INVALID;
-    RC(enter(ctx));
+    HIPCHK(hipSetDevice(ctx->device));
+    Group* ng = new_group(ctx);
+    if (!ng) return CC_E_HIP;
+    ng->table = table_id;
+    PassScope scope;
+    if (const int erc = pass_enter(ctx, scope, *ng, nullptr)) {
+        scope.ctx = nullptr;
+        bind(ctx, 0, *ctx->scratch);
+        free_group(*ng);
+        delete ng;
+        return erc;
+    }
     int32_t gid = ctx->next_id++;
-    ctx->groups[gid].reset(new Group());
+    ctx->groups[gid].reset(ng);
     Group& g = *ctx->groups[gid];
-    g.table = table_id;
     g.seed = prm->seed;
     g.scoped = prm->scope_by_run;
     g.delim_filter = prm->delim_filter;
@@ -6630,7 +6796,8 @@
 
 int cc_read_bam_rerun(cc_ctx* ctx, int32_t group_id, uint64_t seed) {
     if (!ctx || !ctx->groups.count(group_id)) return CC_E_INVALID;
-    RC(enter(ctx));
+    PassScope scope;
+    RC(pass_enter(ctx, scope, *ctx->groups[group_id], nullptr));
     ctx->groups[group_id]->seed = seed;
     return read_bam_run(ctx, group_id);
 }
@@ -6643,7 +6810,7 @@
 
 int cc_group_free(cc_ctx* ctx, int32_t group_id) {
     if (!ctx || !ctx->groups.count(group_id)) return CC_E_INVALID;
-    (void)hipStreamSynchronize(ctx->stream);
+    (void)wait_lanes(ctx);
     {
         Group* gp = ctx->groups[group_id].get();
         std::vector<DeferredCheck> keep;
@@ -6651,16 +6818,17 @@
             if (d.g != gp) keep.push_back(d);
         ctx->deferred.swap(keep);
     }
-    for (DevBuf& b : ctx->groups[group_id]->buf)
-        if (b.p) (void)hipFree(b.p);
+    if (ctx->d_err == ctx->groups[group_id]->d_err) bind(ctx, 0, *ctx->scratch);
+    free_group(*ctx->groups[group_id]);
     ctx->groups.erase(group_id);
     return 0;
 }
 
 int cc_consensus_maker(cc_ctx* ctx, int32_t group_id, double cutoff, int64_t* n_out) {
     if (!ctx || !ctx->groups.count(group_id)) return CC_E_INVALID;
-    RC(enter(ctx));
     Group& g = *ctx->groups[group_id];
+    PassScope scope;
+    RC(pass_enter(ctx, scope, g, nullptr));
     auto pass = [&]() -> int {
         RC(flush_derive(ctx, g.table));
         const DevTable& T = ctx->tables[g.table];
@@ -6714,8 +6882,9 @@
 
 int cc_duplex_consensus(cc_ctx* ctx, int32_t group_id, const int32_t* bc_swap, int32_t n_bc, int64_t* n_out) {
     if (!ctx || !ctx->groups.count(group_id) || (!bc_swap && n_bc > 0)) return CC_E_INVALID;
-    RC(enter(ctx));
     Group& g = *ctx->groups[group_id];
+    PassScope scope;
+    RC(pass_enter(ctx, scope, g, nullptr));
     auto pass = [&]() -> int {
         RC(flush_derive(ctx, g.table));
         const DevTable& T = ctx->tables[g.table];
@@ -6751,9 +6920,10 @@
                             int64_t* n_out) {
     if (!ctx || !ctx->groups.count(sgroup) || !ctx->groups.count(ssgroup) || (!bc_swap && n_bc > 0))
         return CC_E_INVALID;
-    RC(enter(ctx));
     Group& g = *ctx->groups[sgroup];
     Group& s = *ctx->groups[ssgroup];
+    PassScope scope;
+    RC(pass_enter(ctx, scope, g, &s));
     auto pass = [&]() -> int {
         RC(flush_derive(ctx, g.table));
         RC(flush_derive(ctx, s.table));
@@ -6837,7 +7007,6 @@
 }
 
 Group& scratch_group(cc_ctx* ctx, int32_t table) {
-    if (!ctx->scratch) ctx->scratch.reset(new Group());
     Group& g = *ctx->scratch;
     g.table = table;
     g.fast = false;
@@ -7754,7 +7923,6 @@
     const int64_t nsum = (int64_t)n_counters + fam_len, ntot = nsum + fam_len;
     if (ntot == 0) return 0;
     int brc = 0;
-    if (!ctx->scratch) ctx->scratch.reset(new Group());
     Group& g = *ctx->scratch;
     int64_t* d = GB(reduce_buf, ntot);
     std::vector<int64_t> h((size_t)ntot);
@@ -7790,7 +7958,6 @@
     if (!r) return CC_E_UNSUPPORTED;
     RC(enter(ctx));
     int brc = 0;
-    if (!ctx->scratch) ctx->scratch.reset(new Group());
     Group& g = *ctx->scratch;
     int64_t* d = GB(reduce_max, n);
     HIPCHK(hipMemcpyAsync(d, v, sizeof(int64_t) * n, hipMemcpyHostToDevice, ctx->stream));
diff --git a/consensuscruncher_amd/csrc/name_format.hip.inc b/consensuscruncher_amd/csrc/name_format.hip.inc
--- a/consensuscruncher_amd/csrc/name_format.hip.inc
+++ b/consensuscruncher_amd/csrc/name_format.hip.inc
@@ -133,9 +133,9 @@
     const uint32_t j = threadIdx.x % NM_LANES;
     if (i >= n) return;
     const int32_t* f = src.fields(i);
-    (void)CC_IDX(f[0], bc.n, DS_REC);
-    (void)CC_IDX(f[5], cg.n, DS_REC);
-    (void)CC_IDX(f[6], cg.n, DS_REC);
+    (void)CC_IDXG(f[0], bc.n, DS_REC, &st->guard);
+    (void)CC_IDXG(f[5], cg.n, DS_REC, &st->guard);
+    (void)CC_IDXG(f[6], cg.n, DS_REC, &st->guard);
     nmc::CsnLay y;
     const uint32_t e = nmc::csn_layout(f, src.suf(i), bc, cg, y);
     const uint64_t off = off32[i];
@@ -158,7 +158,7 @@
     const int64_t i = (int64_t)blockIdx.x * (NM_T / NM_LANES) + (threadIdx.x / NM_LANES);
     const uint32_t j = threadIdx.x % NM_LANES;
     if (i >= n) return;
-    const int64_t rt = CC_IDX(rec_tag[i], T.n, DS_REC), rd = CC_IDX(rec_ds[i], T.n, DS_REC);
+    const int64_t rt = CC_IDXG(rec_tag[i], T.n, DS_REC, &st->guard), rd = CC_IDXG(rec_ds[i], T.n, DS_REC, &st->guard);
     uint64_t ta, da;
     uint32_t tl, dl;
     const bool ok = name_slots(T, rt, rd, &ta, &tl, &da, &dl);
diff --git a/consensuscruncher_amd/csrc/table_unpack.hip.inc b/consensuscruncher_amd/csrc/table_unpack.hip.inc
--- a/consensuscruncher_amd/csrc/table_unpack.hip.inc
+++ b/consensuscruncher_amd/csrc/table_unpack.hip.inc
@@ -180,6 +180,7 @@
     std::vector<void*>& al = ctx->table_allocs[id];
     UnpackGuard guard{ctx, id};
     DevTable T{};
+    T.guard = ctx->d_err + ERR_GUARD;
     T.n = n;
     RC(dev_alloc(ctx, al, &T.tid, n));
     RC(dev_alloc(ctx, al, &T.pos, n));
diff --git a/consensuscruncher_amd/native.py b/consensuscruncher_amd/native.py
--- a/consensuscruncher_amd/native.py
+++ b/consensuscruncher_amd/native.py
@@ -252,6 +252,7 @@
     "cc_table_derive": (C.c_int, [P, C.c_int32]),
     "cc_table_fetch": (C.c_int64, [P, C.c_int32, C.c_char_p, P, C.c_int64]),
     "cc_guard_reruns": (C.c_int64, [P]),
+    "cc_group_reruns": (C.c_int, [P, C.c_int32, i64p]),
     "cc_debug_poison": (C.c_int, [P, C.c_int32, C.c_char_p, C.c_int64, C.c_int32]),
     "cc_debug_scan": (C.c_int, [P, C.c_int32, C.c_int32, P, C.c_int64, P, P, P, i64p]),
     "cc_debug_sort_pairs": (C.c_int, [P, C.c_int32, P, P, C.c_int64, C.c_uint32, C.c_uint32, P, P]),
diff --git a/include/consensuscruncher_amd.h b/include/consensuscruncher_amd.h
--- a/include/consensuscruncher_amd.h
+++ b/include/consensuscruncher_amd.h
@@ -296,6 +296,7 @@
 int cc_debug_build(void);
 int64_t cc_launch_count(void);
 int64_t cc_guard_reruns(cc_ctx *ctx);
+int cc_group_reruns(cc_ctx *ctx, int32_t group_id, int64_t *out);
 int cc_debug_poison(cc_ctx *ctx, int32_t group_id, const char *name, int64_t bytes, int32_t value);
 int cc_debug_scan(cc_ctx *ctx, int32_t kind, int32_t engine, const void *in, int64_t n, const int32_t *aux,
                   void *out_a, void *out_b, int64_t *total);
```

Measured after the change: 3.309 billion, median of 6. 1.11x the previous value.
